# apple/ml-4m

Hardware: AMD Instinct MI355X
Metric: multimodal tokens/sec (4M-B train step, whole job) (higher is better)
Workload: dtype bf16; 1 GPU; 4M-B mod7 (fm_base_12e_12d_swiglu_nobias, 360.8M params, 8 input / 7 target modalities) masked-modeling train step, 224^2 token grids, 128 input + 128 target tokens/sample, AdamW; model=fm_base_12e_12d_swiglu_nobias, per_gpu_batch=256, global_batch=256, seq_len=256, parallelism=dp1

## Files before the change

include/fourm_hip.h:

```cpp
#ifndef FOURM_HIP_H
#define FOURM_HIP_H
#include <stdint.h>

#ifdef __cplusplus
extern "C" {
#endif

#define FM_ABI_VERSION 11
int fm_abi_version(void);
const char* fm_last_error(void);

enum fm_epilogue {
    FM_EPI_BF16 = 0,
    FM_EPI_GELU = 1,
    FM_EPI_RESIDUAL = 2,
    FM_EPI_SWIGLU = 3,
    FM_EPI_F32 = 4,
    FM_EPI_TANH = 5,
    FM_EPI_SWIGLU_BWD = 6,
    FM_EPI_GELU_BWD = 7
};

typedef struct fm_gemm_group {
    const void* W;
    void* out;
    int32_t N, K, ldw, pad_;
} fm_gemm_group;

typedef struct fm_gemm_nt_args {
    const void* W; const void* W2; const void* X;
    void* out; void* out2; const void* res; const void* bias; const void* bias2;
    int32_t M, N, K, ldw, ldx, ldo, ldo2, ldr, Hp, epilogue;
    const fm_gemm_group* groups; const int32_t* tile_group; int32_t max_N;
    int32_t fixed_tiling;
    const int32_t* m_dev; const int32_t* row0_dev;
    void* splitk_ws; int64_t splitk_ws_bytes;
    int32_t conv_C, conv_H, conv_W, conv_Ho, conv_Wo, conv_stride, conv_up, conv_pad_;
} fm_gemm_nt_args;
int fm_gemm_nt(const fm_gemm_nt_args* args, void* stream);
void fm_set_gemm_nt_config(int cfg);
int fm_get_gemm_nt_config(void);
void fm_set_reserved_cus(int n);
int fm_get_reserved_cus(void);

typedef struct fm_gemm_tn_args {
    const void* A; const void* B; void* out;
    int32_t R, N, K, lda, ldb, ldo, a_cols, b_cols, splits, force_tr;
    const fm_gemm_group* groups; const int32_t* seg_start; const int32_t* seg_count;
    int32_t n_groups, max_N, max_R, pad_;
} fm_gemm_tn_args;
int fm_gemm_tn(const fm_gemm_tn_args* args, void* stream);
#define FM_TN_MAX_JOBS 16
typedef struct fm_gemm_tn_job {
    const void* A; const void* B; void* out;
    int32_t R, N, K, lda, ldb, ldo, a_cols, b_cols;
} fm_gemm_tn_job;
int fm_gemm_tn_multi(const fm_gemm_tn_job* jobs, int n_jobs, void* stream);
void fm_set_gemm_tn_config(int cfg);
int fm_get_gemm_tn_config(void);
void fm_set_tn_transpose_read(int on);
int fm_get_tn_transpose_read(void);

int fm_layernorm_fwd(const void* x, int ldx, const void* w, const void* b, void* y, int ldy, int y_is_f32,
                     void* mean, void* rstd, const int32_t* row_map, int R, int D, float eps, void* stream);
int fm_layernorm_fwd_res(const void* x, int ldx, const void* delta, int ldd, void* x_out, int ldxo, const void* w, const void* b,
                         void* y, int ldy, int y_is_f32, void* mean, void* rstd, const int32_t* row_map, int R, int D, float eps,
                         void* stream);
int fm_layernorm_bwd(const void* dy, int lddy, const int32_t* dy_row_map, const void* x, int ldx, const void* w,
                     const void* mean, const void* rstd, const void* dres, void* dx, int lddx, void* dx_bf16,
                     int lddxbf, void* dw, void* db, int R, int D, void* stream);
int fm_layernorm_bwd_h(const void* dy, int lddy, const void* h, int ldh, const void* x, int ldx, const void* w,
                       const void* mean, const void* rstd, const void* dres, void* dx, int lddx, void* dx_bf16,
                       int lddxbf, void* dw, int R, int D, void* stream);

int fm_headnorm_fwd(const void* x, int ldx, const void* w, const void* b, void* y, int ldy, void* stats, int R, int H, float eps,
                    void* stream);
int fm_headnorm_bwd(const void* dy, int lddy, const void* x, int ldx, const void* w, const void* stats, void* dx, int lddx, void* dw,
                    void* db, int R, int H, void* stream);

enum fm_mask_kind {
    FM_MASK_NONE = 0,
    FM_MASK_KEYPAD = 1,
    FM_MASK_DECODER = 2,
    FM_MASK_DENSE = 3
};
typedef struct fm_attn_args {
    const void* Q; const void* K; const void* V; void* O;
    void* stat_m; void* stat_l;
    int32_t ldq, ldk, ldv, ldo;
    int32_t B, H, Nq, Nk, head_dim, mask_kind;
    float scale; int32_t causal;
    const void* kpad; const int32_t* cs; const int16_t* modq; const int16_t* modk; const void* dense;
    const void* dO; void* dQ; void* dK; void* dV;
    int32_t lddo, lddq, lddk, lddv;
    int32_t force_tr;
    int32_t kv_batch_rows;
    int32_t zero_attn;
} fm_attn_args;
int fm_attn_fwd(const fm_attn_args* args, void* stream);
int fm_attn_bwd(const fm_attn_args* args, void* stream);
void fm_set_attn_transpose_read(int on);
int fm_get_attn_transpose_read(void);

#define FM_ATTN_DECODE_MAX_NK 8192
typedef struct fm_attn_decode_args {
    const void* q; void* k; const void* v; void* o;
    const void* q_w; const void* q_b; const void* k_w; const void* k_b;
    const void* kpad;
    int32_t ldq, ldk, ldv, ldo;
    int32_t B, H, Nk, kv_batch_rows, k_new_row, is_f32, zero_attn, pad_;
    float scale, eps;
} fm_attn_decode_args;
int fm_attn_decode(const fm_attn_decode_args* args, void* stream);

#define FM_MAX_MODS 24
enum fm_mod_kind {
    FM_KIND_TOK = 0,
    FM_KIND_PATCH = 1,
    FM_KIND_SEQ = 2,
    FM_KIND_SEQ_EMB = 3
};
typedef struct fm_mod_desc {
    const void* ids;
    const void* mask;
    const void* dam;
    const void* table;
    const void* pos;
    const void* mod_emb;
    const void* proj_bias;
    int32_t L;
    int32_t kind, ids_are_i64, mod_id;
    int32_t max_len;
    int32_t shifted;
    int32_t mask_stride, id_stride;
    int32_t patch, channels, grid_w, orig_dim;
    int32_t head_index;
    int32_t pad_;
} fm_mod_desc;

typedef struct fm_select_desc {
    fm_mod_desc mods[FM_MAX_MODS];
    int32_t n_mods, batch, dim, n_keep, n_reg, total_len, is_decoder;
    int32_t raw;
    const void* reg_tokens;
    const void* mask_token;
    void* tokens;
    void* emb;
    void* x0;
    void* out_mask;
    void* out_mod;
    void* slot_mod;
    void* slot_src;
    void* slot_pos;
    void* target_ids;
    void* out_cs;
    void* out_mod_pre;
    void* out_mod_index;
    void* patch_rows;
    void* seqemb_rows;
    int32_t patch_ld, seqemb_ld;
    int32_t rows_f32;
    int32_t pad2_;
} fm_select_desc;
int fm_select_embed(const fm_select_desc* desc, void* stream);

typedef struct fm_embed_bwd_mod {
    void* d_table;
    void* d_pos;
    void* d_mod_emb;
    void* d_proj_bias;
    int32_t kind, has_padding_idx, padding_idx, pad_;
} fm_embed_bwd_mod;
typedef struct fm_embed_bwd_desc {
    fm_embed_bwd_mod mods[FM_MAX_MODS];
    const void* dx;
    const void* slot_mod; const void* slot_src; const void* slot_pos;
    void* d_mask_token;
    void* d_reg_tokens;
    int32_t n_mods, batch, dim, Nt, lddx, is_decoder;
} fm_embed_bwd_desc;
int fm_embed_bwd(const fm_embed_bwd_desc* desc, void* stream);

int fm_dense_decoder_mask(const int32_t* cs, const int16_t* mod, void* out, int B, int M, int causal, int use_cs,
                          int use_sep, void* stream);

enum fm_loss_type { FM_LOSS_MOD = 0, FM_LOSS_TOKEN = 1 };
#define FM_SEG_ROWS 256
int fm_segment_rows(const int32_t* head_of_row, int R, int n_heads, int32_t* seg_start, int32_t* seg_count,
                    int32_t* perm, int32_t* row_to_padded, int32_t* tile_group, int Rp, void* stream);
int fm_gather_rows(const void* src, int ld_src, const int32_t* perm, void* dst, int ld_dst, int Rp, int D, void* stream);
int fm_cross_entropy(void* logits, int ldl, const int32_t* perm, const int32_t* tile_group, const int64_t* target_ids,
                     const int32_t* vocab, const int32_t* seg_start, const int32_t* seg_count, const void* grad_scale,
                     int loss_type, int n_heads, int Rp, int max_vocab, void* row_loss, void* row_lse, void* head_loss,
                     void* total_loss, int write_grad, void* stream);

int fm_swiglu_bwd(const void* da, int ldda, const void* gu, int ldgu, void* dgu, int lddgu, int R, int H, int Hp, void* stream);
int fm_gelu_bwd(const void* dh, int lddh, const void* pre, int ldp, void* dpre, int lddp, int R, int H, int Hp, void* stream);
typedef struct fm_shadow_desc {
    const void* src; void* dst;
    int32_t ld_src, ld_dst, rows, cols, transpose, tile_start;
    const void* col_scale;
    int32_t dst_f32, reserved;
} fm_shadow_desc;
int fm_shadow_refresh(const fm_shadow_desc* descs, int n_descs, int total_tiles, void* stream);
#define FM_FOLD_MAX_JOBS 48
typedef struct fm_fold_grad_job {
    const void* dWp; const void* W; const void* gamma; void* gW; void* ggamma;
    int32_t rows, cols, ld_dwp, reserved;
} fm_fold_grad_job;
int fm_fold_colscale_grad(const fm_fold_grad_job* jobs, int n_jobs, void* stream);

int fm_cast_pad(const void* src, int ld_src, void* dst, int ld_dst, int rows, int cols, void* stream);
int fm_transpose_cast_pad(const void* src, int ld_src, void* dst, int ld_dst, int dst_cols, int rows, int cols, void* stream);
int fm_colsum(const void* dy, int ldy, void* db, int R, int N, void* stream);
int fm_f32_to_bf16(const void* src, void* dst, int64_t n, void* stream);
int fm_bf16_to_f32_scaled(const void* src, void* dst, int64_t n, float scale, void* stream);
int fm_add_bf16_f32(const void* x, const void* delta, void* out, int64_t n, void* stream);
int fm_scale_rows_bf16(void* x, int ld, const void* scale, int rows_per_sample, int R, int N, void* stream);

int fm_vit_patch_rows(const void* pixels, void* rows, int ld, int B, int C, int H, int W, int P, int rows_f32, void* stream);
int fm_vit_emb_rows(const void* pos, const void* mod_emb, void* x, int ldx, int B, int Np, int D, void* stream);
int fm_vit_colsum(const void* dy, int ldy, void* db, int R, int N, void* ws, int64_t ws_bytes, void* stream);

int fm_lora_apply(const void* x, int ldx, const void* down, int64_t down_sr, int64_t down_sk, const void* up, int64_t up_sn, int64_t up_sr,
                  void* y, int ldy, float scale, void* p_out, int R, int K, int N, int r, int x_f32, int y_f32, void* stream);
int fm_lora_grad(const void* a, int lda, const void* b, void* out, int64_t out_sn, int64_t out_sr, float scale, int accumulate,
                 int R, int n, int r, int a_f32, void* stream);

int fm_adamw(void* p, const void* g, void* m, void* v, int64_t n, float lr, float beta1, float beta2, float eps,
             float weight_decay, int64_t step, const void* grad_mult, const void* hyper, void* sumsq, void* stream);
#define FM_ADAMW_CHUNK 8192
typedef struct fm_adamw_job {
    void* p; const void* g; void* m; void* v; void* dst_plain; void* dst_t;
    int32_t rows, cols, ld_plain, ld_t, tile_start, pad_;
} fm_adamw_job;
int fm_adamw_shadow(const fm_adamw_job* jobs, int n_jobs, int total_tiles, float lr, float beta1, float beta2, float eps,
                    float weight_decay, int64_t step, const void* grad_mult, const void* hyper, void* sumsq, void* stream);
int fm_sumsq(const void* x, int64_t n, void* out, void* stream);
int fm_clip_coef(const void* sumsq, float max_norm, void* norm_out, void* coef_out, void* stream);

int fm_sample_tokens(const void* logits, int ld, int logits_are_f32, int R, int V, float temperature, int top_k, float top_p,
                     const void* uniforms, void* out_ids, void* out_prob, void* stream);
int fm_guidance_combine(const void* uncond, int ldu, int uncond_is_f32, const void* cond, int ldc, int cond_is_f32, float weight,
                        void* out, int ldo, int R, int V, int accumulate, void* stream);
int fm_maskgit_commit(const void* prob, const void* samples, const int32_t* mod_pos, int B, int N, int num_select, void* tensor,
                      int tensor_is_i64, int L, void* input_mask, void* target_mask, int32_t* top_idx, void* stream);

typedef struct fm_gemm_f32_args {
    const void* X; const void* W; const void* W2; void* out; void* out2; const void* res; const void* bias; const void* bias2;
    int64_t sxm, sxk, swn, swk;
    int32_t M, N, K, ldo, ldo2, ldr, Hp, epilogue, accumulate, max_N, seg_rows, n_groups;
    const fm_gemm_group* groups; const int32_t* tile_group; const int32_t* seg_start; const int32_t* seg_count;
} fm_gemm_f32_args;
int fm_gemm_f32(const fm_gemm_f32_args* args, void* stream);
int fm_attn_f32_fwd(const fm_attn_args* args, void* stream);
int fm_attn_f32_bwd(const fm_attn_args* args, void* stream);
int fm_layernorm_bwd_f32(const void* dy, int lddy, const int32_t* dy_row_map, const void* x, int ldx, const void* w, const void* mean,
                         const void* rstd, const void* dres, void* dx, int lddx, void* dx2, int lddx2, void* dw, void* db, int R, int D,
                         void* stream);
int fm_headnorm_f32_fwd(const void* x, int ldx, const void* w, const void* b, void* y, int ldy, void* stats, int R, int H, float eps, void* stream);
int fm_headnorm_f32_bwd(const void* dy, int lddy, const void* x, int ldx, const void* w, const void* stats, void* dx, int lddx, void* dw, void* db,
                        int R, int H, void* stream);
int fm_swiglu_bwd_f32(const void* da, int ldda, const void* gu, int ldgu, void* dgu, int lddgu, int R, int H, int Hp, void* stream);
int fm_gelu_bwd_f32(const void* dh, int lddh, const void* pre, int ldp, void* dpre, int lddp, int R, int H, void* stream);
int fm_colsum_f32(const void* dy, int ldy, void* db, int R, int N, void* stream);
int fm_cross_entropy_f32(void* logits, int ldl, const int32_t* perm, const int32_t* tile_group, const int64_t* target_ids,
                         const int32_t* vocab, const int32_t* seg_start, const int32_t* seg_count, const void* grad_scale, int loss_type,
                         int n_heads, int padded_rows, int max_vocab, void* row_loss, void* row_lse, void* head_loss, void* total_loss,
                         int write_grad, void* stream);

int fm_unet_im2col_f32(const void* src1, int ld1, int C1, const void* src2, int ld2, int C2, int H2, int W2, void* out, int ldo, int kpad,
                       int B, int H, int W, int ksize, int stride, int up1, void* stream);
int fm_groupnorm_nhwc_f32(const void* x, int ldx, const void* add, int ld_add, const void* w, const void* b, void* y, int ldy, int B, int HW, int C,
                          int groups, float eps, int silu, void* stream);
int fm_unet_attention_f32(const void* qkv, int ld, void* out, int ldo, int B, int T, int heads, int ch, void* stream);
int fm_add_f32(const void* a, int lda, const void* b, int ldb, void* out, int ldo, int64_t rows, int C, void* stream);
int fm_silu_f32(const void* x, void* y, int64_t n, void* stream);
int fm_timestep_embedding_f32(const void* t, void* out, int ldo, int B, int dim, float max_period, void* stream);
int fm_unet_col2im_f32(const void* col, int ldc, void* dsrc, int ld, int C, int B, int H, int W, int ksize, int stride, int up1, int accumulate, void* stream);
int fm_groupnorm_nhwc_bwd_f32(const void* dy, int lddy, const void* x, int ldx, const void* add, int ld_add, const void* w, const void* b, void* dx, int lddx,
                              void* dw, void* db, void* dadd, int ld_dadd, void* scratch, int B, int HW, int C, int groups, float eps, int silu, void* stream);
int fm_unet_attention_bwd_f32(const void* qkv, int ld, const void* dout, int lddo, void* dqkv, int lddqkv, void* scratch, int B, int T, int heads, int ch,
                              void* stream);
int fm_silu_bwd_f32(const void* dy, const void* x, void* dx, int64_t n, void* stream);

int fm_vq_patchify(const void* img, void* out, int ld_out, int B, int C, int H, int W, int P, void* stream);
int fm_l2norm_rows(const void* x, int ldx, void* y, int ldy, int R, int D, void* stream);
int fm_vq_assign(const void* z, int ldz, const void* codes_normalized, const void* embed, int K, int D, int R,
                 int tokens_per_image, int normalize_latents, void* ws_val, void* ws_idx, int splits, int64_t* tokens,
                 void* quant, void* stream);
#define FM_VQ_WIDE_TILE 128
int fm_vq_assign_wide(const void* z, int ldz, const void* codes_normalized, const void* embed, int K, int D, int R,
                      int tokens_per_image, void* ws_val, void* ws_idx, int code_tiles, int64_t* tokens, void* quant, void* stream);
int fm_memcodes_assign(const void* z, int ldz, const void* keys, const void* values, int K, int d, int H, int R,
                       int tokens_per_image, void* ws_val, void* ws_idx, int code_tiles, int64_t* tokens, void* quant, void* stream);
int fm_vq_code_stats(const void* z, int ldz, const int64_t* tokens, int R, int D, int K, void* bins, void* sums, void* stream);
int fm_vq_ema_update(const void* bins, const void* sums, void* embed, void* cluster_size, int K, int D, float decay, void* stream);
int fm_vq_code_bias(const void* embed, int K, int D, void* bias, void* stream);
int fm_vq_assign_bias(const void* z, int ldz, const void* codes, const void* code_bias, const void* embed, int K, int D, int R,
                      int tokens_per_image, int normalize_latents, void* ws_val, void* ws_idx, int splits, int64_t* tokens,
                      void* quant, void* stream);
int fm_vq_code_stats_raw(const void* z, int ldz, const int64_t* tokens, int R, int D, int K, void* bins, void* sums, void* stream);
int fm_vq_ema_update_euclid(const void* bins, const void* sums, void* embed, void* embed_avg, void* cluster_size, void* total_scratch,
                            int K, int D, float decay, float eps, void* stream);

int fm_vq_unpatchify(const void* rows, int ld_rows, void* img, int B, int C, int H, int W, int P, void* stream);
#define FM_CONVNEXT_MAX_C 4
int fm_convnext_block(const void* x, void* y, const void* dw_weight, const void* dw_bias, const void* ln_weight, const void* ln_bias,
                      const void* pw1_weight, const void* pw1_bias, const void* pw2_weight, const void* pw2_bias, const void* gamma,
                      int B, int C, int H, int W, float eps, void* stream);
int fm_vq_latent_grad(const void* z, int ldz, const void* embed, const int64_t* tokens, const void* dquant, int ld_dquant, const void* grad_loss,
                      float commitment_weight, void* dz, int ld_dz, void* commit_value, int R, int D, void* stream);
int fm_tanh_bwd_f32(const void* dy, const void* t, void* dx, int R, int N, int ld, void* stream);
int fm_embed_rows_f32(const void* table, const int64_t* idx, void* out, int ld_out, int R, int D, void* stream);
int fm_split3_bf16(const void* x, int ldx, void* out, int ldo, int R, int K, int weight_order, int apply_tanh, void* stream);
int fm_vq_patchify_ex(const void* img, const int64_t* labels, const void* cls_emb, const void* scale, const void* shift, void* out, int ld_out,
                      int B, int C, int H, int W, int P, void* stream);
int fm_vq_cls_emb_bwd(const void* d_patches, int ld, const int64_t* labels, void* d_cls_emb, int B, int C, int H, int W, int P, void* stream);
int fm_vq_latent_grad_normalized(const void* z, int ldz, const void* embed, const int64_t* tokens, const void* dquant, int ld_dquant, const void* grad_loss,
                                 float commitment_weight, void* dz, int ld_dz, void* commit_value, int R, int D, void* stream);

int fm_image_mask(const void* noise, const int32_t* input_budget, const int32_t* target_budget, int B, int L, void* input_mask,
                  void* target_mask, int32_t* decoder_attention_mask, void* stream);

int fm_unpack_image_u8(const void* src, void* dst, int B, int H, int W, int C, const float* mean, const float* stdv, void* stream);
int fm_unpack_ids_u16(const void* src, int64_t* dst, int64_t n, void* stream);
int fm_unpack_mask_bits(const void* bits, void* dst, int B, int L, void* stream);
int fm_decoder_attention_from_target(const void* target_mask, int32_t* decoder_attention_mask, int B, int L, void* stream);

int fm_token_budgets(const void* main_draws, const void* extra_draws, const int32_t* num_tokens, const int32_t* min_tokens,
                     const int32_t* max_tokens, const void* is_img, const int32_t* input_budget, int B, int T, int E, int M,
                     int32_t* budget, int32_t* tries, void* stream);

typedef struct fm_span_mask_args {
    const int32_t* ids; const int32_t* len; const int32_t* unit; const void* noise; const double* keep_prob; const int32_t* r_choice;
    const int32_t* input_budget; const int32_t* target_budget; const int32_t* sentinel_ids;
    const void* emb; void* emb_out; int32_t* src;
    int32_t* tensor; void* input_mask; void* target_mask; int32_t* decoder_attention_mask; int32_t* tries;
    int32_t B, ld_ids, T, ld_noise, n_sentinels, max_tokens, vocab_offset, pad_id, emb_rows, emb_dim;
} fm_span_mask_args;
int fm_span_mask(const fm_span_mask_args* p, void* stream);

int fm_unet_im2col(const void* src1, int ld1, int C1, const void* src2, int ld2, int C2, int H2, int W2, void* out, int ldo, int kpad,
// ... 19 lines not shown
```

ml-4m_amd/csrc/layernorm.hip:

```cpp
#include <algorithm>
#include "common.h"
#include "fourm_hip.h"

namespace {

constexpr int MAXC_LIMIT = 8;

__device__ __forceinline__ float4 ld4(const float* p, bool nt) {
    if (nt) { const f32x4_t t = __builtin_nontemporal_load((const f32x4_t*)p); return make_float4(t[0], t[1], t[2], t[3]); }
    return *(const float4*)p;
}
__device__ __forceinline__ uint2 ld2u(const bf16_t* p, bool nt) {
    typedef __attribute__((ext_vector_type(2))) unsigned int u2_t;
    if (nt) { const u2_t t = __builtin_nontemporal_load((const u2_t*)p); return make_uint2(t[0], t[1]); }
    return *(const uint2*)p;
}
template <typename T> __device__ __forceinline__ void store4(T* p, float a, float b, float c, float d);
template <> __device__ __forceinline__ void store4<float>(float* p, float a, float b, float c, float d) {
    *(float4*)p = make_float4(a, b, c, d);
}
template <> __device__ __forceinline__ void store4<bf16_t>(bf16_t* p, float a, float b, float c, float d) {
    *(uint2*)p = make_uint2(pack2bf(a, b), pack2bf(c, d));
}

template <typename OutT, int MAXC, bool RES = false>
__global__ __launch_bounds__(256) void ln_fwd_kernel(const float* __restrict__ x, int ldx, const float* __restrict__ w,
                                                     const float* __restrict__ b, OutT* __restrict__ y, int ldy,
                                                     float* __restrict__ mean, float* __restrict__ rstd,
                                                     const int* __restrict__ row_map, int R, int D, float eps,
                                                     const bf16_t* __restrict__ delta = nullptr, int ldd = 0, float* __restrict__ xo = nullptr, int ldxo = 0,
                                                     int nt_res = 0) {
    const int lane = threadIdx.x & 63, wave = threadIdx.x >> 6;
    const int nch = D >> 2;
    float4 ww[MAXC], bb[MAXC];
#pragma unroll
    for (int c = 0; c < MAXC; ++c) {
        const int ch = lane + 64 * c;
        ww[c] = ch < nch ? *(const float4*)(w + ch * 4) : make_float4(0.f, 0.f, 0.f, 0.f);
        bb[c] = (b && ch < nch) ? *(const float4*)(b + ch * 4) : make_float4(0.f, 0.f, 0.f, 0.f);
    }
    constexpr int NR = 2;
    for (int r0 = blockIdx.x * 4 + wave; r0 < R; r0 += gridDim.x * 4 * NR) {
        float4 v[NR][MAXC];
#pragma unroll
        for (int q = 0; q < NR; ++q) {
            const int r = r0 + q * gridDim.x * 4;
#pragma unroll
            for (int c = 0; c < MAXC; ++c) {
                const int ch = lane + 64 * c;
                v[q][c] = (ch < nch && r < R) ? ld4(x + (size_t)r * ldx + ch * 4, nt_res & 2) : make_float4(0.f, 0.f, 0.f, 0.f);
            }
        }
        if constexpr (RES) {
            uint2 dl[NR][MAXC];
#pragma unroll
            for (int q = 0; q < NR; ++q) {
                const int r = r0 + q * gridDim.x * 4;
#pragma unroll
                for (int c = 0; c < MAXC; ++c) {
                    const int ch = lane + 64 * c;
                    dl[q][c] = (ch < nch && r < R) ? ld2u(delta + (size_t)r * ldd + ch * 4, nt_res & 2) : make_uint2(0u, 0u);
                }
            }
#pragma unroll
            for (int q = 0; q < NR; ++q) {
                const int r = r0 + q * gridDim.x * 4;
#pragma unroll
                for (int c = 0; c < MAXC; ++c) {
                    const int ch = lane + 64 * c;
                    float d4[4];
                    unpack_bf4(dl[q][c], d4);
                    v[q][c].x += d4[0]; v[q][c].y += d4[1]; v[q][c].z += d4[2]; v[q][c].w += d4[3];
                    if (ch < nch && r < R) {
                        if (nt_res & 1) __builtin_nontemporal_store(f32x4_t{v[q][c].x, v[q][c].y, v[q][c].z, v[q][c].w}, (f32x4_t*)(xo + (size_t)r * ldxo + ch * 4));
                        else *(float4*)(xo + (size_t)r * ldxo + ch * 4) = v[q][c];
                    }
                }
            }
        }
#pragma unroll
        for (int q = 0; q < NR; ++q) {
            const int r = r0 + q * gridDim.x * 4;
            if (r >= R) continue;
            float s = 0.f;
#pragma unroll
            for (int c = 0; c < MAXC; ++c) s += (v[q][c].x + v[q][c].y) + (v[q][c].z + v[q][c].w);
            const float mu = wave_sum(s) / (float)D;
            float sq = 0.f;
#pragma unroll
            for (int c = 0; c < MAXC; ++c) {
                const int ch = lane + 64 * c;
                if (ch < nch) {
                    const float a0 = v[q][c].x - mu, a1 = v[q][c].y - mu, a2 = v[q][c].z - mu, a3 = v[q][c].w - mu;
                    sq += (a0 * a0 + a1 * a1) + (a2 * a2 + a3 * a3);
                }
            }
            const float rs = rsqrtf(wave_sum(sq) / (float)D + eps);
            if (lane == 0) {
                if (mean) mean[r] = mu;
                if (rstd) rstd[r] = rs;
            }
            const int dst = row_map ? row_map[r] : r;
            if (dst < 0) continue;
            OutT* yr = y + (size_t)dst * ldy;
#pragma unroll
            for (int c = 0; c < MAXC; ++c) {
                const int ch = lane + 64 * c;
                if (ch < nch)
                    store4<OutT>(yr + ch * 4, (v[q][c].x - mu) * rs * ww[c].x + bb[c].x, (v[q][c].y - mu) * rs * ww[c].y + bb[c].y,
                                 (v[q][c].z - mu) * rs * ww[c].z + bb[c].z, (v[q][c].w - mu) * rs * ww[c].w + bb[c].w);
            }
        }
    }
}

static int ln_nt_flags() {
    static const int f = [] { const char* e = getenv("FOURM_LN_NT"); return e ? atoi(e) : 24; }();
    return f;
}
static int bwd_rows(int R) {
    static const int env = [] { const char* e = getenv("FOURM_LN_BWD_ROWS"); return e ? atoi(e) : 0; }();
    if (env >= 4) return env;
    return R >= 512 * 64 ? 64 : 32;
}

template <int MAXC, bool FROM_H = false, bool HAS_DB = true>
__global__ __launch_bounds__(256) void ln_bwd_kernel(const bf16_t* __restrict__ dy, int lddy, const int* __restrict__ dy_row_map,
                                                     const bf16_t* __restrict__ h, int ldh,
                                                     const float* __restrict__ x, int ldx, const float* __restrict__ w,
                                                     const float* __restrict__ mean, const float* __restrict__ rstd,
                                                     const float* dres, float* dx, int lddx, bf16_t* __restrict__ dx_bf, int lddxbf,
                                                     float* __restrict__ dw, float* __restrict__ db, int R, int D, int BWD_ROWS, int nt_dx) {
    extern __shared__ __attribute__((aligned(16))) char smem[];
    float* red = (float*)smem;
    const int lane = threadIdx.x & 63, wave = threadIdx.x >> 6;
    const int nch = D >> 2;
    float4 aw[MAXC], ab[MAXC], wv[MAXC], iw[FROM_H ? MAXC : 1];
    bool from_x[FROM_H ? MAXC : 1];
#pragma unroll
    for (int c = 0; c < MAXC; ++c) {
        aw[c] = ab[c] = make_float4(0.f, 0.f, 0.f, 0.f);
        const int ch = lane + 64 * c;
        wv[c] = ch < nch ? *(const float4*)(w + ch * 4) : make_float4(0.f, 0.f, 0.f, 0.f);
        if constexpr (FROM_H) {
            from_x[c] = fminf(fminf(fabsf(wv[c].x), fabsf(wv[c].y)), fminf(fabsf(wv[c].z), fabsf(wv[c].w))) < 1e-20f;
            iw[c] = from_x[c] ? make_float4(0.f, 0.f, 0.f, 0.f) : make_float4(1.f / wv[c].x, 1.f / wv[c].y, 1.f / wv[c].z, 1.f / wv[c].w);
        }
    }
    const int r_end = min(R, (int)(blockIdx.x + 1) * BWD_ROWS);
    constexpr int NR = 2;
    for (int r0 = blockIdx.x * BWD_ROWS + wave; r0 < r_end; r0 += 4 * NR) {
        uint2 dyp[NR][MAXC], hp[NR][FROM_H ? MAXC : 1];
        float4 xv[NR][MAXC], rv[NR][MAXC];
        float mu[NR], rs[NR];
        bool live[NR];
#pragma unroll
        for (int q = 0; q < NR; ++q) {
            const int r = r0 + 4 * q;
            live[q] = r < r_end;
            const int rr = live[q] ? r : r0;
            const int src = dy_row_map ? dy_row_map[rr] : rr;
            mu[q] = mean[rr]; rs[q] = rstd[rr];
#pragma unroll
            for (int c = 0; c < MAXC; ++c) {
                const int ch = lane + 64 * c;
                dyp[q][c] = make_uint2(0u, 0u);
                xv[q][c] = rv[q][c] = make_float4(0.f, 0.f, 0.f, 0.f);
                if (ch < nch && live[q]) {
                    if (src >= 0) dyp[q][c] = ld2u(dy + (size_t)src * lddy + ch * 4, nt_dx & 2);
                    if constexpr (FROM_H) {
                        hp[q][c] = ld2u(h + (size_t)rr * ldh + ch * 4, nt_dx & 4);
                        if (from_x[c]) xv[q][c] = *(const float4*)(x + (size_t)rr * ldx + ch * 4);
                    } else xv[q][c] = *(const float4*)(x + (size_t)rr * ldx + ch * 4);
                    if (dres) rv[q][c] = ld4(dres + (size_t)rr * lddx + ch * 4, nt_dx & 2);
                }
            }
        }
#pragma unroll
        for (int q = 0; q < NR; ++q) {
            if (!live[q]) continue;
            const int r = r0 + 4 * q;
            float4 g[MAXC], xh[MAXC];
            float s1 = 0.f, s2 = 0.f;
#pragma unroll
            for (int c = 0; c < MAXC; ++c) {
                const int ch = lane + 64 * c;
                g[c] = xh[c] = make_float4(0.f, 0.f, 0.f, 0.f);
                if (ch < nch) {
                    const uint2 p = dyp[q][c];
                    const float4 d = make_float4(bf2f((bf16_t)(p.x & 0xffff)), bf2f((bf16_t)(p.x >> 16)), bf2f((bf16_t)(p.y & 0xffff)), bf2f((bf16_t)(p.y >> 16)));
                    const float4 v = xv[q][c];
                    xh[c] = make_float4((v.x - mu[q]) * rs[q], (v.y - mu[q]) * rs[q], (v.z - mu[q]) * rs[q], (v.w - mu[q]) * rs[q]);
                    if constexpr (FROM_H) {
                        const uint2 hh = hp[q][c];
                        if (!from_x[c]) xh[c] = make_float4(bf2f((bf16_t)(hh.x & 0xffff)) * iw[c].x, bf2f((bf16_t)(hh.x >> 16)) * iw[c].y,
                                                            bf2f((bf16_t)(hh.y & 0xffff)) * iw[c].z, bf2f((bf16_t)(hh.y >> 16)) * iw[c].w);
                    }
                    aw[c].x += d.x * xh[c].x; aw[c].y += d.y * xh[c].y; aw[c].z += d.z * xh[c].z; aw[c].w += d.w * xh[c].w;
                    if constexpr (HAS_DB) { ab[c].x += d.x; ab[c].y += d.y; ab[c].z += d.z; ab[c].w += d.w; }
                    g[c] = make_float4(d.x * wv[c].x, d.y * wv[c].y, d.z * wv[c].z, d.w * wv[c].w);
                    s1 += (g[c].x + g[c].y) + (g[c].z + g[c].w);
                    s2 += (g[c].x * xh[c].x + g[c].y * xh[c].y) + (g[c].z * xh[c].z + g[c].w * xh[c].w);
                }
            }
            const float m1 = wave_sum(s1) / (float)D, m2 = wave_sum(s2) / (float)D;
#pragma unroll
            for (int c = 0; c < MAXC; ++c) {
                const int ch = lane + 64 * c;
                if (ch < nch) {
                    const float4 t = rv[q][c];
                    const float4 o = make_float4(rs[q] * (g[c].x - m1 - xh[c].x * m2) + t.x, rs[q] * (g[c].y - m1 - xh[c].y * m2) + t.y,
                                                 rs[q] * (g[c].z - m1 - xh[c].z * m2) + t.z, rs[q] * (g[c].w - m1 - xh[c].w * m2) + t.w);
                    if (nt_dx & 1) __builtin_nontemporal_store(f32x4_t{o.x, o.y, o.z, o.w}, (f32x4_t*)(dx + (size_t)r * lddx + ch * 4));
                    else *(float4*)(dx + (size_t)r * lddx + ch * 4) = o;
                    if (dx_bf) *(uint2*)(dx_bf + (size_t)r * lddxbf + ch * 4) = make_uint2(pack2bf(o.x, o.y), pack2bf(o.z, o.w));
                }
            }
        }
    }
    if (!dw && !db) return;
#pragma unroll
    for (int c = 0; c < MAXC; ++c) {
        const int ch = lane + 64 * c;
        if (ch < nch) {
            *(float4*)(red + (size_t)wave * D + ch * 4) = aw[c];
            if constexpr (HAS_DB) *(float4*)(red + (size_t)(4 + wave) * D + ch * 4) = ab[c];
        }
    }
    __syncthreads();
    for (int i = threadIdx.x; i < D; i += 256) {
        if (dw) unsafeAtomicAdd(dw + i, (red[i] + red[D + i]) + (red[2 * D + i] + red[3 * D + i]));
        if constexpr (HAS_DB) if (db) unsafeAtomicAdd(db + i, (red[4 * D + i] + red[5 * D + i]) + (red[6 * D + i] + red[7 * D + i]));
    }
}


__device__ __forceinline__ float group16_sum(float v) {
    v += __shfl_xor(v, 1, 64); v += __shfl_xor(v, 2, 64); v += __shfl_xor(v, 4, 64); v += __shfl_xor(v, 8, 64);
    return v;
}

__global__ __launch_bounds__(256) void headnorm_fwd_kernel(const bf16_t* __restrict__ x, int ldx, const float* __restrict__ w,
                                                           const float* __restrict__ b, bf16_t* __restrict__ y, int ldy,
                                                           float2* __restrict__ stats, int R, int H, float eps) {
    const int sub = threadIdx.x & 15;
    const float4 wv = *(const float4*)(w + sub * 4);
    const float4 bv = b ? *(const float4*)(b + sub * 4) : make_float4(0.f, 0.f, 0.f, 0.f);
    const size_t total = (size_t)R * H;
    for (size_t v = (size_t)blockIdx.x * 16 + (threadIdx.x >> 4); v < total; v += (size_t)gridDim.x * 16) {
        const int r = v / H, h = v % H;
        const uint2 p = *(const uint2*)(x + (size_t)r * ldx + h * 64 + sub * 4);
        const float e[4] = {bf2f((bf16_t)(p.x & 0xffff)), bf2f((bf16_t)(p.x >> 16)), bf2f((bf16_t)(p.y & 0xffff)), bf2f((bf16_t)(p.y >> 16))};
        const float mean = group16_sum(e[0] + e[1] + e[2] + e[3]) * (1.0f / 64.0f);
        float q = 0.f;
#pragma unroll
        for (int i = 0; i < 4; ++i) q += (e[i] - mean) * (e[i] - mean);
        const float rs = rsqrtf(group16_sum(q) * (1.0f / 64.0f) + eps);
        const float o0 = (e[0] - mean) * rs * wv.x + bv.x, o1 = (e[1] - mean) * rs * wv.y + bv.y;
        const float o2 = (e[2] - mean) * rs * wv.z + bv.z, o3 = (e[3] - mean) * rs * wv.w + bv.w;
        *(uint2*)(y + (size_t)r * ldy + h * 64 + sub * 4) = make_uint2(pack2bf(o0, o1), pack2bf(o2, o3));
        if (sub == 0 && stats) stats[v] = make_float2(mean, rs);
    }
}

__global__ __launch_bounds__(256) void headnorm_bwd_kernel(const bf16_t* __restrict__ dy, int lddy, const bf16_t* __restrict__ x, int ldx,
                                                           const float* __restrict__ w, const float2* __restrict__ stats,
                                                           bf16_t* __restrict__ dx, int lddx, float* __restrict__ dw, float* __restrict__ db,
                                                           int R, int H) {
    __shared__ float red[2][16][64];
    const int sub = threadIdx.x & 15, grp = threadIdx.x >> 4;
    const float4 wv = *(const float4*)(w + sub * 4);
    const float wj[4] = {wv.x, wv.y, wv.z, wv.w};
    float aw[4] = {0.f, 0.f, 0.f, 0.f}, ab[4] = {0.f, 0.f, 0.f, 0.f};
    const size_t total = (size_t)R * H;
    for (size_t v = (size_t)blockIdx.x * 16 + grp; v < total; v += (size_t)gridDim.x * 16) {
        const int r = v / H, h = v % H;
        const uint2 px = *(const uint2*)(x + (size_t)r * ldx + h * 64 + sub * 4);
        const uint2 pd = *(const uint2*)(dy + (size_t)r * lddy + h * 64 + sub * 4);
        const float2 st = stats[v];
        const float e[4] = {bf2f((bf16_t)(px.x & 0xffff)), bf2f((bf16_t)(px.x >> 16)), bf2f((bf16_t)(px.y & 0xffff)), bf2f((bf16_t)(px.y >> 16))};
        const float d[4] = {bf2f((bf16_t)(pd.x & 0xffff)), bf2f((bf16_t)(pd.x >> 16)), bf2f((bf16_t)(pd.y & 0xffff)), bf2f((bf16_t)(pd.y >> 16))};
        float xh[4], g[4], s1 = 0.f, s2 = 0.f;
#pragma unroll
        for (int i = 0; i < 4; ++i) {
            xh[i] = (e[i] - st.x) * st.y;
            g[i] = d[i] * wj[i];
            s1 += g[i]; s2 += g[i] * xh[i];
            aw[i] += d[i] * xh[i]; ab[i] += d[i];
        }
        s1 = group16_sum(s1) * (1.0f / 64.0f); s2 = group16_sum(s2) * (1.0f / 64.0f);
        float o[4];
#pragma unroll
        for (int i = 0; i < 4; ++i) o[i] = st.y * (g[i] - s1 - xh[i] * s2);
        *(uint2*)(dx + (size_t)r * lddx + h * 64 + sub * 4) = make_uint2(pack2bf(o[0], o[1]), pack2bf(o[2], o[3]));
    }
#pragma unroll
    for (int i = 0; i < 4; ++i) { red[0][grp][sub * 4 + i] = aw[i]; red[1][grp][sub * 4 + i] = ab[i]; }
    __syncthreads();
    if (threadIdx.x < 128) {
        const int which = threadIdx.x >> 6, c = threadIdx.x & 63;
        float s = 0.f;
#pragma unroll
        for (int gq = 0; gq < 16; ++gq) s += red[which][gq][c];
        float* dst = which ? db : dw;
        if (dst) unsafeAtomicAdd(dst + c, s);
    }
}

}

static int chunks_for(int D) { const int c = (D / 4 + 63) / 64; return c <= 2 ? 2 : c <= 3 ? 3 : c <= 4 ? 4 : 8; }

extern "C" int fm_layernorm_fwd(const void* x, int ldx, const void* w, const void* b, void* y, int ldy, int y_is_f32,
                                void* mean, void* rstd, const int32_t* row_map, int R, int D, float eps, void* stream) {
    FM_CHECK_ARG(x && w && y, "fm_layernorm_fwd: null pointer");
    FM_CHECK_ARG(R > 0 && D > 0 && D % 4 == 0 && D <= 64 * 4 * MAXC_LIMIT, "fm_layernorm_fwd: D=%d must be a multiple of 4 and <= %d", D, 64 * 4 * MAXC_LIMIT);
    FM_CHECK_ARG(ldx % 4 == 0 && ldy % 4 == 0, "fm_layernorm_fwd: leading dims must be multiples of 4");
    int grid = (R + 3) / 4;
    if (grid > 256 * 16) grid = 256 * 16;
#define LN_FWD(T, C)                                                                                                        \
    hipLaunchKernelGGL((ln_fwd_kernel<T, C>), dim3(grid), dim3(256), 0, (hipStream_t)stream, (const float*)x, ldx, (const float*)w, \
                       (const float*)b, (T*)y, ldy, (float*)mean, (float*)rstd, row_map, R, D, eps)
#define LN_FWD_C(T)                                    \
    switch (chunks_for(D)) {                           \
        case 2: LN_FWD(T, 2); break;                   \
        case 3: LN_FWD(T, 3); break;                   \
        case 4: LN_FWD(T, 4); break;                   \
        default: LN_FWD(T, 8); break;                  \
    }
    if (y_is_f32) { LN_FWD_C(float) } else { LN_FWD_C(bf16_t) }
#undef LN_FWD_C
#undef LN_FWD
    FM_CHECK_LAUNCH("fm_layernorm_fwd");
    return 0;
}

extern "C" int fm_layernorm_fwd_res(const void* x, int ldx, const void* delta, int ldd, void* x_out, int ldxo, const void* w, const void* b,
                                    void* y, int ldy, int y_is_f32, void* mean, void* rstd, const int32_t* row_map, int R, int D, float eps,
                                    void* stream) {
    FM_CHECK_ARG(x && delta && x_out && w && y, "fm_layernorm_fwd_res: null pointer");
    FM_CHECK_ARG(R > 0 && D > 0 && D % 4 == 0 && D <= 64 * 4 * MAXC_LIMIT, "fm_layernorm_fwd_res: D=%d must be a multiple of 4 and <= %d", D, 64 * 4 * MAXC_LIMIT);
    FM_CHECK_ARG(ldx % 4 == 0 && ldy % 4 == 0 && ldd % 4 == 0 && ldxo % 4 == 0, "fm_layernorm_fwd_res: leading dims must be multiples of 4");
    FM_CHECK_ARG((((uintptr_t)delta) & 7) == 0 && (((uintptr_t)x_out | (uintptr_t)x) & 15) == 0, "fm_layernorm_fwd_res: alignment (delta 8 B, x / x_out 16 B)");
    int grid = (R + 3) / 4;
    if (grid > 256 * 16) grid = 256 * 16;
#define LN_FWD(T, C)                                                                                                        \
    hipLaunchKernelGGL((ln_fwd_kernel<T, C, true>), dim3(grid), dim3(256), 0, (hipStream_t)stream, (const float*)x, ldx, (const float*)w, \
                       (const float*)b, (T*)y, ldy, (float*)mean, (float*)rstd, row_map, R, D, eps, (const bf16_t*)delta, ldd, (float*)x_out, ldxo, (ln_nt_flags() & 1) | ((ln_nt_flags() >> 1) & 2))
#define LN_FWD_C(T)                                    \
    switch (chunks_for(D)) {                           \
        case 2: LN_FWD(T, 2); break;                   \
        case 3: LN_FWD(T, 3); break;                   \
        case 4: LN_FWD(T, 4); break;                   \
        default: LN_FWD(T, 8); break;                  \
    }
    if (y_is_f32) { LN_FWD_C(float) } else { LN_FWD_C(bf16_t) }
#undef LN_FWD_C
#undef LN_FWD
    FM_CHECK_LAUNCH("fm_layernorm_fwd_res");
    return 0;
}

static int layernorm_bwd_launch(const void* dy, int lddy, const int32_t* dy_row_map, const void* h, int ldh, const void* x, int ldx, const void* w,
                                const void* mean, const void* rstd, const void* dres, void* dx, int lddx, void* dx_bf16,
                                int lddxbf, void* dw, void* db, int R, int D, void* stream) {
    FM_CHECK_ARG(dy && x && w && mean && rstd && dx, "fm_layernorm_bwd: null pointer");
    FM_CHECK_ARG(!h || ldh % 4 == 0, "fm_layernorm_bwd_h: ldh must be a multiple of 4");
    FM_CHECK_ARG(R > 0 && D > 0 && D % 4 == 0 && D <= 64 * 4 * MAXC_LIMIT, "fm_layernorm_bwd: D=%d unsupported", D);
    FM_CHECK_ARG(ldx % 4 == 0 && lddy % 4 == 0 && lddx % 4 == 0 && lddxbf % 4 == 0, "fm_layernorm_bwd: leading dims must be multiples of 4");
    const int BWD_ROWS = bwd_rows(R);
    const int grid = (R + BWD_ROWS - 1) / BWD_ROWS;
    const size_t lds = (size_t)8 * D * sizeof(float);
#define LN_BWD_(C, FH)                                                                                                      \
    {                                                                                                                       \
        auto k = ln_bwd_kernel<C, FH, !FH>;                                                                                     \
        static bool once = (hipFuncSetAttribute((const void*)k, hipFuncAttributeMaxDynamicSharedMemorySize, 8 * 2048 * 4) == hipSuccess); \
        (void)once;                                                                                                         \
        hipLaunchKernelGGL(k, dim3(grid), dim3(256), lds, (hipStream_t)stream, (const bf16_t*)dy, lddy, dy_row_map, (const bf16_t*)h, ldh, \
                           (const float*)x, ldx, (const float*)w, (const float*)mean, (const float*)rstd, (const float*)dres, (float*)dx, lddx, \
                           (bf16_t*)dx_bf16, lddxbf, (float*)dw, (float*)db, R, D, BWD_ROWS, ((ln_nt_flags() >> 1) & 1) | ((ln_nt_flags() >> 2) & 2) | ((ln_nt_flags() >> 2) & 4));                               \
    }
#define LN_BWD(C) { if (h) LN_BWD_(C, true) else LN_BWD_(C, false) }
    switch (chunks_for(D)) {
        case 2: LN_BWD(2) break;
        case 3: LN_BWD(3) break;
        case 4: LN_BWD(4) break;
        default: LN_BWD(8) break;
    }
#undef LN_BWD
#undef LN_BWD_
    FM_CHECK_LAUNCH("fm_layernorm_bwd");
    return 0;
}

extern "C" int fm_layernorm_bwd(const void* dy, int lddy, const int32_t* dy_row_map, const void* x, int ldx, const void* w,
                                const void* mean, const void* rstd, const void* dres, void* dx, int lddx, void* dx_bf16,
                                int lddxbf, void* dw, void* db, int R, int D, void* stream) {
    return layernorm_bwd_launch(dy, lddy, dy_row_map, nullptr, 0, x, ldx, w, mean, rstd, dres, dx, lddx, dx_bf16, lddxbf, dw, db, R, D, stream);
}

extern "C" int fm_layernorm_bwd_h(const void* dy, int lddy, const void* h, int ldh, const void* x, int ldx, const void* w,
                                  const void* mean, const void* rstd, const void* dres, void* dx, int lddx, void* dx_bf16,
                                  int lddxbf, void* dw, int R, int D, void* stream) {
    FM_CHECK_ARG(h, "fm_layernorm_bwd_h: null pointer");
    return layernorm_bwd_launch(dy, lddy, nullptr, h, ldh, x, ldx, w, mean, rstd, dres, dx, lddx, dx_bf16, lddxbf, dw, nullptr, R, D, stream);
}

extern "C" int fm_headnorm_fwd(const void* x, int ldx, const void* w, const void* b, void* y, int ldy, void* stats, int R, int H, float eps,
                               void* stream) {
    FM_CHECK_ARG(x && w && y && R > 0 && H > 0, "fm_headnorm_fwd: bad argument");
    FM_CHECK_ARG(ldx % 4 == 0 && ldy % 4 == 0 && ((((uintptr_t)x | (uintptr_t)y) & 7) == 0) && ((((uintptr_t)w | (uintptr_t)b) & 15) == 0),
                 "fm_headnorm_fwd: alignment (x/y 8 B, w/b 16 B, leading dims %% 4)");
    const size_t total = (size_t)R * H;
    const int grid = (int)std::min<size_t>((total + 15) / 16, 256 * 32);
    hipLaunchKernelGGL(headnorm_fwd_kernel, dim3(grid), dim3(256), 0, (hipStream_t)stream, (const bf16_t*)x, ldx, (const float*)w, (const float*)b,
                       (bf16_t*)y, ldy, (float2*)stats, R, H, eps);
    FM_CHECK_LAUNCH("fm_headnorm_fwd");
    return 0;
}

extern "C" int fm_headnorm_bwd(const void* dy, int lddy, const void* x, int ldx, const void* w, const void* stats, void* dx, int lddx, void* dw,
                               void* db, int R, int H, void* stream) {
    FM_CHECK_ARG(dy && x && w && stats && dx && R > 0 && H > 0, "fm_headnorm_bwd: bad argument");
    FM_CHECK_ARG(ldx % 4 == 0 && lddy % 4 == 0 && lddx % 4 == 0 && ((((uintptr_t)x | (uintptr_t)dy | (uintptr_t)dx) & 7) == 0) &&
                     ((((uintptr_t)w) & 15) == 0), "fm_headnorm_bwd: alignment (x/dy/dx 8 B, w 16 B, leading dims %% 4)");
    const size_t total = (size_t)R * H;
    const int grid = (int)std::min<size_t>((total + 15) / 16, 256 * 8);
    hipLaunchKernelGGL(headnorm_bwd_kernel, dim3(grid), dim3(256), 0, (hipStream_t)stream, (const bf16_t*)dy, lddy, (const bf16_t*)x, ldx,
                       (const float*)w, (const float2*)stats, (bf16_t*)dx, lddx, (float*)dw, (float*)db, R, H);
    FM_CHECK_LAUNCH("fm_headnorm_bwd");
    return 0;
}
```

ml-4m_amd/csrc/loss.hip:

```cpp
#include "common.h"
#include "fourm_hip.h"

namespace {

constexpr int SEG_ALIGN = FM_SEG_ROWS;

__global__ __launch_bounds__(1024) void segment_rows_kernel(const int32_t* __restrict__ head_of_row, int R, int n_heads,
                                                            int32_t* __restrict__ seg_start, int32_t* __restrict__ seg_count,
                                                            int32_t* __restrict__ perm, int32_t* __restrict__ row_to_padded,
                                                            int32_t* __restrict__ tile_group, int Rp) {
    __shared__ int cnt[FM_MAX_MODS];
    __shared__ int wtot[16];
    const int g = blockIdx.x, tid = threadIdx.x, lane = tid & 63, wave = tid >> 6;
    if (tid < FM_MAX_MODS) cnt[tid] = 0;
    __syncthreads();
    for (int r = tid; r < R; r += 1024) {
        const int hh = head_of_row[r];
        if (hh >= 0 && hh <= g) atomicAdd(&cnt[hh], 1);
    }
    __syncthreads();
    int start = 0;
    for (int m = 0; m < g; ++m) start += (cnt[m] + SEG_ALIGN - 1) / SEG_ALIGN * SEG_ALIGN;
    const int mine = cnt[g];
    const int padded = (mine + SEG_ALIGN - 1) / SEG_ALIGN * SEG_ALIGN;
    if (tid == 0) { seg_start[g] = start; seg_count[g] = mine; }
    for (int t = tid; t < padded / SEG_ALIGN; t += 1024) tile_group[start / SEG_ALIGN + t] = g;
    if (g == n_heads - 1) {
        for (int t = (start + padded) / SEG_ALIGN + tid; t < Rp / SEG_ALIGN; t += 1024) tile_group[t] = -1;
        for (int r = start + padded + tid; r < Rp; r += 1024) perm[r] = -1;
    }
    for (int r = start + mine + tid; r < start + padded; r += 1024) perm[r] = -1;
    int run = 0;
    for (int base = 0; base < R; base += 1024) {
        const int r = base + tid;
        const int f = (r < R && head_of_row[r] == g) ? 1 : 0;
        const int inc = wave_scan_incl(f);
        if (lane == 63) wtot[wave] = inc;
        __syncthreads();
        int off = 0, tot = 0;
        for (int w = 0; w < 16; ++w) { if (w < wave) off += wtot[w]; tot += wtot[w]; }
        __syncthreads();
        if (f) {
            const int dst = start + run + off + inc - 1;
            perm[dst] = r;
            row_to_padded[r] = dst;
        }
        run += tot;
    }
}

__global__ void fill_i32_kernel(int32_t* p, int v, int n) {
    const int i = blockIdx.x * 256 + threadIdx.x;
    if (i < n) p[i] = v;
}

__device__ __forceinline__ void online_merge(float& m, float& s, float m2, float s2) {
    const float mn = fmaxf(m, m2);
    s = s * __expf(m - mn) + s2 * __expf(m2 - mn);
    m = mn;
}

__global__ __launch_bounds__(256) void ce_fwd_kernel(const bf16_t* __restrict__ logits, int ldl, const int32_t* __restrict__ perm,
                                                     const int32_t* __restrict__ tile_group, const long long* __restrict__ target_ids,
                                                     const int32_t* __restrict__ vocab, float* __restrict__ row_loss, float* __restrict__ row_lse) {
    __shared__ float red_m[4], red_s[4];
    const int pr = blockIdx.x;
    const int g = tile_group[pr / SEG_ALIGN];
    if (g < 0) return;
    const int src = perm[pr];
    if (src < 0) {
        if (threadIdx.x == 0) { row_loss[pr] = 0.f; row_lse[pr] = 0.f; }
        return;
    }
    const int V = vocab[g];
    const bf16_t* row = logits + (size_t)pr * ldl;
    float m = -INFINITY, ssum = 0.f;
    for (int c = threadIdx.x * 8; c < V; c += 256 * 8) {
        float v[8];
        if (c + 8 <= V) {
            const uint4 p = *(const uint4*)(row + c);
            const uint32_t w[4] = {p.x, p.y, p.z, p.w};
#pragma unroll
            for (int e = 0; e < 4; ++e) { v[2 * e] = bf2f((bf16_t)(w[e] & 0xffff)); v[2 * e + 1] = bf2f((bf16_t)(w[e] >> 16)); }
        } else {
#pragma unroll
            for (int e = 0; e < 8; ++e) v[e] = c + e < V ? bf2f(row[c + e]) : -INFINITY;
        }
        float cm = v[0];
#pragma unroll
        for (int e = 1; e < 8; ++e) cm = fmaxf(cm, v[e]);
        const float mn = fmaxf(m, cm);
        float add = 0.f;
#pragma unroll
        for (int e = 0; e < 8; ++e) add += __expf(v[e] - mn);
        ssum = ssum * __expf(m - mn) + add;
        m = mn;
    }
#pragma unroll
    for (int o = 32; o > 0; o >>= 1) {
        const float m2 = __shfl_xor(m, o, 64), s2 = __shfl_xor(ssum, o, 64);
        if (m2 > -INFINITY || m > -INFINITY) online_merge(m, ssum, m2, s2);
    }
    const int lane = threadIdx.x & 63, wave = threadIdx.x >> 6;
    if (lane == 0) { red_m[wave] = m; red_s[wave] = ssum; }
    __syncthreads();
    if (threadIdx.x == 0) {
        float M = red_m[0], S = red_s[0];
        for (int w = 1; w < 4; ++w)
            if (red_m[w] > -INFINITY) online_merge(M, S, red_m[w], red_s[w]);
        const float lse = M + __logf(S);
        row_lse[pr] = lse;
        row_loss[pr] = lse - bf2f(row[target_ids[src]]);
    }
}

__global__ __launch_bounds__(256) void ce_bwd_kernel(bf16_t* __restrict__ logits, int ldl, const int32_t* __restrict__ perm,
                                                     const int32_t* __restrict__ tile_group, const long long* __restrict__ target_ids,
                                                     const int32_t* __restrict__ vocab, const int32_t* __restrict__ seg_count,
                                                     const float* __restrict__ gscale, int loss_type, int n_heads,
                                                     const float* __restrict__ row_lse) {
    const int pr = blockIdx.x;
    const int g = tile_group[pr / SEG_ALIGN];
    if (g < 0) return;
    const int V = vocab[g];
    const int Vp = (V + 63) / 64 * 64;
    bf16_t* row = logits + (size_t)pr * ldl;
    const int src = perm[pr];
    if (src < 0) {
        for (int c = threadIdx.x; c < Vp / 8; c += 256) *(uint4*)(row + c * 8) = make_uint4(0u, 0u, 0u, 0u);
        return;
    }
    float w;
    if (loss_type == FM_LOSS_MOD) {
        w = 1.0f / ((float)seg_count[g] * (float)n_heads);
    } else {
        float tot = 0.f;
        for (int mm = 0; mm < n_heads; ++mm) tot += (float)seg_count[mm] * (float)vocab[mm];
        w = (float)V / tot;
    }
    w *= gscale ? gscale[0] : 1.0f;
    const float lse = row_lse[pr];
    const int tgt = (int)target_ids[src];
    for (int c = threadIdx.x * 8; c < Vp; c += 256 * 8) {
        const uint4 p = *(const uint4*)(row + c);
        const uint32_t wd[4] = {p.x, p.y, p.z, p.w};
        float o[8];
#pragma unroll
        for (int e = 0; e < 8; ++e) {
            const float x = bf2f((bf16_t)((e & 1) ? (wd[e >> 1] >> 16) : (wd[e >> 1] & 0xffff)));
            o[e] = (c + e < V) ? (__expf(x - lse) - ((c + e) == tgt ? 1.f : 0.f)) * w : 0.f;
        }
        *(uint4*)(row + c) = make_uint4(pack2bf(o[0], o[1]), pack2bf(o[2], o[3]), pack2bf(o[4], o[5]), pack2bf(o[6], o[7]));
    }
}

__global__ __launch_bounds__(256) void loss_finalize_kernel(const float* __restrict__ row_loss, const int32_t* __restrict__ seg_start,
                                                            const int32_t* __restrict__ seg_count, const int32_t* __restrict__ vocab,
                                                            int n_heads, int loss_type, float* __restrict__ head_loss, float* __restrict__ total) {
    __shared__ float red[4];
    __shared__ float hl[FM_MAX_MODS];
    const int lane = threadIdx.x & 63, wave = threadIdx.x >> 6;
    for (int g = 0; g < n_heads; ++g) {
        const int s0 = seg_start[g], n = seg_count[g];
        float s = 0.f;
        for (int i = threadIdx.x; i < n; i += 256) s += row_loss[s0 + i];
        s = wave_sum(s);
        if (lane == 0) red[wave] = s;
        __syncthreads();
        if (threadIdx.x == 0) hl[g] = n > 0 ? ((red[0] + red[1]) + (red[2] + red[3])) / (float)n : 0.f;
        __syncthreads();
    }
    if (threadIdx.x == 0) {
        float tot = 0.f, wsum = 0.f;
        for (int g = 0; g < n_heads; ++g) {
            head_loss[g] = hl[g];
            if (loss_type == FM_LOSS_MOD) { tot += hl[g]; wsum += 1.f; }
            else { const float w = (float)seg_count[g] * (float)vocab[g]; tot += hl[g] * w; wsum += w; }
        }
        total[0] = tot / wsum;
    }
}

__global__ __launch_bounds__(256) void ce_f32_kernel(float* logits, int ld, const int* perm, const int* tile_group, const long long* target_ids,
                                                     const int* vocab, const int* seg_count, const float* grad_scale, int loss_type, int n_heads,
                                                     float* row_loss, float* row_lse, int write_grad, int seg_rows) {
    __shared__ float red[4];
    const int pr = blockIdx.x;
    const int g = tile_group[pr / seg_rows];
    if (g < 0) return;
    const int src = perm[pr];
    const int V = vocab[g];
    float* row = logits + (size_t)pr * ld;
    if (src < 0) {
        if (!write_grad) { if (threadIdx.x == 0) { row_loss[pr] = 0.f; row_lse[pr] = 0.f; } }
        else for (int c = threadIdx.x; c < V; c += 256) row[c] = 0.f;
        return;
    }
    const int tgt = (int)target_ids[src];
    if (!write_grad) {
        float mx = -INFINITY;
        for (int c = threadIdx.x; c < V; c += 256) mx = fmaxf(mx, row[c]);
        mx = wave_max(mx);
        __syncthreads();
        if ((threadIdx.x & 63) == 0) red[threadIdx.x >> 6] = mx;
        __syncthreads();
        mx = fmaxf(fmaxf(red[0], red[1]), fmaxf(red[2], red[3]));
        float s = 0.f;
        for (int c = threadIdx.x; c < V; c += 256) s += expf(row[c] - mx);
        s = wave_sum(s);
        __syncthreads();
        if ((threadIdx.x & 63) == 0) red[threadIdx.x >> 6] = s;
        __syncthreads();
        s = (red[0] + red[1]) + (red[2] + red[3]);
        const float lse = mx + logf(s);
        if (threadIdx.x == 0) { row_lse[pr] = lse; row_loss[pr] = lse - row[tgt]; }
        return;
    }
    float coef;
    if (loss_type == FM_LOSS_MOD) coef = 1.0f / ((float)n_heads * (float)seg_count[g]);
    else {
        double tot = 0.0;
        for (int h = 0; h < n_heads; ++h) tot += (double)seg_count[h] * (double)vocab[h];
        coef = (float)((double)V / tot);
    }
    coef *= grad_scale ? grad_scale[0] : 1.0f;
    const float lse = row_lse[pr];
    for (int c = threadIdx.x; c < V; c += 256) row[c] = coef * (expf(row[c] - lse) - (c == tgt ? 1.0f : 0.f));
}


__global__ __launch_bounds__(256) void gather_rows_kernel(const bf16_t* __restrict__ src, int lds_, const int32_t* __restrict__ perm,
                                                          bf16_t* __restrict__ dst, int ldd, int Rp, int D) {
    const int lane = threadIdx.x & 63, wave = threadIdx.x >> 6;
    for (int pr = blockIdx.x * 4 + wave; pr < Rp; pr += gridDim.x * 4) {
        const int s = perm[pr];
        for (int c = lane; c < D / 8; c += 64) {
            uint4 v = make_uint4(0u, 0u, 0u, 0u);
            if (s >= 0) v = *(const uint4*)(src + (size_t)s * lds_ + c * 8);
            *(uint4*)(dst + (size_t)pr * ldd + c * 8) = v;
        }
    }
}

}

extern "C" int fm_segment_rows(const int32_t* head_of_row, int R, int n_heads, int32_t* seg_start, int32_t* seg_count,
                               int32_t* perm, int32_t* row_to_padded, int32_t* tile_group, int Rp, void* stream) {
    FM_CHECK_ARG(head_of_row && seg_start && seg_count && perm && row_to_padded && tile_group, "fm_segment_rows: null pointer");
    FM_CHECK_ARG(n_heads > 0 && n_heads <= FM_MAX_MODS && R > 0, "fm_segment_rows: bad shape");
    FM_CHECK_ARG(Rp % SEG_ALIGN == 0 && Rp >= (R + SEG_ALIGN - 1) / SEG_ALIGN * SEG_ALIGN + (n_heads - 1) * SEG_ALIGN,
                 "fm_segment_rows: padded capacity Rp=%d too small for R=%d rows in %d segments", Rp, R, n_heads);
    hipLaunchKernelGGL(fill_i32_kernel, dim3((R + 255) / 256), dim3(256), 0, (hipStream_t)stream, row_to_padded, -1, R);
    hipLaunchKernelGGL(segment_rows_kernel, dim3(n_heads), dim3(1024), 0, (hipStream_t)stream, head_of_row, R, n_heads, seg_start,
                       seg_count, perm, row_to_padded, tile_group, Rp);
    FM_CHECK_LAUNCH("fm_segment_rows");
    return 0;
}

extern "C" int fm_gather_rows(const void* src, int ld_src, const int32_t* perm, void* dst, int ld_dst, int Rp, int D, void* stream) {
    FM_CHECK_ARG(src && perm && dst && D % 8 == 0 && ld_src % 8 == 0 && ld_dst % 8 == 0, "fm_gather_rows: bad argument");
    int grid = (Rp + 3) / 4;
    if (grid > 4096) grid = 4096;
    hipLaunchKernelGGL(gather_rows_kernel, dim3(grid), dim3(256), 0, (hipStream_t)stream, (const bf16_t*)src, ld_src, perm, (bf16_t*)dst, ld_dst, Rp, D);
    FM_CHECK_LAUNCH("fm_gather_rows");
    return 0;
}

extern "C" int fm_cross_entropy(void* logits, int ldl, const int32_t* perm, const int32_t* tile_group, const int64_t* target_ids,
                                const int32_t* vocab, const int32_t* seg_start, const int32_t* seg_count, const void* grad_scale,
                                int loss_type, int n_heads, int Rp, int max_vocab, void* row_loss, void* row_lse, void* head_loss,
                                void* total_loss, int write_grad, void* stream) {
    FM_CHECK_ARG(logits && perm && tile_group && target_ids && vocab && seg_start && seg_count && row_loss && row_lse && head_loss && total_loss,
                 "fm_cross_entropy: null pointer");
    FM_CHECK_ARG(loss_type == FM_LOSS_MOD || loss_type == FM_LOSS_TOKEN, "fm_cross_entropy: invalid loss type %d", loss_type);
    FM_CHECK_ARG(ldl % 8 == 0 && ldl >= (max_vocab + 63) / 64 * 64, "fm_cross_entropy: ldl=%d too small for vocab %d", ldl, max_vocab);
    FM_CHECK_ARG((((uintptr_t)logits) & 15) == 0, "fm_cross_entropy: logits must be 16-byte aligned");
    if (!write_grad) {
        hipLaunchKernelGGL(ce_fwd_kernel, dim3(Rp), dim3(256), 0, (hipStream_t)stream, (const bf16_t*)logits, ldl, perm, tile_group,
                           (const long long*)target_ids, vocab, (float*)row_loss, (float*)row_lse);
        hipLaunchKernelGGL(loss_finalize_kernel, dim3(1), dim3(256), 0, (hipStream_t)stream, (const float*)row_loss, seg_start, seg_count,
                           vocab, n_heads, loss_type, (float*)head_loss, (float*)total_loss);
    } else {
        hipLaunchKernelGGL(ce_bwd_kernel, dim3(Rp), dim3(256), 0, (hipStream_t)stream, (bf16_t*)logits, ldl, perm, tile_group,
                           (const long long*)target_ids, vocab, seg_count, (const float*)grad_scale, loss_type, n_heads, (const float*)row_lse);
    }
    FM_CHECK_LAUNCH("fm_cross_entropy");
    return 0;
}

extern "C" int fm_cross_entropy_f32(void* logits, int ldl, const int32_t* perm, const int32_t* tile_group, const int64_t* target_ids,
                                    const int32_t* vocab, const int32_t* seg_start, const int32_t* seg_count, const void* grad_scale,
                                    int loss_type, int n_heads, int Rp, int max_vocab, void* row_loss, void* row_lse, void* head_loss,
                                    void* total_loss, int write_grad, void* stream) {
    FM_CHECK_ARG(logits && perm && tile_group && target_ids && vocab && seg_start && seg_count && row_loss && row_lse && head_loss && total_loss,
                 "fm_cross_entropy_f32: null pointer");
    FM_CHECK_ARG(loss_type == FM_LOSS_MOD || loss_type == FM_LOSS_TOKEN, "fm_cross_entropy_f32: invalid loss type %d", loss_type);
    FM_CHECK_ARG(ldl >= max_vocab, "fm_cross_entropy_f32: ldl=%d too small for vocab %d", ldl, max_vocab);
    hipLaunchKernelGGL(ce_f32_kernel, dim3(Rp), dim3(256), 0, (hipStream_t)stream, (float*)logits, ldl, perm, tile_group,
                       (const long long*)target_ids, vocab, seg_count, (const float*)grad_scale, loss_type, n_heads, (float*)row_loss,
                       (float*)row_lse, write_grad, SEG_ALIGN);
    if (!write_grad)
        hipLaunchKernelGGL(loss_finalize_kernel, dim3(1), dim3(256), 0, (hipStream_t)stream, (const float*)row_loss, seg_start, seg_count,
                           vocab, n_heads, loss_type, (float*)head_loss, (float*)total_loss);
    FM_CHECK_LAUNCH("fm_cross_entropy_f32");
    return 0;
}
```

ml-4m_amd/fourm/hip/_lib.py:

```python
import ctypes as C
import os

FM_MAX_MODS = 24
_LIB_PATH = os.environ.get("FOURM_HIP_LIB") or os.path.join(os.path.dirname(os.path.dirname(os.path.abspath(__file__))), "_lib", "libfourm_hip.so")


class FourmHipUnavailable(ImportError):
    pass


def _load():
    if not os.path.exists(_LIB_PATH):
        raise FourmHipUnavailable(
            f"{_LIB_PATH} is missing - build the gfx950 kernels first: python ml-4m_amd/build_ext.py "
            "(the 4M hot path has no fallback implementation)")
    return C.CDLL(_LIB_PATH)


lib = _load()
lib.fm_last_error.restype = C.c_char_p
lib.fm_abi_version.restype = C.c_int
ABI_VERSION = 11
if lib.fm_abi_version() != ABI_VERSION:
    raise FourmHipUnavailable(f"libfourm_hip.so ABI {lib.fm_abi_version()} != expected {ABI_VERSION}; rebuild")

vp, i32, i64, f32 = C.c_void_p, C.c_int32, C.c_int64, C.c_float

EPI_BF16, EPI_GELU, EPI_RESIDUAL, EPI_SWIGLU, EPI_F32, EPI_TANH, EPI_SWIGLU_BWD, EPI_GELU_BWD = 0, 1, 2, 3, 4, 5, 6, 7
MASK_NONE, MASK_KEYPAD, MASK_DECODER, MASK_DENSE = 0, 1, 2, 3
KIND_TOK, KIND_PATCH, KIND_SEQ, KIND_SEQ_EMB = 0, 1, 2, 3
LOSS_MOD, LOSS_TOKEN = 0, 1


class GemmGroup(C.Structure):
    _fields_ = [("W", vp), ("out", vp), ("N", i32), ("K", i32), ("ldw", i32), ("pad_", i32)]


class GemmNTArgs(C.Structure):
    _fields_ = [("W", vp), ("W2", vp), ("X", vp), ("out", vp), ("out2", vp), ("res", vp), ("bias", vp), ("bias2", vp),
                ("M", i32), ("N", i32), ("K", i32), ("ldw", i32), ("ldx", i32), ("ldo", i32), ("ldo2", i32), ("ldr", i32),
                ("Hp", i32), ("epilogue", i32), ("groups", vp), ("tile_group", vp), ("max_N", i32), ("fixed_tiling", i32),
                ("m_dev", vp), ("row0_dev", vp), ("splitk_ws", vp), ("splitk_ws_bytes", i64),
                ("conv_C", i32), ("conv_H", i32), ("conv_W", i32), ("conv_Ho", i32), ("conv_Wo", i32), ("conv_stride", i32), ("conv_up", i32), ("conv_pad_", i32)]


class GemmTNArgs(C.Structure):
    _fields_ = [("A", vp), ("B", vp), ("out", vp), ("R", i32), ("N", i32), ("K", i32), ("lda", i32), ("ldb", i32),
                ("ldo", i32), ("a_cols", i32), ("b_cols", i32), ("splits", i32), ("force_tr", i32), ("groups", vp),
                ("seg_start", vp), ("seg_count", vp), ("n_groups", i32), ("max_N", i32), ("max_R", i32), ("pad_", i32)]


class GemmTNJob(C.Structure):
    _fields_ = [("A", vp), ("B", vp), ("out", vp), ("R", i32), ("N", i32), ("K", i32), ("lda", i32), ("ldb", i32),
                ("ldo", i32), ("a_cols", i32), ("b_cols", i32)]


TN_MAX_JOBS = 16


class AttnArgs(C.Structure):
    _fields_ = [("Q", vp), ("K", vp), ("V", vp), ("O", vp), ("stat_m", vp), ("stat_l", vp),
                ("ldq", i32), ("ldk", i32), ("ldv", i32), ("ldo", i32),
                ("B", i32), ("H", i32), ("Nq", i32), ("Nk", i32), ("head_dim", i32), ("mask_kind", i32),
                ("scale", f32), ("causal", i32),
                ("kpad", vp), ("cs", vp), ("modq", vp), ("modk", vp), ("dense", vp),
                ("dO", vp), ("dQ", vp), ("dK", vp), ("dV", vp),
                ("lddo", i32), ("lddq", i32), ("lddk", i32), ("lddv", i32), ("force_tr", i32), ("kv_batch_rows", i32), ("zero_attn", i32)]


class AttnDecodeArgs(C.Structure):
    _fields_ = [("q", vp), ("k", vp), ("v", vp), ("o", vp), ("q_w", vp), ("q_b", vp), ("k_w", vp), ("k_b", vp), ("kpad", vp),
                ("ldq", i32), ("ldk", i32), ("ldv", i32), ("ldo", i32),
                ("B", i32), ("H", i32), ("Nk", i32), ("kv_batch_rows", i32), ("k_new_row", i32), ("is_f32", i32), ("zero_attn", i32), ("pad_", i32),
                ("scale", f32), ("eps", f32)]


class ModDesc(C.Structure):
    _fields_ = [("ids", vp), ("mask", vp), ("dam", vp), ("table", vp), ("pos", vp), ("mod_emb", vp), ("proj_bias", vp),
                ("L", i32), ("kind", i32), ("ids_are_i64", i32), ("mod_id", i32), ("max_len", i32), ("shifted", i32),
                ("mask_stride", i32), ("id_stride", i32), ("patch", i32), ("channels", i32), ("grid_w", i32),
                ("orig_dim", i32), ("head_index", i32), ("pad_", i32)]


class ShadowDesc(C.Structure):
    _fields_ = [("src", vp), ("dst", vp), ("ld_src", i32), ("ld_dst", i32), ("rows", i32), ("cols", i32),
                ("transpose", i32), ("tile_start", i32), ("col_scale", vp), ("dst_f32", i32), ("reserved", i32)]


FOLD_MAX_JOBS = 48


class FoldGradJob(C.Structure):
    _fields_ = [("dWp", vp), ("W", vp), ("gamma", vp), ("gW", vp), ("ggamma", vp), ("rows", i32), ("cols", i32), ("ld_dwp", i32), ("reserved", i32)]


class GemmF32Args(C.Structure):
    _fields_ = [("X", vp), ("W", vp), ("W2", vp), ("out", vp), ("out2", vp), ("res", vp), ("bias", vp), ("bias2", vp),
                ("sxm", i64), ("sxk", i64), ("swn", i64), ("swk", i64),
                ("M", i32), ("N", i32), ("K", i32), ("ldo", i32), ("ldo2", i32), ("ldr", i32), ("Hp", i32), ("epilogue", i32),
                ("accumulate", i32), ("max_N", i32), ("seg_rows", i32), ("n_groups", i32),
                ("groups", vp), ("tile_group", vp), ("seg_start", vp), ("seg_count", vp)]


class SpanMaskArgs(C.Structure):
    _fields_ = [("ids", vp), ("len", vp), ("unit", vp), ("noise", vp), ("keep_prob", vp), ("r_choice", vp), ("input_budget", vp), ("target_budget", vp),
                ("sentinel_ids", vp), ("emb", vp), ("emb_out", vp), ("src", vp), ("tensor", vp), ("input_mask", vp), ("target_mask", vp),
                ("decoder_attention_mask", vp), ("tries", vp),
                ("B", i32), ("ld_ids", i32), ("T", i32), ("ld_noise", i32), ("n_sentinels", i32), ("max_tokens", i32), ("vocab_offset", i32), ("pad_id", i32),
                ("emb_rows", i32), ("emb_dim", i32)]


class AdamWJob(C.Structure):
    _fields_ = [("p", vp), ("g", vp), ("m", vp), ("v", vp), ("dst_plain", vp), ("dst_t", vp),
                ("rows", i32), ("cols", i32), ("ld_plain", i32), ("ld_t", i32), ("tile_start", i32), ("pad_", i32)]


class SelectDesc(C.Structure):
    _fields_ = [("mods", ModDesc * FM_MAX_MODS),
                ("n_mods", i32), ("batch", i32), ("dim", i32), ("n_keep", i32), ("n_reg", i32), ("total_len", i32),
                ("is_decoder", i32), ("raw", i32),
                ("reg_tokens", vp), ("mask_token", vp),
                ("tokens", vp), ("emb", vp), ("x0", vp), ("out_mask", vp), ("out_mod", vp), ("slot_mod", vp),
                ("slot_src", vp), ("slot_pos", vp), ("target_ids", vp), ("out_cs", vp), ("out_mod_pre", vp),
                ("out_mod_index", vp), ("patch_rows", vp), ("seqemb_rows", vp), ("patch_ld", i32), ("seqemb_ld", i32),
                ("rows_f32", i32), ("pad2_", i32)]


class EmbedBwdMod(C.Structure):
    _fields_ = [("d_table", vp), ("d_pos", vp), ("d_mod_emb", vp), ("d_proj_bias", vp),
                ("kind", i32), ("has_padding_idx", i32), ("padding_idx", i32), ("pad_", i32)]


class EmbedBwdDesc(C.Structure):
    _fields_ = [("mods", EmbedBwdMod * FM_MAX_MODS), ("dx", vp), ("slot_mod", vp), ("slot_src", vp), ("slot_pos", vp),
                ("d_mask_token", vp), ("d_reg_tokens", vp),
                ("n_mods", i32), ("batch", i32), ("dim", i32), ("Nt", i32), ("lddx", i32), ("is_decoder", i32)]


def _sig(name, *argtypes):
    fn = getattr(lib, name)
    fn.argtypes = list(argtypes)
    fn.restype = C.c_int
    return fn


P = C.POINTER
gemm_nt = _sig("fm_gemm_nt", P(GemmNTArgs), vp)
gemm_tn = _sig("fm_gemm_tn", P(GemmTNArgs), vp)
gemm_tn_multi = _sig("fm_gemm_tn_multi", P(GemmTNJob), C.c_int, vp)
layernorm_fwd = _sig("fm_layernorm_fwd", vp, i32, vp, vp, vp, i32, i32, vp, vp, vp, i32, i32, f32, vp)
layernorm_fwd_res = _sig("fm_layernorm_fwd_res", vp, i32, vp, i32, vp, i32, vp, vp, vp, i32, i32, vp, vp, vp, i32, i32, f32, vp)
layernorm_bwd = _sig("fm_layernorm_bwd", vp, i32, vp, vp, i32, vp, vp, vp, vp, vp, i32, vp, i32, vp, vp, i32, i32, vp)
layernorm_bwd_h = _sig("fm_layernorm_bwd_h", vp, i32, vp, i32, vp, i32, vp, vp, vp, vp, vp, i32, vp, i32, vp, i32, i32, vp)
attn_fwd = _sig("fm_attn_fwd", P(AttnArgs), vp)
attn_bwd = _sig("fm_attn_bwd", P(AttnArgs), vp)
attn_decode = _sig("fm_attn_decode", P(AttnDecodeArgs), vp)
ATTN_DECODE_MAX_NK = 8192
select_embed = _sig("fm_select_embed", P(SelectDesc), vp)
embed_bwd = _sig("fm_embed_bwd", P(EmbedBwdDesc), vp)
dense_decoder_mask = _sig("fm_dense_decoder_mask", vp, vp, vp, i32, i32, i32, i32, i32, vp)
segment_rows = _sig("fm_segment_rows", vp, i32, i32, vp, vp, vp, vp, vp, i32, vp)
gather_rows = _sig("fm_gather_rows", vp, i32, vp, vp, i32, i32, i32, vp)
cross_entropy = _sig("fm_cross_entropy", vp, i32, vp, vp, vp, vp, vp, vp, vp, i32, i32, i32, i32, vp, vp, vp, vp, i32, vp)
swiglu_bwd = _sig("fm_swiglu_bwd", vp, i32, vp, i32, vp, i32, i32, i32, i32, vp)
gelu_bwd = _sig("fm_gelu_bwd", vp, i32, vp, i32, vp, i32, i32, i32, i32, vp)
cast_pad = _sig("fm_cast_pad", vp, i32, vp, i32, i32, i32, vp)
transpose_cast_pad = _sig("fm_transpose_cast_pad", vp, i32, vp, i32, i32, i32, i32, vp)
colsum = _sig("fm_colsum", vp, i32, vp, i32, i32, vp)
shadow_refresh = _sig("fm_shadow_refresh", vp, i32, i32, vp)
fold_colscale_grad = _sig("fm_fold_colscale_grad", vp, i32, vp)
headnorm_fwd = _sig("fm_headnorm_fwd", vp, i32, vp, vp, vp, i32, vp, i32, i32, C.c_float, vp)
headnorm_bwd = _sig("fm_headnorm_bwd", vp, i32, vp, i32, vp, vp, vp, i32, vp, vp, i32, i32, vp)
f32_to_bf16 = _sig("fm_f32_to_bf16", vp, vp, i64, vp)
bf16_to_f32_scaled = _sig("fm_bf16_to_f32_scaled", vp, vp, i64, f32, vp)
add_bf16_f32 = _sig("fm_add_bf16_f32", vp, vp, vp, i64, vp)
lib.fm_set_reserved_cus.argtypes = [C.c_int]
lib.fm_get_reserved_cus.restype = C.c_int
lib.fm_get_reserved_cus.argtypes = []
adamw = _sig("fm_adamw", vp, vp, vp, vp, i64, f32, f32, f32, f32, f32, i64, vp, vp, vp, vp)
adamw_shadow = _sig("fm_adamw_shadow", vp, i32, i32, f32, f32, f32, f32, f32, i64, vp, vp, vp, vp)
sumsq = _sig("fm_sumsq", vp, i64, vp, vp)
clip_coef = _sig("fm_clip_coef", vp, f32, vp, vp, vp)
sample_tokens = _sig("fm_sample_tokens", vp, i32, i32, i32, i32, f32, i32, f32, vp, vp, vp, vp)
maskgit_commit = _sig("fm_maskgit_commit", vp, vp, vp, i32, i32, i32, vp, i32, i32, vp, vp, vp, vp)
gemm_f32 = _sig("fm_gemm_f32", P(GemmF32Args), vp)
attn_f32_fwd = _sig("fm_attn_f32_fwd", P(AttnArgs), vp)
attn_f32_bwd = _sig("fm_attn_f32_bwd", P(AttnArgs), vp)
layernorm_bwd_f32 = _sig("fm_layernorm_bwd_f32", vp, i32, vp, vp, i32, vp, vp, vp, vp, vp, i32, vp, i32, vp, vp, i32, i32, vp)
headnorm_f32_fwd = _sig("fm_headnorm_f32_fwd", vp, i32, vp, vp, vp, i32, vp, i32, i32, C.c_float, vp)
headnorm_f32_bwd = _sig("fm_headnorm_f32_bwd", vp, i32, vp, i32, vp, vp, vp, i32, vp, vp, i32, i32, vp)
swiglu_bwd_f32 = _sig("fm_swiglu_bwd_f32", vp, i32, vp, i32, vp, i32, i32, i32, i32, vp)
gelu_bwd_f32 = _sig("fm_gelu_bwd_f32", vp, i32, vp, i32, vp, i32, i32, i32, vp)
colsum_f32 = _sig("fm_colsum_f32", vp, i32, vp, i32, i32, vp)
cross_entropy_f32 = _sig("fm_cross_entropy_f32", vp, i32, vp, vp, vp, vp, vp, vp, vp, i32, i32, i32, i32, vp, vp, vp, vp, i32, vp)
vq_patchify = _sig("fm_vq_patchify", vp, vp, i32, i32, i32, i32, i32, i32, vp)
l2norm_rows = _sig("fm_l2norm_rows", vp, i32, vp, i32, i32, i32, vp)
vq_assign = _sig("fm_vq_assign", vp, i32, vp, vp, i32, i32, i32, i32, i32, vp, vp, i32, vp, vp, vp)
lib.fm_set_tn_transpose_read.argtypes = [C.c_int]
lib.fm_set_gemm_tn_config.argtypes = [C.c_int]
lib.fm_set_attn_transpose_read.argtypes = [C.c_int]

lib.fm_set_gemm_nt_config.argtypes = [C.c_int]
lib.fm_lab_set.argtypes = [C.c_int, C.c_int]
lib.fm_lab_set.restype = None
vq_code_stats = _sig("fm_vq_code_stats", vp, i32, vp, i32, i32, i32, vp, vp, vp)
vq_ema_update = _sig("fm_vq_ema_update", vp, vp, vp, vp, i32, i32, f32, vp)
vq_code_bias = _sig("fm_vq_code_bias", vp, i32, i32, vp, vp)
vq_assign_bias = _sig("fm_vq_assign_bias", vp, i32, vp, vp, vp, i32, i32, i32, i32, i32, vp, vp, i32, vp, vp, vp)
vq_code_stats_raw = _sig("fm_vq_code_stats_raw", vp, i32, vp, i32, i32, i32, vp, vp, vp)
vq_ema_update_euclid = _sig("fm_vq_ema_update_euclid", vp, vp, vp, vp, vp, vp, i32, i32, f32, f32, vp)
vq_unpatchify = _sig("fm_vq_unpatchify", vp, i32, vp, i32, i32, i32, i32, i32, vp)
VQ_WIDE_TILE, CONVNEXT_MAX_C = 128, 4
vq_assign_wide = _sig("fm_vq_assign_wide", vp, i32, vp, vp, i32, i32, i32, i32, vp, vp, i32, vp, vp, vp)
memcodes_assign = _sig("fm_memcodes_assign", vp, i32, vp, vp, i32, i32, i32, i32, i32, vp, vp, i32, vp, vp, vp)
convnext_block = _sig("fm_convnext_block", vp, vp, vp, vp, vp, vp, vp, vp, vp, vp, vp, i32, i32, i32, i32, f32, vp)
vq_latent_grad = _sig("fm_vq_latent_grad", vp, i32, vp, vp, vp, i32, vp, f32, vp, i32, vp, i32, i32, vp)
tanh_bwd_f32 = _sig("fm_tanh_bwd_f32", vp, vp, vp, i32, i32, i32, vp)
embed_rows_f32 = _sig("fm_embed_rows_f32", vp, vp, vp, i32, i32, i32, vp)
vq_patchify_ex = _sig("fm_vq_patchify_ex", vp, vp, vp, vp, vp, vp, i32, i32, i32, i32, i32, i32, vp)
vq_cls_emb_bwd = _sig("fm_vq_cls_emb_bwd", vp, i32, vp, vp, i32, i32, i32, i32, i32, vp)
vq_latent_grad_normalized = _sig("fm_vq_latent_grad_normalized", vp, i32, vp, vp, vp, i32, vp, f32, vp, i32, vp, i32, i32, vp)
scale_rows_bf16 = _sig("fm_scale_rows_bf16", vp, i32, vp, i32, i32, i32, vp)
image_mask = _sig("fm_image_mask", vp, vp, vp, i32, i32, vp, vp, vp, vp)
token_budgets = _sig("fm_token_budgets", vp, vp, vp, vp, vp, vp, vp, i32, i32, i32, i32, vp, vp, vp)
span_mask = _sig("fm_span_mask", P(SpanMaskArgs), vp)
guidance_combine = _sig("fm_guidance_combine", vp, i32, i32, vp, i32, i32, f32, vp, i32, i32, i32, i32, vp)
unpack_image_u8 = _sig("fm_unpack_image_u8", vp, vp, i32, i32, i32, i32, P(C.c_float), P(C.c_float), vp)
unpack_ids_u16 = _sig("fm_unpack_ids_u16", vp, vp, i64, vp)
unpack_mask_bits = _sig("fm_unpack_mask_bits", vp, vp, i32, i32, vp)
decoder_attention_from_target = _sig("fm_decoder_attention_from_target", vp, vp, i32, i32, vp)
split3_bf16 = _sig("fm_split3_bf16", vp, i32, vp, i32, i32, i32, i32, i32, vp)
unet_im2col = _sig("fm_unet_im2col", vp, i32, i32, vp, i32, i32, i32, i32, vp, i32, i32, i32, i32, i32, i32, i32, i32, vp)
groupnorm_nhwc = _sig("fm_groupnorm_nhwc", vp, i32, vp, i32, vp, vp, vp, i32, vp, i32, i32, i32, i32, f32, i32, vp)
add_bf16 = _sig("fm_add_bf16", vp, i32, vp, i32, vp, i32, i64, i32, vp)
silu_f32_to_bf16 = _sig("fm_silu_f32_to_bf16", vp, vp, i64, vp)
timestep_embedding = _sig("fm_timestep_embedding", vp, vp, i32, i32, i32, f32, vp)
unet_attention = _sig("fm_unet_attention", vp, i32, vp, i32, i32, i32, i32, i32, vp)
unet_im2col_f32 = _sig("fm_unet_im2col_f32", vp, i32, i32, vp, i32, i32, i32, i32, vp, i32, i32, i32, i32, i32, i32, i32, i32, vp)
groupnorm_nhwc_f32 = _sig("fm_groupnorm_nhwc_f32", vp, i32, vp, i32, vp, vp, vp, i32, i32, i32, i32, i32, f32, i32, vp)
unet_attention_f32 = _sig("fm_unet_attention_f32", vp, i32, vp, i32, i32, i32, i32, i32, vp)
add_f32 = _sig("fm_add_f32", vp, i32, vp, i32, vp, i32, i64, i32, vp)
silu_f32 = _sig("fm_silu_f32", vp, vp, i64, vp)
timestep_embedding_f32 = _sig("fm_timestep_embedding_f32", vp, vp, i32, i32, i32, f32, vp)
unet_col2im_f32 = _sig("fm_unet_col2im_f32", vp, i32, vp, i32, i32, i32, i32, i32, i32, i32, i32, i32, vp)
groupnorm_nhwc_bwd_f32 = _sig("fm_groupnorm_nhwc_bwd_f32", vp, i32, vp, i32, vp, i32, vp, vp, vp, i32, vp, vp, vp, i32, vp, i32, i32, i32, i32, f32, i32, vp)
unet_attention_bwd_f32 = _sig("fm_unet_attention_bwd_f32", vp, i32, vp, i32, vp, i32, vp, i32, i32, i32, i32, vp)
silu_bwd_f32 = _sig("fm_silu_bwd_f32", vp, vp, vp, i64, vp)
diffusion_x0 = _sig("fm_diffusion_x0", vp, vp, f32, f32, vp, i64, vp)
quantile_abs = _sig("fm_quantile_abs", vp, i32, i64, f32, vp, vp)
diffusion_step = _sig("fm_diffusion_step", vp, vp, f32, f32, vp, vp, vp, f32, f32, f32, f32, vp, vp, i32, i64, vp)
lora_apply = _sig("fm_lora_apply", vp, i32, vp, i64, i64, vp, i64, i64, vp, i32, f32, vp, i32, i32, i32, i32, i32, i32, vp)
lora_grad = _sig("fm_lora_grad", vp, i32, vp, vp, i64, i64, f32, i32, i32, i32, i32, i32, vp)
vit_patch_rows = _sig("fm_vit_patch_rows", vp, vp, i32, i32, i32, i32, i32, i32, i32, vp)
vit_emb_rows = _sig("fm_vit_emb_rows", vp, vp, vp, i32, i32, i32, i32, vp)
vit_colsum = _sig("fm_vit_colsum", vp, i32, vp, i32, i32, vp, i64, vp)
EXPORTS = ["fm_attn_decode", "fm_vit_patch_rows", "fm_vit_emb_rows", "fm_vit_colsum", "fm_lora_apply", "fm_lora_grad", "fm_vq_assign_wide", "fm_memcodes_assign", "fm_convnext_block", "fm_split3_bf16", "fm_unet_im2col", "fm_groupnorm_nhwc", "fm_add_bf16", "fm_silu_f32_to_bf16", "fm_timestep_embedding", "fm_unet_attention", "fm_diffusion_x0", "fm_quantile_abs",
           "fm_diffusion_step", "fm_unpack_image_u8", "fm_unpack_ids_u16", "fm_unpack_mask_bits", "fm_decoder_attention_from_target", "fm_guidance_combine", "fm_image_mask", "fm_token_budgets", "fm_span_mask", "fm_vq_code_stats", "fm_vq_ema_update", "fm_vq_code_bias", "fm_vq_assign_bias", "fm_vq_code_stats_raw", "fm_vq_ema_update_euclid", "fm_vq_unpatchify", "fm_vq_latent_grad", "fm_tanh_bwd_f32", "fm_embed_rows_f32", "fm_vq_patchify_ex", "fm_vq_cls_emb_bwd", "fm_vq_latent_grad_normalized", "fm_abi_version", "fm_last_error", "fm_gemm_nt", "fm_set_gemm_nt_config", "fm_get_gemm_nt_config", "fm_set_reserved_cus", "fm_get_reserved_cus", "fm_bf16_to_f32_scaled", "fm_add_bf16_f32", "fm_scale_rows_bf16", "fm_gemm_tn", "fm_gemm_tn_multi", "fm_set_gemm_tn_config", "fm_get_gemm_tn_config", "fm_set_tn_transpose_read",
           "fm_get_tn_transpose_read", "fm_layernorm_fwd", "fm_layernorm_fwd_res", "fm_layernorm_bwd", "fm_layernorm_bwd_h", "fm_headnorm_fwd", "fm_headnorm_bwd", "fm_attn_fwd", "fm_attn_bwd",
           "fm_set_attn_transpose_read", "fm_get_attn_transpose_read", "fm_select_embed", "fm_embed_bwd",
           "fm_dense_decoder_mask", "fm_segment_rows", "fm_gather_rows", "fm_cross_entropy", "fm_swiglu_bwd",
           "fm_gelu_bwd", "fm_cast_pad", "fm_transpose_cast_pad", "fm_shadow_refresh", "fm_fold_colscale_grad", "fm_colsum", "fm_f32_to_bf16", "fm_adamw", "fm_adamw_shadow",
           "fm_sumsq", "fm_clip_coef", "fm_vq_patchify", "fm_l2norm_rows", "fm_vq_assign",
           "fm_sample_tokens", "fm_maskgit_commit", "fm_gemm_f32", "fm_attn_f32_fwd", "fm_attn_f32_bwd", "fm_layernorm_bwd_f32", "fm_headnorm_f32_fwd", "fm_headnorm_f32_bwd",
           "fm_swiglu_bwd_f32", "fm_gelu_bwd_f32", "fm_colsum_f32", "fm_cross_entropy_f32", "fm_lab_set",
           "fm_unet_im2col_f32", "fm_groupnorm_nhwc_f32", "fm_unet_attention_f32", "fm_add_f32", "fm_silu_f32", "fm_timestep_embedding_f32",
           "fm_unet_col2im_f32", "fm_groupnorm_nhwc_bwd_f32", "fm_unet_attention_bwd_f32", "fm_silu_bwd_f32"]


def check(rc: int):
    if rc != 0:
        raise RuntimeError(f"libfourm_hip: {lib.fm_last_error().decode()} (rc={rc})")
```

ml-4m_amd/fourm/hip/engine.py:

```python
import math
import os
import random
import weakref
from typing import Dict, List, Optional

import torch
import torch.nn as nn

from . import _lib as L
from . import ops

_WEIGHT_EPOCH = 0
FUSE_ACT_BWD = os.environ.get("FOURM_FUSE_ACT_BWD", "0") == "1"
HEADS_DENSE = os.environ.get("FOURM_HEADS_DENSE", "1") == "1"
HEADS_DENSE_MAX = int(os.environ.get("FOURM_HEADS_DENSE_MAX", "8"))
DEFER_RESIDUAL = os.environ.get("FOURM_DEFER_RESIDUAL", "1") == "1"
HOIST_CTX = os.environ.get("FOURM_HOIST_CTX", "1") == "1"
LN_BWD_FROM_H = os.environ.get("FOURM_LN_BWD_FROM_H", "1") == "1"
DP_RESERVE_ALWAYS = os.environ.get("FOURM_DP_RESERVE_ALWAYS", "0") == "1"


def bump_weight_epoch():
    global _WEIGHT_EPOCH
    _WEIGHT_EPOCH += 1


def ru(x, m):
    return (x + m - 1) // m * m


def is_lora(lin) -> bool:
    return hasattr(lin, "lora_down")


def check_lora_targets(model):
    from fourm.models.lora_utils import MAX_LORA_WIDTH, LoRAWrapper
    ok = set()
    for blk in model.encoder:
        ok |= {id(blk.attn.qkv), id(blk.attn.proj)}
    for blk in getattr(model, "decoder", ()):
        ok |= {id(blk.self_attn.qkv), id(blk.self_attn.proj), id(blk.cross_attn.q), id(blk.cross_attn.kv), id(blk.cross_attn.proj)}
    for name, mod in model.named_modules():
        if not isinstance(mod, LoRAWrapper):
            continue
        if id(mod) not in ok:
            raise NotImplementedError(f"LoRA wrapper at '{name}': the HIP engine adapts the attention Linears of the encoder / decoder blocks only "
                                      "(the MLP's fc1 / fc3 run as one launch whose SwiGLU epilogue consumes the pre-activation; embeddings and "
                                      "heads have no low-rank path)")
        width = mod.lora_down.weight.shape[0]
        if width > MAX_LORA_WIDTH:
            raise NotImplementedError(f"LoRA wrapper at '{name}': rank x packed Linears = {width} exceeds {MAX_LORA_WIDTH}")


class Shadow:
    __slots__ = ("buf", "params", "jobs", "stamp")

    def __init__(self, buf, params, jobs):
        self.buf, self.params, self.jobs, self.stamp = buf, params, jobs, None


class Workspace:

    def __init__(self, device, per_stream: bool = False):
        self.device = device
        self.per_stream = per_stream
        self.bufs: Dict[tuple, torch.Tensor] = {}

    def get(self, name, shape, dtype):
        key = (name, tuple(shape), dtype, torch.cuda.current_stream(self.device).cuda_stream) if self.per_stream else (name, tuple(shape), dtype)
        t = self.bufs.get(key)
        if t is None:
            t = self.bufs[key] = torch.zeros(shape, dtype=dtype, device=self.device)
        return t

    def nbytes(self):
        return sum(t.numel() * t.element_size() for t in self.bufs.values())


def fill_mod_desc(md, d, emb, is_dec: bool, mod_id: int, head_index: int = 0, raw: int = 0, name: str = "modality"):
    kind = emb.kind
    t = d["tensor"]
    B = t.shape[0]
    mask = d["target_mask" if is_dec else "input_mask"]
    mask = mask.reshape(B, -1)
    if mask.dtype != torch.bool:
        mask = mask.bool()
    mask = mask.contiguous()
    keep = [mask]
    md.mask, md.mask_stride = mask.data_ptr(), mask.shape[1]
    md.kind, md.mod_id, md.head_index = kind, mod_id, head_index
    md.pos = emb.pos_emb.data_ptr()
    md.mod_emb = emb.mod_emb.data_ptr()
    md.shifted = 1 if (is_dec and kind == L.KIND_SEQ and raw != 2) else 0
    md.max_len = getattr(emb, "max_length", 0) or 0
    if kind in (L.KIND_TOK, L.KIND_SEQ):
        ids = t.reshape(B, -1)
        if ids.dtype not in (torch.int32, torch.int64):
            ids = ids.long()
        ids = ids.contiguous()
        keep.append(ids)
        md.ids, md.ids_are_i64, md.id_stride = ids.data_ptr(), 1 if ids.dtype == torch.int64 else 0, ids.shape[1]
        md.table = emb.token_emb.weight.data_ptr()
        md.L = ids.shape[1] - (1 if md.shifted else 0)
        if ids.shape[1] != mask.shape[1]:
            raise ValueError(f"{name}: tensor has {ids.shape[1]} positions but the mask has {mask.shape[1]}")
    elif kind == L.KIND_PATCH:
        px = t.float().contiguous()
        keep.append(px)
        _, C, Hh, Ww = px.shape
        ps = emb.patch_size[0]
        md.ids, md.id_stride = px.data_ptr(), C * Hh * Ww
        md.patch, md.channels, md.grid_w = ps, C, Ww // ps
        md.L = (Hh // ps) * (Ww // ps)
    else:
        e = t.float().contiguous()
        keep.append(e)
        md.ids, md.id_stride, md.orig_dim = e.data_ptr(), e.shape[1] * e.shape[2], e.shape[2]
        md.proj_bias = emb.emb_proj.bias.data_ptr()
        md.L = e.shape[1]
    if is_dec and (raw != 2 or "decoder_attention_mask" in d):
        dam = d["decoder_attention_mask"].reshape(B, -1)
        if dam.dtype != torch.int32:
            dam = dam.int()
        dam = dam.contiguous()
        keep.append(dam)
        md.dam = dam.data_ptr()
    return keep


class FourMEngine:
    _pending = None
    _drop_now = None
    drop_uniforms = None

    def __init__(self, model):
        from fourm.models.fm_utils import GatedMlp, NormAttention, act_name
        self.model = model
        check_lora_targets(model)
        self.D = model.dim
        blk = model.encoder[0] if len(model.encoder) else model.decoder[0]
        attn0 = blk.attn if hasattr(blk, "attn") else blk.self_attn
        self.H = attn0.num_heads
        if self.D // self.H != 64:
            raise NotImplementedError(f"head_dim {self.D // self.H}: the HIP attention kernels are built for head_dim 64")
        self.qk_norm = isinstance(attn0, NormAttention)
        self.gated = isinstance(blk.mlp, GatedMlp)
        self.act = act_name(blk.mlp.act)
        if self.gated and self.act != "silu":
            raise NotImplementedError("gated MLP is implemented for SiLU (SwiGLU) only")
        if not self.gated and self.act != "gelu":
            raise NotImplementedError("plain MLP is implemented for exact GELU only")
        self.Hd = blk.mlp.hidden_features
        self.Hp = ru(self.Hd, 64)
        self.scale = 64 ** -0.5
        self.eps = blk.norm1.eps
        prec = getattr(model, "compute_precision", None) or os.environ.get("FOURM_PRECISION", "bf16")
        if prec not in ("bf16", "fp32"):
            raise ValueError(f"compute_precision {prec!r}: 'bf16' or 'fp32'")
        self.fp32 = prec == "fp32"
        self.adt = torch.float32 if self.fp32 else torch.bfloat16
        self.ws: Optional[Workspace] = None
        self.shadows: Dict[tuple, Shadow] = {}
        self._shadow_table = None
        self.flat_params = self.flat_grads = None
        self._slices = {}
        self._ctx = None
        self._dw_jobs = None
        self._pending = None
        self.reducer = None

    @property
    def checkpointing(self):
        return bool(getattr(self.model, "use_act_checkpoint", False))

    @property
    def device(self):
        t = getattr(self.model, "mask_token", None)
        return (t if t is not None else next(self.model.parameters())).device

    def _unique_params(self):
        seen, out = set(), []
        for n, p in getattr(self.model, "engine_parameters", self.model.named_parameters)():
            if id(p) not in seen:
                seen.add(id(p))
                out.append((n, p))
        return out

    def flatten(self):
        named = self._unique_params()
        dev = self.device

        def nodecay(n):
            return "norm." in n or ".norm" in n or n.endswith(".bias")
        late = {id(b.cross_attn.kv.weight) for b in self.model.decoder} if self.hoist_ctx else set()
        named.sort(key=lambda np_: (nodecay(np_[0]), id(np_[1]) in late))
        off, slices = 0, {}
        for n, p in named:
            slices[id(p)] = (off, p.numel())
            off += ru(p.numel(), 16)
        flat = torch.zeros(off, dtype=torch.float32, device=dev)
        for n, p in named:
            o, k = slices[id(p)]
            flat[o:o + k].copy_(p.data.reshape(-1))
            p.data = flat[o:o + k].view(p.shape)
        self.flat_params, self._slices = flat, slices
        self.flat_grads = torch.zeros_like(flat)
        self._named = named
        bump_weight_epoch()

    def _ensure_flat(self):
        if self.flat_params is None or self.flat_params.device != self.device:
            self.flatten()
            return
        for n, p in self._named[:4] + self._named[-4:]:
            o, k = self._slices[id(p)]
            if p.data_ptr() != self.flat_params.data_ptr() + 4 * o:
                self.flatten()
                return

    def grad_stages(self):
        m = self.model
        owner = {}

        def claim(stage, module_or_params):
            ps = module_or_params.parameters() if isinstance(module_or_params, nn.Module) else module_or_params
            for p in ps:
                owner[id(p)] = stage
        for i, blk in enumerate(m.decoder):
            claim(f"dec{i}", blk)
        if self.hoist_ctx:
            claim("dec_emb", [b.cross_attn.kv.weight for b in m.decoder] + [b.context_norm.weight for b in m.decoder])
        claim("heads", [m.decoder_norm.weight] + ([m.decoder_norm.bias] if isinstance(m.decoder_norm.bias, nn.Parameter) else []))
        claim("dec_emb", m.decoder_embeddings)
        claim("dec_emb", [m.mask_token])
        claim("ctx", m.decoder_proj_context)
        claim("ctx", m.encoder_norm)
        for i, blk in enumerate(m.encoder):
            claim(f"enc{i}", blk)
        claim("enc_emb", m.encoder_embeddings)
        if m.register_tokens is not None:
            claim("enc_emb", [m.register_tokens])
        stages = {}
        for n, p in self._named:
            o, k = self._slices[id(p)]
            stage = owner.get(id(p), "enc_emb") if k >= 65536 else "tail"
            stages.setdefault(stage, []).append((o, ru(k, 16)))
        return stages

    def _stage(self, name):
        if self.reducer is not None:
            self.reducer.stage_done(name)

    def grad_view(self, p):
        o, k = self._slices[id(p)]
        return self.flat_grads[o:o + k].view(p.shape)

    def grads_were_cleared(self) -> bool:
        live = getattr(self, "_attached", None)
        if not live:
            return True
        for p in live[:4] + live[-4:]:
            if p.grad is None or p.grad.data_ptr() != self.grad_view(p).data_ptr():
                return True
        return False

    def untouched_params(self):
        c = self._ctx
        if c is None or self.reducer is not None:
            return []
        m, touched, cand = self.model, set(), []
        for names, embs in ((c["enc"]["names"], m.encoder_embeddings), (c["dec"]["names"], m.decoder_embeddings)):
            for n, e in embs.items():
                if n in names:
                    touched.update(id(p) for p in e.parameters())
                else:
                    cand.extend(e.parameters())
        return [p for p in cand if id(p) not in touched]

    def attach_grads(self, zero: bool, untouched=()):
        if zero:
            with ops._prof("fills"):
                self.flat_grads.zero_()
            self._window_touched = set()
        skip = {id(p) for p in untouched} - getattr(self, "_window_touched", set())
        self._attached = []
        for n, p in self._named:
            if not p.requires_grad:
                continue
            if id(p) in skip:
                p.grad = None
                continue
            self._window_touched.add(id(p))
            p.grad = self.grad_view(p)
            self._attached.append(p)

    def _stamp(self, params):
        return tuple((p._version, _WEIGHT_EPOCH, p.data_ptr()) for p in params)

    def _get_shadow(self, key, make) -> torch.Tensor:
        s = self.shadows.get(key)
        if s is None:
            s = self.shadows[key] = make()
            for p in s.params:
                regs = getattr(p, "_fourm_shadows", None)
                if regs is None:
                    regs = p._fourm_shadows = []
                regs.append((weakref.ref(self), key))
        if s.stamp != self._stamp(s.params):
            self._refresh_shadows()
        return s.buf

    def _refresh_shadows(self):
        stale = [s for s in self.shadows.values() if s.stamp != self._stamp(s.params)]
        jobs = []
        for s in stale:
            jobs += [(j[0].detach().reshape(j[0].shape[0], -1), j[1], j[2], j[3].detach() if len(j) > 3 and j[3] is not None else None) for j in s.jobs]
        sig = tuple((a.data_ptr(), b.data_ptr(), tr, sc.data_ptr() if sc is not None else 0) for (a, b, tr, sc) in jobs)
        if self._shadow_table is None or self._shadow_table[0] != sig:
            table, tiles = ops.shadow_jobs_table(jobs, self.device)
            self._shadow_table = (sig, table, len(jobs), tiles)
        _, table, n, tiles = self._shadow_table
        ops.shadow_refresh(table, n, tiles)
        for s in stale:
            s.stamp = self._stamp(s.params)

    def mark_shadows_fresh(self, keys, written):
        for key in keys:
            s = self.shadows.get(key)
            if s is not None and all(len(j) == 3 and (id(j[0]), j[1].data_ptr()) in written for j in s.jobs):
                s.stamp = self._stamp(s.params)

    def w(self, p, pad_rows=False):
        if self.fp32:
            return p.detach().reshape(p.shape[0], -1)
        def make():
            out_f, in_f = p.shape[0], p[0].numel()
            buf = torch.zeros(ru(out_f, 64) if pad_rows else out_f, ru(in_f, 64), dtype=torch.bfloat16, device=p.device)
            return Shadow(buf, (p,), [(p, buf, False)])
        s = self._get_shadow(("w", id(p)), make)
        assert not pad_rows or s.shape[0] >= ru(p.shape[0], 64), "w(): the cached image was created without pad_rows"
        return s

    def wt(self, p, pad_rows=False):
        if self.fp32:
            return p.detach().reshape(p.shape[0], -1).t()
        def make():
            out_f, in_f = p.shape[0], p[0].numel()
            buf = torch.zeros(ru(in_f, 64) if pad_rows else in_f, ru(out_f, 64), dtype=torch.bfloat16, device=p.device)
            return Shadow(buf, (p,), [(p, buf, True)])
        s = self._get_shadow(("wt", id(p)), make)
        assert not pad_rows or s.shape[0] >= ru(p[0].numel(), 64), "wt(): the cached image was created without pad_rows"
        return s

    def w_fold(self, lin, norm):
        p, g = lin.weight, norm.weight
        def make():
            out_f, in_f = p.shape
            buf = torch.zeros(out_f, in_f if self.fp32 else ru(in_f, 64), dtype=self.adt, device=p.device)
            return Shadow(buf, (p, g), [(p, buf, False, g)])
        return self._get_shadow(("wfold", id(p)), make)

    def wt_fold_stack(self):
        m, D = self.model, self.D
        def make():
            Ld = len(m.decoder)
            buf = torch.zeros(D, Ld * 2 * D, dtype=self.adt, device=self.device)
            ps, jobs = [], []
            for i, blk in enumerate(m.decoder):
                p, g = blk.cross_attn.kv.weight, blk.context_norm.weight
                ps += [p, g]
                jobs.append((p, buf[:, i * 2 * D:(i + 1) * 2 * D], True, g))
            return Shadow(buf, tuple(ps), jobs)
        return self._get_shadow(("wtfold", 0), make)

    @property
    def hoist_ctx(self):
        h = getattr(self, "_hoist_ctx", None)
        if h is None:
            dec = getattr(self.model, "decoder", ())
            h = HOIST_CTX and len(dec) > 0 and all(
                not isinstance(b.context_norm.bias, nn.Parameter) and b.cross_attn.kv.bias is None and not is_lora(b.cross_attn.kv)
                for b in dec)
            self._hoist_ctx = h
        return h

    def w13t(self, mlp):
        def make():
            buf = torch.zeros(self.D, 2 * self.Hp, dtype=torch.bfloat16, device=self.device)
            p1, p3 = mlp.fc1.weight, mlp.fc3.weight
            return Shadow(buf, (p1, p3), [(p1, buf[:, :self.Hp], True), (p3, buf[:, self.Hp:], True)])
        return self._get_shadow(("w13t", id(mlp)), make)

    def _mod_desc(self, md: L.ModDesc, name, d, emb, is_dec, head_index=0, raw=0):
        return fill_mod_desc(md, d, emb, is_dec, int(self.model.modality_info[name]["id"]), head_index, raw, name)

    def select(self, mod_dict, n_keep: int, is_dec: bool, order: List[str], prefix: str, want_x0=True, heads=None, raw=0):
        m = self.model
        embs = m.decoder_embeddings if is_dec else m.encoder_embeddings
        names = [n for n in order if n in embs]
        if not names:
            raise ValueError("no modality of mod_dict is known to the model")
        if len(names) > L.FM_MAX_MODS:
            raise ValueError(f"{len(names)} modalities exceed FM_MAX_MODS={L.FM_MAX_MODS}")
# ... 216 lines not shown
        R, Rp, D = B * N, x_in.shape[0], self.D
        bf, f32 = self.adt, torch.float32
        dp = self._drop_scales(blk, B, 2, sv, dp)
        h1 = self._ln(blk.norm1, x_in, self._buf(sv, tag, "h1", (Rp, D), bf), R, sv, "n1", tag)
        x_mid = self._buf(sv, tag, "x_mid", (Rp, D), f32)
        self._drop_now = (dp[0], N) if dp else None
        self._self_attn_fwd(blk.attn, h1, x_in, x_mid, B, N, R, Rp, mask, sv, tag)
        h2 = self._ln(blk.norm2, x_mid, self._buf(sv, tag, "h2", (Rp, D), bf), R, sv, "n2", tag)
        x_out = self.ws.get(out_name or (tag + ".x_out" if sv is not None else "scratch.x_out" + tag[-1:]), (Rp, D), f32)
        self._drop_now = (dp[1], N) if dp else None
        self._mlp_fwd(blk.mlp, h2, x_mid, x_out, R, Rp, sv, tag, defer=defer_out)
        self._drop_now = None
        if sv is not None:
            sv["x_in"] = x_in
        return x_out

    def decoder_block_fwd(self, blk, y_in, ctx, B, M, N, sa_mask, xa_mask, sv, tag, defer_out=False, out_name=None, dp=None, ctx_hat=None):
        Rq, Rqp, Rc, Rcp, D = B * M, y_in.shape[0], B * N, ctx.shape[0], self.D
        bf, f32 = self.adt, torch.float32
        dp = self._drop_scales(blk, B, 3, sv, dp)
        h1 = self._ln(blk.norm1, y_in, self._buf(sv, tag, "h1", (Rqp, D), bf), Rq, sv, "n1", tag)
        y1 = self._buf(sv, tag, "y1", (Rqp, D), f32)
        self._drop_now = (dp[0], M) if dp else None
        self._self_attn_fwd(blk.self_attn, h1, y_in, y1, B, M, Rq, Rqp, sa_mask, sv, tag)
        self._drop_now = (dp[1], M) if dp else None
        hq = self._ln(blk.query_norm, y1, self._buf(sv, tag, "hq", (Rqp, D), bf), Rq, sv, "nq", tag)
        if ctx_hat is None:
            hc, w_kv = self._ln(blk.context_norm, ctx, self._buf(sv, tag, "hc", (Rcp, D), bf), Rc, sv, "nc", tag), None
        else:
            hc, w_kv = ctx_hat, self.w_fold(blk.cross_attn.kv, blk.context_norm)
        y2 = self._buf(sv, tag, "y2", (Rqp, D), f32)
        self._cross_attn_fwd(blk.cross_attn, hq, hc, y1, y2, B, M, N, Rq, Rqp, Rc, Rcp, xa_mask, sv, tag, w_kv=w_kv)
        h2 = self._ln(blk.norm2, y2, self._buf(sv, tag, "h2", (Rqp, D), bf), Rq, sv, "n2", tag)
        y_out = self.ws.get(out_name or (tag + ".y_out" if sv is not None else "scratch.y_out" + tag[-1:]), (Rqp, D), f32)
        self._drop_now = (dp[2], M) if dp else None
        self._mlp_fwd(blk.mlp, h2, y2, y_out, Rq, Rqp, sv, tag, defer=defer_out)
        self._drop_now = None
        if sv is not None:
            sv["y_in"] = y_in
        return y_out

    def prepare(self):
        if self.ws is None or self.ws.device != self.device:
            self.ws = Workspace(self.device)

    @staticmethod
    def keypad(mask_u8):
        return dict(mask_kind=L.MASK_KEYPAD, kpad=mask_u8)

    def decoder_mask(self, cs, mod_pre):
        m = self.model
        return dict(mask_kind=L.MASK_DECODER, cs=None if m.decoder_causal_mask else cs, causal=m.decoder_causal_mask,
                    modq=mod_pre if m.decoder_sep_mask else None, modk=mod_pre if m.decoder_sep_mask else None)

    def encode_context(self, enc, st=None):
        m = self.model
        save = st is not None
        B, N = enc["B"], enc["Nt"]
        emask = self.keypad(enc["mask"])
        x = enc["x0"]
        ckpt = save and self.checkpointing
        for i, blk in enumerate(m.encoder):
            if ckpt:
                st["enc_layers"].append(dict(ckpt_in=x))
                x = self.encoder_block_fwd(blk, x, B, N, emask, None, f"enc{i % 2}", defer_out=True, out_name=f"enc{i}.x_out")
                st["enc_layers"][-1]["dp"] = self._last_dp
                continue
            sv = {} if save else None
            x = self.encoder_block_fwd(blk, x, B, N, emask, sv, f"enc{i}" if save else f"enc{i % 2}", defer_out=True)
            if save:
                st["enc_layers"].append(sv)
        R, Rp, D = B * N, x.shape[0], self.D
        sv_top = {} if save else None
        xn = self._ln(m.encoder_norm, x, self._buf(sv_top, "top", "xn", (Rp, D), self.adt), R, sv_top, "en", "top")
        ctx = self._buf(sv_top, "top", "ctx", (Rp, D), torch.float32)
        pc = m.decoder_proj_context
        ops.gemm_nt(xn, self.w(pc.weight), ctx, epilogue=L.EPI_RESIDUAL, res=enc["emb"], bias=pc.bias, M=R, N=D, K=D)
        return x, ctx, emask, sv_top

    def trunk_forward(self, enc, dec, save: bool):
        m = self.model
        B, N, Mt = enc["B"], enc["Nt"], dec["Nt"]
        st = dict(enc_layers=[], dec_layers=[]) if save else None
        x, ctx, emask, sv_top = self.encode_context(enc, st)
        y = dec["x0"]
        smask = self.decoder_mask(dec["cs"], dec["mod_pre"]) if "cs" in dec else dec["sa_mask"]
        ctx_hat, sv_hat = None, None
        if self.hoist_ctx:
            sv_hat = {} if save else None
            ctx_hat = self._ln(self._unit_norm(), ctx, self._buf(sv_hat, "top", "ctx_hat", (ctx.shape[0], self.D), self.adt), B * N, sv_hat, "ch", "top")
        for i, blk in enumerate(m.decoder):
            if save and self.checkpointing:
                st["dec_layers"].append(dict(ckpt_in=y))
                y = self.decoder_block_fwd(blk, y, ctx, B, Mt, N, smask, emask, None, f"dec{i % 2}", defer_out=i + 1 < len(m.decoder),
                                           out_name=f"dec{i}.y_out", ctx_hat=ctx_hat)
                st["dec_layers"][-1]["dp"] = self._last_dp
                continue
            sv = {} if save else None
            y = self.decoder_block_fwd(blk, y, ctx, B, Mt, N, smask, emask, sv, f"dec{i}" if save else f"dec{i % 2}",
                                       defer_out=i + 1 < len(m.decoder), ctx_hat=ctx_hat)
            if save:
                st["dec_layers"].append(sv)
        if save:
            st.update(top=sv_top, x_final=x, y_final=y, ctx=ctx, emask=emask, smask=smask, ctx_hat=ctx_hat, sv_hat=sv_hat)
        return y, st

    def heads_setup(self, dec, y_final, save):
        m = self.model
        heads = dec["heads"]
        nH = len(heads)
        B, Mt, D = dec["B"], dec["Nt"], self.D
        R = B * Mt
        Rp = ops.padded_rows(R, nH)
        ws, dev, i32 = self.ws, self.device, torch.int32
        hs = dict(n=nH, Rp=Rp, heads=heads)
        hs["seg_start"], hs["seg_count"] = ws.get("heads.seg_start", (nH,), i32), ws.get("heads.seg_count", (nH,), i32)
        hs["perm"], hs["r2p"] = ws.get("heads.perm", (Rp,), i32), ws.get("heads.r2p", (R,), i32)
        hs["tile_group"] = ws.get("heads.tile_group", (Rp // ops.SEG,), i32)
        ops.segment_rows(dec["head_of_row"].view(-1), nH, hs["seg_start"], hs["seg_count"], hs["perm"], hs["r2p"], hs["tile_group"])
        sv = {} if save else None
        yp = ws.get("heads.yp", (Rp, D), self.adt)
        with ops._prof("fills"):
            yp.zero_()
        self._ln(m.decoder_norm, y_final, yp, R, sv, "dn", "heads", row_map=hs["r2p"])
        vocabs = [m.decoder_embeddings[h].vocab_size for h in heads]
        hs["vocabs"], hs["maxV"] = vocabs, max(vocabs)
        ldl = ru(hs["maxV"], 64)
        w_fwd = [self.w(m.decoder_embeddings[h].to_logits.weight) for h in heads]
        w_bwd = [self.wt(m.decoder_embeddings[h].to_logits.weight) for h in heads] if save else None
        key = tuple(t.data_ptr() for t in w_fwd) + (tuple(t.data_ptr() for t in w_bwd) if save else ())
        cache = getattr(self, "_head_groups", None)
        if cache is None or cache[0] != key:
            fwd = ops.make_groups([dict(W=t, N=v, K=D, ldw=D) for t, v in zip(w_fwd, vocabs)], dev)
            if self.fp32:
                bwd = ops.make_groups([dict(W=m.decoder_embeddings[h].to_logits.weight, N=D, K=v, ldw=D, transposed=1)
                                       for h, v in zip(heads, vocabs)], dev) if save else None
            else:
                bwd = ops.make_groups([dict(W=t, N=D, K=ru(v, 64), ldw=ru(v, 64)) for t, v in zip(w_bwd, vocabs)], dev) if save else None
            vt = torch.tensor(vocabs, dtype=i32, device=dev)
            self._head_groups = cache = (key, fwd, bwd, vt)
        hs["g_fwd"], hs["g_bwd"], hs["vocab_t"] = cache[1], cache[2], cache[3]
        logits = ws.get("heads.logits", (Rp, ldl), self.adt)
        if HEADS_DENSE and not self.fp32 and nH <= HEADS_DENSE_MAX and ops.heads_dense_ok(w_fwd, vocabs, logits):
            ops.gemm_nt_heads(yp, w_fwd, vocabs, hs["seg_start"], hs["seg_count"], logits, D)
        else:
            ops.gemm_nt_grouped(yp, hs["g_fwd"], hs["tile_group"], logits, hs["maxV"], max_K=D)
        hs.update(yp=yp, logits=logits, sv=sv)
        hs["row_loss"] = ws.get("heads.row_loss", (Rp,), torch.float32)
        hs["row_lse"] = ws.get("heads.row_lse", (Rp,), torch.float32)
        hs["head_loss"] = ws.get("heads.head_loss", (nH,), torch.float32)
        hs["total"] = ws.get("heads.total", (1,), torch.float32)
        return hs

    def loss_forward(self, dec, hs, loss_type):
        lt = L.LOSS_MOD if loss_type in ("mod", "modality") else L.LOSS_TOKEN
        hs["loss_type"] = lt
        ops.cross_entropy(hs["logits"], hs["perm"], hs["tile_group"], dec["target_ids"].view(-1), hs["vocab_t"], hs["seg_start"],
                          hs["seg_count"], hs["n"], hs["maxV"], hs["row_loss"], hs["row_lse"], hs["head_loss"], hs["total"], loss_type=lt)
        return hs["total"], hs["head_loss"]

    def dec_order(self, mod_dict):
        names = [n for n in mod_dict if n in self.model.decoder_embeddings]
        return random.sample(names, len(names))

    def train_forward(self, mod_dict, n_enc, n_dec, loss_type, save=True):
        if loss_type not in ("mod", "modality", "token"):
            raise ValueError("Invalid loss type")
        self.prepare()
        if save:
            self._ensure_flat()
        enc_names = [n for n in mod_dict if n in self.model.encoder_embeddings]
        enc = self.select(mod_dict, n_enc, False, enc_names, "enc.")
        dec = self.select(mod_dict, n_dec, True, self.dec_order(mod_dict), "dec.")
        y, st = self.trunk_forward(enc, dec, save)
        hs = self.heads_setup(dec, y, save)
        total, head_loss = self.loss_forward(dec, hs, loss_type)
        if save:
            self._ctx = dict(enc=enc, dec=dec, st=st, hs=hs)
        return total, head_loss, hs["heads"], hs["seg_count"]

    def _g(self, p):
        return self.grad_view(p) if p.requires_grad else None

    def _dW(self, dy, x, lin, R64, n_cols=None, dy_cols=None):
        g = self._g(lin.weight)
        N = lin.weight.shape[0] if n_cols is None else n_cols
        if g is not None:
            if self._dw_jobs is not None:
                self._dw_jobs.append((dy, x, g.view(g.shape[0], -1), N, lin.weight[0].numel(), R64))
            else:
                ops.gemm_tn(dy, x, g.view(g.shape[0], -1), N=N, K=lin.weight[0].numel(), R=R64)
        if lin.bias is not None and lin.bias.requires_grad:
            ops.colsum(dy, self.grad_view(lin.bias), N, R=R64)

    def _flush_dW(self):
        jobs, self._dw_jobs = self._dw_jobs, None
        ops.gemm_tn_multi(jobs)

    def _ln_bwd(self, norm, dy, x, sv, key, g, g_bf, R, dres, dy_row_map=None):
        dw = self._g(norm.weight)
        db = self._g(norm.bias) if isinstance(norm.bias, nn.Parameter) else None
        ops.layernorm_bwd(dy, x, norm.weight, sv[key + ".mu"], sv[key + ".rs"], g, dres=dres, dx_bf16=g_bf, dw=dw, db=db,
                          dy_row_map=dy_row_map, R=R, h=sv.get(key + ".h"))

    def _mlp_bwd(self, mlp, sv, g_bf, R, Rp):
        bf, D, Hp, Hd = self.adt, self.D, self.Hp, self.Hd
        R64 = R
        ws = self.ws
        self._dW(g_bf, sv["act"], mlp.fc2, R64)
        dh = ws.get("bwd.dh", (Rp, D), bf)
        fuse = FUSE_ACT_BWD
        if not fuse:
            da = ws.get("bwd.da", (Rp, Hp), bf)
            padN = not self.fp32 and Hp != Hd
            ops.gemm_nt(g_bf, self.wt(mlp.fc2.weight, padN), da, M=R, N=Hp if padN else Hd, K=D)
        if self.gated:
            dgu = ws.get("bwd.dgu", (Rp, 2 * Hp), bf)
            if fuse:
                ops.gemm_nt(g_bf, self.wt(mlp.fc2.weight), dgu, M=R, N=Hd, K=D, epilogue=L.EPI_SWIGLU_BWD, res=sv["gu"], Hp=Hp)
            else:
                ops.swiglu_bwd(da, sv["gu"], dgu, Hd, Hp, R=R)
            self._dW(dgu[:, :Hp], sv["h2"], mlp.fc1, R64, n_cols=Hd)
            self._dW(dgu[:, Hp:], sv["h2"], mlp.fc3, R64, n_cols=Hd)
            if self.fp32:
                ops.gemm_nt(dgu[:, :Hp], self.wt(mlp.fc1.weight), dh, M=R, N=D, K=Hd)
                ops.gemm_nt(dgu[:, Hp:], self.wt(mlp.fc3.weight), dh, M=R, N=D, K=Hd, epilogue=L.EPI_F32, res=dh)
            else:
                ops.gemm_nt(dgu, self.w13t(mlp), dh, M=R, N=D, K=2 * Hp)
        else:
            dpre = ws.get("bwd.dpre", (Rp, Hp), bf)
            if fuse:
                ops.gemm_nt(g_bf, self.wt(mlp.fc2.weight), dpre, M=R, N=Hd, K=D, epilogue=L.EPI_GELU_BWD, res=sv["pre"])
            else:
                ops.gelu_bwd(da, sv["pre"], dpre, Hd, Hp, R=R)
            self._dW(dpre, sv["h2"], mlp.fc1, R64, n_cols=Hd)
            ops.gemm_nt(dpre, self.wt(mlp.fc1.weight), dh, M=R, N=D, K=Hp)
        return dh

    def _self_attn_bwd(self, attn, sv, g_bf, B, N, R, Rp, mask):
        bf, D = self.adt, self.D
        R64, ws = R, self.ws
        self._dW(g_bf, sv["o"], attn.proj, R64)
        do = ws.get("bwd.do", (Rp, D), bf)
        ops.gemm_nt(g_bf, self.wt(attn.proj.weight), do, M=R, N=D, K=D)
        self._lora_bwd(attn.proj, g_bf, sv["o"], do, sv.get("lora.proj"), R)
        dqkv = ws.get("bwd.dqkv", (Rp, 3 * D), bf)
        qkv = sv["qkv"]
        if self.qk_norm:
            dqkn = ws.get("bwd.dqkn", (Rp, 2 * D), bf)
            ops.attn_bwd(sv["qkn.q"], sv["qkn.k"], qkv[:, 2 * D:], sv["o"], do, dqkn[:, :D], dqkn[:, D:], dqkv[:, 2 * D:],
                         B, self.H, N, N, self.scale, sv["sm"], sv["sl"], zero_attn=getattr(attn, "allow_zero_attn", False), **mask)
            self._qk_norm_bwd(attn, sv, "qkn", dqkn[:, :D], dqkn[:, D:], qkv[:, :D], qkv[:, D:2 * D], dqkv[:, :D], dqkv[:, D:2 * D], R, R)
        else:
            ops.attn_bwd(qkv[:, :D], qkv[:, D:2 * D], qkv[:, 2 * D:], sv["o"], do, dqkv[:, :D], dqkv[:, D:2 * D], dqkv[:, 2 * D:],
                         B, self.H, N, N, self.scale, sv["sm"], sv["sl"], zero_attn=getattr(attn, "allow_zero_attn", False), **mask)
        self._dW(dqkv, sv["h1"], attn.qkv, R64)
        dh = ws.get("bwd.dh", (Rp, D), bf)
        ops.gemm_nt(dqkv, self.wt(attn.qkv.weight), dh, M=R, N=D, K=3 * D)
        self._lora_bwd(attn.qkv, dqkv, sv["h1"], dh, sv.get("lora.qkv"), R)
        return dh

    def encoder_block_bwd(self, blk, sv, g, g_bf, B, N, mask):
        R, Rp = B * N, g.shape[0]
        self._dw_jobs = []
        dp = sv.get("dp")
        if dp:
            ops.scale_rows_bf16(g_bf, dp[1], N, R)
        dh = self._mlp_bwd(blk.mlp, sv, g_bf, R, Rp)
        g1 = self.ws.get("bwd.enc.gbf1", tuple(g_bf.shape), g_bf.dtype)
        self._ln_bwd(blk.norm2, dh, sv["x_mid"], sv, "n2", g, g1, R, dres=g)
        if dp:
            ops.scale_rows_bf16(g1, dp[0], N, R)
        dh = self._self_attn_bwd(blk.attn, sv, g1, B, N, R, Rp, mask)
        self._flush_dW()
        self._ln_bwd(blk.norm1, dh, sv["x_in"], sv, "n1", g, g_bf, R, dres=g)

    def decoder_block_bwd(self, blk, sv, g, g_bf, dctx, dctx_bf, ctx, B, M, N, sa_mask, xa_mask, hoist=None):
        bf, D = self.adt, self.D
        Rq, Rqp, Rc, Rcp = B * M, g.shape[0], B * N, ctx.shape[0]
        ws = self.ws
        self._dw_jobs = []
        g_in = g_bf
        dp = sv.get("dp")
        if dp:
            ops.scale_rows_bf16(g_in, dp[2], M, Rq)
        dh = self._mlp_bwd(blk.mlp, sv, g_in, Rq, Rqp)
        g_bf = ws.get("bwd.dec.gbf1", tuple(g_in.shape), g_in.dtype)
        self._ln_bwd(blk.norm2, dh, sv["y2"], sv, "n2", g, g_bf, Rq, dres=g)
        if dp:
            ops.scale_rows_bf16(g_bf, dp[1], M, Rq)
        xa = blk.cross_attn
        self._dW(g_bf, sv["o2"], xa.proj, Rq)
        do = ws.get("bwd.do", (Rqp, D), bf)
        ops.gemm_nt(g_bf, self.wt(xa.proj.weight), do, M=Rq, N=D, K=D)
        self._lora_bwd(xa.proj, g_bf, sv["o2"], do, sv.get("lora.proj2"), Rq)
        dq = ws.get("bwd.dq", (Rqp, D), bf)
        dkv = ws.get("bwd.dkv", (Rcp, 2 * D), bf) if hoist is None else hoist[0]
        kv = sv["kv"]
        if self.qk_norm:
            dqn = ws.get("bwd.dqn", (Rqp, D), bf)
            dkn = ws.get("bwd.dkn", (Rcp, D), bf)
            ops.attn_bwd(sv["xqkn.q"], sv["xqkn.k"], kv[:, D:], sv["o2"], do, dqn, dkn, dkv[:, D:], B, self.H, M, N, self.scale,
                         sv["sm2"], sv["sl2"], zero_attn=getattr(xa, "allow_zero_attn", False), **xa_mask)
            self._qk_norm_bwd(xa, sv, "xqkn", dqn, dkn, sv["q"], kv[:, :D], dq, dkv[:, :D], Rq, Rc)
        else:
            ops.attn_bwd(sv["q"], kv[:, :D], kv[:, D:], sv["o2"], do, dq, dkv[:, :D], dkv[:, D:], B, self.H, M, N, self.scale,
                         sv["sm2"], sv["sl2"], zero_attn=getattr(xa, "allow_zero_attn", False), **xa_mask)
        self._dW(dq, sv["hq"], xa.q, Rq)
        dhq = ws.get("bwd.dh", (Rqp, D), bf)
        ops.gemm_nt(dq, self.wt(xa.q.weight), dhq, M=Rq, N=D, K=D)
        self._lora_bwd(xa.q, dq, sv["hq"], dhq, sv.get("lora.q"), Rq)
        g_bf = ws.get("bwd.dec.gbf2", tuple(g_in.shape), g_in.dtype)
        self._ln_bwd(blk.query_norm, dhq, sv["y1"], sv, "nq", g, g_bf, Rq, dres=g)
        if dp:
            ops.scale_rows_bf16(g_bf, dp[0], M, Rq)
        if hoist is None:
            self._dW(dkv, sv["hc"], xa.kv, Rc)
            dhc = ws.get("bwd.dhc", (Rcp, D), bf)
            ops.gemm_nt(dkv, self.wt(xa.kv.weight), dhc, M=Rc, N=D, K=2 * D)
            self._lora_bwd(xa.kv, dkv, sv["hc"], dhc, sv.get("lora.kv"), Rc)
            self._ln_bwd(blk.context_norm, dhc, ctx, sv, "nc", dctx, dctx_bf, Rc, dres=dctx)
        elif xa.kv.weight.requires_grad or blk.context_norm.weight.requires_grad:
            self._dw_jobs.append((dkv, hoist[1], hoist[2], 2 * D, D, Rc))
        dh = self._self_attn_bwd(blk.self_attn, sv, g_bf, B, M, Rq, Rqp, sa_mask)
        self._flush_dW()
        self._ln_bwd(blk.norm1, dh, sv["y_in"], sv, "n1", g, g_in, Rq, dres=g)

    def _embed_bwd(self, sel, dx, dx_extra, is_dec):
        m = self.model
        embs = m.decoder_embeddings if is_dec else m.encoder_embeddings
        d = L.EmbedBwdDesc()
        for i, n in enumerate(sel["names"]):
            e, md = embs[n], d.mods[i]
            md.kind = e.kind
            if e.kind in (L.KIND_TOK, L.KIND_SEQ) and not (is_dec and e.kind == L.KIND_TOK):
                w = e.token_emb.weight
                md.d_table = self.grad_view(w).data_ptr() if w.requires_grad else None
                pad = e.token_emb.padding_idx
                md.has_padding_idx, md.padding_idx = (1, pad) if pad is not None else (0, 0)
            if isinstance(e.pos_emb, nn.Parameter) and e.pos_emb.requires_grad:
                md.d_pos = self.grad_view(e.pos_emb).data_ptr()
            if e.mod_emb.requires_grad:
                md.d_mod_emb = self.grad_view(e.mod_emb).data_ptr()
            if e.kind == L.KIND_SEQ_EMB and e.emb_proj.bias.requires_grad:
                md.d_proj_bias = self.grad_view(e.emb_proj.bias).data_ptr()
        d.dx, d.lddx = dx.data_ptr(), dx.stride(0)
        d.slot_mod, d.slot_src, d.slot_pos = sel["slot_mod"].data_ptr(), sel["slot_src"].data_ptr(), sel["slot_pos"].data_ptr()
        if is_dec and m.mask_token.requires_grad:
            d.d_mask_token = self.grad_view(m.mask_token).data_ptr()
        if not is_dec and m.num_register_tokens and m.register_tokens.requires_grad:
            d.d_reg_tokens = self.grad_view(m.register_tokens).data_ptr()
        d.n_mods, d.batch, d.dim, d.Nt, d.is_decoder = len(sel["names"]), sel["B"], self.D, sel["Nt"], 1 if is_dec else 0
        with ops._prof("embed_bwd"):
            L.check(L.embed_bwd(ops.C.byref(d), ops._stream()))
        if dx_extra is not None:
            d2 = L.EmbedBwdDesc()
            ops.C.memmove(ops.C.byref(d2), ops.C.byref(d), ops.C.sizeof(d))
            for i in range(d.n_mods):
                d2.mods[i].d_table = None
                d2.mods[i].d_proj_bias = None
            d2.d_reg_tokens = None
            d2.dx, d2.lddx = dx_extra.data_ptr(), dx_extra.stride(0)
            with ops._prof("embed_bwd"):
                L.check(L.embed_bwd(ops.C.byref(d2), ops._stream()))

    def train_backward(self, grad_scale: torch.Tensor):
        c = self._ctx
        if c is None:
            raise RuntimeError("train_backward without a preceding training forward")
        self._ctx, self._dw_jobs = None, None
        if self.reducer is not None:
            self.reducer.begin()
            if getattr(self.reducer, "reserved_cus", 0):
                L.lib.fm_set_reserved_cus(int(self.reducer.reserved_cus))
        m, ws = self.model, self.ws
        enc, dec, st, hs = c["enc"], c["dec"], c["st"], c["hs"]
        B, N, Mt, D = enc["B"], enc["Nt"], dec["Nt"], self.D
        bf, f32 = self.adt, torch.float32
        Rq, Rc = B * Mt, B * N
        Rqp, Rcp = st["y_final"].shape[0], st["x_final"].shape[0]
        ops.cross_entropy(hs["logits"], hs["perm"], hs["tile_group"], dec["target_ids"].view(-1), hs["vocab_t"], hs["seg_start"],
                          hs["seg_count"], hs["n"], hs["maxV"], hs["row_loss"], hs["row_lse"], hs["head_loss"], hs["total"],
                          loss_type=hs["loss_type"], grad_scale=grad_scale, write_grad=True)
        dyp = ws.get("bwd.dyp", (hs["Rp"], D), bf)
        ops.gemm_nt_grouped(hs["logits"], hs["g_bwd"], hs["tile_group"], dyp, D, max_K=ru(hs["maxV"], 64))
        heads = [m.decoder_embeddings[h] for h in hs["heads"]]
        if any(h.to_logits.weight.requires_grad for h in heads):
            outs = [self.grad_view(h.to_logits.weight) if h.to_logits.weight.requires_grad else None for h in heads]
            key = tuple(o.data_ptr() if o is not None else 0 for o in outs)
            cache = getattr(self, "_head_tn_groups", None)
            if cache is None or cache[0] != key:
                cache = self._head_tn_groups = (key, ops.make_groups(
                    [dict(out=o, N=(v if o is not None else 0)) for o, v in zip(outs, hs["vocabs"])], self.device))
            tn = cache[1]
            ops.gemm_tn_grouped(hs["logits"], hs["yp"], tn, hs["seg_start"], hs["seg_count"], hs["n"], hs["maxV"], hs["Rp"], D)
        g = ws.get("bwd.g_dec", (Rqp, D), f32)
        g_bf = ws.get("bwd.g_dec_bf", (Rqp, D), bf)
        self._ln_bwd(m.decoder_norm, dyp, st["y_final"], hs["sv"], "dn", g, g_bf, Rq, dres=None, dy_row_map=hs["r2p"])
        self._stage("heads")
        dctx = ws.get("bwd.dctx", (Rcp, D), f32)
        dctx_bf = ws.get("bwd.dctx_bf", (Rcp, D), bf)
        Ld = len(m.decoder)
        ctx_hat = st.get("ctx_hat")
        if ctx_hat is None:
            with ops._prof("fills"):
                dctx.zero_()
        else:
            dkv_all = ws.get("bwd.dkv_all", (Rcp, Ld * 2 * D), bf)
            dwp = ws.get("bwd.dwp", (Ld, 2 * D, D), f32)
            with ops._prof("fills"):
                dwp.zero_()
        for i in reversed(range(Ld)):
            sv = st["dec_layers"][i]
            if "ckpt_in" in sv:
                y_in, dp, sv = sv["ckpt_in"], sv["dp"], {}
                self.decoder_block_fwd(m.decoder[i], y_in, st["ctx"], B, Mt, N, st["smask"], st["emask"], sv, "ckpt", out_name="ckpt.out", dp=dp,
                                       ctx_hat=ctx_hat)
            hoist = None if ctx_hat is None else (dkv_all[:, i * 2 * D:(i + 1) * 2 * D], ctx_hat, dwp[i])
            self.decoder_block_bwd(m.decoder[i], sv, g, g_bf, dctx, dctx_bf, st["ctx"], B, Mt, N, st["smask"], st["emask"], hoist=hoist)
            self._stage(f"dec{i}")
        if ctx_hat is not None and Ld:
            dxh = ws.get("bwd.dhc", (Rcp, D), bf)
            ops.gemm_nt(dkv_all, self.wt_fold_stack(), dxh, M=Rc, N=D, K=Ld * 2 * D)
            self._ln_bwd(self._unit_norm(), dxh, st["ctx"], st["sv_hat"], "ch", dctx, dctx_bf, Rc, dres=None)
            jobs = [(dwp[i], b.cross_attn.kv.weight.detach(), b.context_norm.weight.detach(), self._g(b.cross_attn.kv.weight), self._g(b.context_norm.weight))
                    for i, b in enumerate(m.decoder) if b.cross_attn.kv.weight.requires_grad or b.context_norm.weight.requires_grad]
            if jobs:
                ops.fold_colscale_grad(jobs)
        self._embed_bwd(dec, g, None, True)
        self._stage("dec_emb")
        top = st["top"]
        if len(m.decoder) == 0:
            ops.f32_to_bf16(dctx, dctx_bf)
        self._dW(dctx_bf, top["xn"], m.decoder_proj_context, Rc)
        dxn = ws.get("bwd.dh", (Rcp, D), bf)
        ops.gemm_nt(dctx_bf, self.wt(m.decoder_proj_context.weight), dxn, M=Rc, N=D, K=D)
        ge = ws.get("bwd.g_enc", (Rcp, D), f32)
        ge_bf = ws.get("bwd.g_enc_bf", (Rcp, D), bf)
        self._ln_bwd(m.encoder_norm, dxn, st["x_final"], top, "en", ge, ge_bf, Rc, dres=None)
        self._stage("ctx")
        for i in reversed(range(len(m.encoder))):
            sv = st["enc_layers"][i]
            if "ckpt_in" in sv:
                x_in, dp, sv = sv["ckpt_in"], sv["dp"], {}
                self.encoder_block_fwd(m.encoder[i], x_in, B, N, st["emask"], sv, "ckpt", out_name="ckpt.out", dp=dp)
            self.encoder_block_bwd(m.encoder[i], sv, ge, ge_bf, B, N, st["emask"])
            self._stage(f"enc{i}")
        for n in enc["names"]:
            e = m.encoder_embeddings[n]
            if e.kind == L.KIND_PATCH and e.proj.weight.requires_grad:
                ops.gemm_tn(ge_bf, enc["patch_rows"], self.grad_view(e.proj.weight), N=D, K=e.proj.weight.shape[1], R=Rc)
            elif e.kind == L.KIND_SEQ_EMB and e.emb_proj.weight.requires_grad:
                ops.gemm_tn(ge_bf, enc["seqemb_rows"], self.grad_view(e.emb_proj.weight), N=D, K=e.emb_proj.weight.shape[1], R=Rc)
        self._embed_bwd(enc, ge, dctx, False)
        if self.reducer is not None:
            self.reducer.finish()
            if getattr(self.reducer, "reserved_cus", 0) and not DP_RESERVE_ALWAYS:
                L.lib.fm_set_reserved_cus(0)
```

ml-4m_amd/fourm/hip/ops.py:

```python
import contextlib
import ctypes as C
import threading
from typing import Optional

import torch

from . import _lib as L

_PROFILER = None


def set_profiler(p):
    global _PROFILER
    _PROFILER = p


class _Null:
    def __enter__(self):
        return self

    def __exit__(self, *a):
        return False


# ... 122 lines not shown
def gemm_nt_grouped(x, groups, tile_group, out, max_N, M=None, max_K=0):
    if x.dtype == torch.float32:
        a = L.GemmF32Args()
        a.X, a.out, a.groups, a.tile_group = _p(x), _p(out), _p(groups), _p(tile_group)
        a.M, a.N, a.max_N, a.seg_rows = (x.shape[0] if M is None else M), max_N, max_N, SEG
        a.sxm, a.sxk, a.ldo, a.epilogue = x.stride(0), 1, out.stride(0), L.EPI_BF16
        L.check(L.gemm_f32(C.byref(a), _stream()))
        return out
    a = L.GemmNTArgs()
    a.X, a.out = _p(x), _p(out)
    a.M = x.shape[0] if M is None else M
    a.K = max_K
    a.ldx, a.ldo = _ld(x), _ld(out)
    a.epilogue = L.EPI_BF16
    a.groups, a.tile_group, a.max_N = _p(groups), _p(tile_group), max_N
    L.check(L.gemm_nt(C.byref(a), _stream()))
    return out


def heads_dense_ok(ws, vocabs, out):
    return (out.dtype == torch.bfloat16 and all(v % 8 == 0 for v in vocabs) and all(w.dtype == torch.bfloat16 and w.shape[1] % 64 == 0 for w in ws)
            and _ld(out) % 64 == 0 and out.data_ptr() % 128 == 0)


@_timed("heads_gemm_nt (logits, dY)")
def gemm_nt_heads(x, ws, vocabs, seg_start, seg_count, out, K):
    for h, (w, v) in enumerate(zip(ws, vocabs)):
        a = L.GemmNTArgs()
        a.W, a.X, a.out = _p(w), _p(x), _p(out)
        a.M, a.N, a.K = x.shape[0], v, K
        a.ldw, a.ldx, a.ldo = _ld(w), _ld(x), _ld(out)
        a.epilogue = L.EPI_BF16
        a.m_dev, a.row0_dev = seg_count.data_ptr() + 4 * h, seg_start.data_ptr() + 4 * h
        L.check(L.gemm_nt(C.byref(a), _stream()))
    return out


def gemm_tn(a_mat, b_mat, out, *, N=None, K=None, R=None, splits=0, force_tr=-1, a_cols=0, b_cols=0):
    if a_mat.dtype == torch.float32:
        g = L.GemmF32Args()
        g.X, g.W, g.out = _p(a_mat), _p(b_mat), _p(out)
        g.M = a_mat.shape[1] if N is None else N
        g.N = b_mat.shape[1] if K is None else K
        g.K = a_mat.shape[0] if R is None else R
        g.sxm, g.sxk, g.swn, g.swk = 1, a_mat.stride(0), 1, b_mat.stride(0)
        g.ldo, g.epilogue, g.accumulate = _ld(out), L.EPI_BF16, 1
        L.check(L.gemm_f32(C.byref(g), _stream()))
        return out
    a = L.GemmTNArgs()
    a.A, a.B, a.out = _p(a_mat), _p(b_mat), _p(out)
    a.R = a_mat.shape[0] if R is None else R
    a.N = a_mat.shape[1] if N is None else N
    a.K = b_mat.shape[1] if K is None else K
    a.lda, a.ldb, a.ldo = _ld(a_mat), _ld(b_mat), _ld(out)
    a.a_cols = a_cols or a_mat.shape[1]
    a.b_cols = b_cols or b_mat.shape[1]
    a.splits, a.force_tr = splits, force_tr
    with _prof("gemm_tn", 2.0 * a.R * a.N * a.K, 2.0 * a.R * (a.N + a.K) + 4.0 * a.N * a.K, tag=f"R{a.R} N{a.N} K{a.K}"):
        L.check(L.gemm_tn(C.byref(a), _stream()))
    return out


def gemm_tn_multi(jobs):
    if not jobs:
        return
    if jobs[0][0].dtype == torch.float32:
        for a_mat, b_mat, out, N, K, R in jobs:
            gemm_tn(a_mat, b_mat, out, N=N, K=K, R=R)
        return
    for lo in range(0, len(jobs), L.TN_MAX_JOBS):
        part = jobs[lo:lo + L.TN_MAX_JOBS]
        arr = (L.GemmTNJob * len(part))()
        flops = 0.0
        for j, (a_mat, b_mat, out, N, K, R) in zip(arr, part):
            j.A, j.B, j.out = _p(a_mat), _p(b_mat), _p(out)
            j.R, j.N, j.K = R, N, K
            j.lda, j.ldb, j.ldo = _ld(a_mat), _ld(b_mat), _ld(out)
            j.a_cols, j.b_cols = a_mat.shape[1], b_mat.shape[1]
            flops += 2.0 * R * N * K
        with _prof("gemm_tn_multi", flops, 0.0, tag=f"jobs{len(part)} R{part[0][5]}"):
            L.check(L.gemm_tn_multi(arr, len(part), _stream()))


@_timed("heads_gemm_tn (dW)")
def gemm_tn_grouped(a_mat, b_mat, groups, seg_start, seg_count, n_groups, max_N, max_R, K, *, splits=0, force_tr=-1):
    if a_mat.dtype == torch.float32:
        g = L.GemmF32Args()
        g.X, g.W, g.groups, g.seg_start, g.seg_count = _p(a_mat), _p(b_mat), _p(groups), _p(seg_start), _p(seg_count)
        g.N, g.max_N, g.n_groups = K, max_N, n_groups
        g.sxm, g.sxk, g.swn, g.swk = 1, a_mat.stride(0), 1, b_mat.stride(0)
        g.ldo, g.epilogue, g.accumulate = K, L.EPI_BF16, 1
        L.check(L.gemm_f32(C.byref(g), _stream()))
        return
    a = L.GemmTNArgs()
    a.A, a.B = _p(a_mat), _p(b_mat)
    a.K = K
    a.lda, a.ldb, a.ldo = _ld(a_mat), _ld(b_mat), K
    a.a_cols, a.b_cols = a_mat.shape[1], b_mat.shape[1]
    a.splits, a.force_tr = splits, force_tr
    a.groups, a.seg_start, a.seg_count = _p(groups), _p(seg_start), _p(seg_count)
    a.n_groups, a.max_N, a.max_R = n_groups, max_N, max_R
    L.check(L.gemm_tn(C.byref(a), _stream()))


def make_groups(entries, device):
    arr = (L.GemmGroup * len(entries))()
    for i, e in enumerate(entries):
        arr[i].W = e["W"].data_ptr() if e.get("W") is not None else None
        arr[i].out = e["out"].data_ptr() if e.get("out") is not None else None
        arr[i].N, arr[i].K, arr[i].ldw = e["N"], e.get("K", 0), e.get("ldw", 0)
        arr[i].pad_ = e.get("transposed", 0)
    host = torch.frombuffer(bytearray(bytes(arr)), dtype=torch.uint8)
    return host.to(device)


def layernorm_fwd(x, w, b, y, mean=None, rstd=None, row_map=None, eps=1e-6, R=None, delta=None, x_out=None):
    R = x.shape[0] if R is None else R
    if delta is not None:
        with _prof("layernorm_fwd", 0.0, R * w.numel() * (10 + y.element_size())):
            L.check(L.layernorm_fwd_res(_p(x), _ld(x), _p(delta), _ld(delta), _p(x_out), _ld(x_out), _p(w), _p(b), _p(y), _ld(y),
                                        1 if y.dtype == torch.float32 else 0, _p(mean), _p(rstd), _p(row_map), R, w.numel(), eps, _stream()))
        return y
    with _prof("layernorm_fwd", 0.0, R * w.numel() * (4 + y.element_size())):
        return _ln_fwd(x, w, b, y, mean, rstd, row_map, eps, R)


def _ln_fwd(x, w, b, y, mean, rstd, row_map, eps, R):
    L.check(L.layernorm_fwd(_p(x), _ld(x), _p(w), _p(b), _p(y), _ld(y), 1 if y.dtype == torch.float32 else 0,
                            _p(mean), _p(rstd), _p(row_map), R, w.numel(), eps, _stream()))
    return y


def layernorm_bwd(dy, x, w, mean, rstd, dx, *, dres=None, dx_bf16=None, dw=None, db=None, dy_row_map=None, R=None, h=None):
    R = x.shape[0] if R is None else R
    if h is not None and dy.dtype != torch.float32 and db is None and dy_row_map is None:
        with _prof("layernorm_bwd", 0.0, R * w.numel() * (2 + 2 + 4 + 4 + (2 if dx_bf16 is not None else 0))):
            L.check(L.layernorm_bwd_h(_p(dy), _ld(dy), _p(h), _ld(h), _p(x), _ld(x), _p(w), _p(mean), _p(rstd), _p(dres), _p(dx), _ld(dx),
                                      _p(dx_bf16), _ld(dx_bf16) if dx_bf16 is not None else 0, _p(dw), R, w.numel(), _stream()))
        return dx
    with _prof("layernorm_bwd", 0.0, R * w.numel() * (2 + 4 + 4 + 4 + (2 if dx_bf16 is not None else 0))):
        return _ln_bwd(dy, x, w, mean, rstd, dx, dres, dx_bf16, dw, db, dy_row_map, R)


def _ln_bwd(dy, x, w, mean, rstd, dx, dres, dx_bf16, dw, db, dy_row_map, R):
    if dy.dtype == torch.float32:
        L.check(L.layernorm_bwd_f32(_p(dy), _ld(dy), _p(dy_row_map), _p(x), _ld(x), _p(w), _p(mean), _p(rstd), _p(dres), _p(dx), _ld(dx),
                                    _p(dx_bf16), _ld(dx_bf16) if dx_bf16 is not None else 0, _p(dw), _p(db), R, w.numel(), _stream()))
        return dx
    L.check(L.layernorm_bwd(_p(dy), _ld(dy), _p(dy_row_map), _p(x), _ld(x), _p(w), _p(mean), _p(rstd), _p(dres), _p(dx), _ld(dx),
                            _p(dx_bf16), _ld(dx_bf16) if dx_bf16 is not None else 0, _p(dw), _p(db), R, w.numel(), _stream()))
    return dx


@_timed("headnorm")
def headnorm_fwd(x, w, b, y, stats, R, H, eps):
    if x.dtype == torch.float32:
        return L.check(L.headnorm_f32_fwd(_p(x), _ld(x), _p(w), _p(b), _p(y), _ld(y), _p(stats), R, H, eps, _stream()))
    L.check(L.headnorm_fwd(_p(x), _ld(x), _p(w), _p(b), _p(y), _ld(y), _p(stats), R, H, eps, _stream()))


@_timed("headnorm")
def headnorm_bwd(dy, x, w, stats, dx, dw, db, R, H):
    if x.dtype == torch.float32:
        return L.check(L.headnorm_f32_bwd(_p(dy), _ld(dy), _p(x), _ld(x), _p(w), _p(stats), _p(dx), _ld(dx), _p(dw), _p(db), R, H, _stream()))
    L.check(L.headnorm_bwd(_p(dy), _ld(dy), _p(x), _ld(x), _p(w), _p(stats), _p(dx), _ld(dx), _p(dw), _p(db), R, H, _stream()))


def _attn_args(q, k, v, o, B, H, Nq, Nk, scale, mask_kind, kpad, cs, modq, modk, dense, causal, stat_m, stat_l, force_tr, zero_attn=False):
    a = L.AttnArgs()
    a.Q, a.K, a.V, a.O = _p(q), _p(k), _p(v), _p(o)
    a.ldq, a.ldk, a.ldv, a.ldo = q.stride(0), k.stride(0), v.stride(0), o.stride(0)
    a.B, a.H, a.Nq, a.Nk, a.head_dim, a.mask_kind = B, H, Nq, Nk, 64, mask_kind
    a.scale, a.causal = scale, 1 if causal else 0
    a.kpad, a.cs, a.modq, a.modk, a.dense = _p(kpad), _p(cs), _p(modq), _p(modk), _p(dense)
    a.stat_m, a.stat_l = _p(stat_m), _p(stat_l)
    a.force_tr, a.zero_attn = force_tr, 1 if zero_attn else 0
    return a


def attn_fwd(q, k, v, o, B, H, Nq, Nk, scale, *, mask_kind=L.MASK_NONE, kpad=None, cs=None, modq=None, modk=None, dense=None,
             causal=False, stat_m=None, stat_l=None, force_tr=-1, kv_batch_rows=0, zero_attn=False):
    a = _attn_args(q, k, v, o, B, H, Nq, Nk, scale, mask_kind, kpad, cs, modq, modk, dense, causal, stat_m, stat_l, force_tr, zero_attn)
    a.kv_batch_rows = kv_batch_rows
    if q.dtype == torch.float32:
        L.check(L.attn_f32_fwd(C.byref(a), _stream()))
        return o
    with _prof("attn_fwd", 4.0 * B * H * Nq * Nk * 64):
        L.check(L.attn_fwd(C.byref(a), _stream()))
    return o


@_timed("attn_decode")
def attn_decode(q, k, v, o, B, H, Nk, scale, *, kv_batch_rows=0, k_new_row=-1, q_norm=None, k_norm=None, eps=1e-6, kpad=None, zero_attn=False):
    a = L.AttnDecodeArgs()
    a.q, a.k, a.v, a.o = _p(q), _p(k), _p(v), _p(o)
    if not (q.dtype == k.dtype == v.dtype == o.dtype) or q.dtype not in (torch.bfloat16, torch.float32):
        raise TypeError("attn_decode: q, k, v, o must share one of bf16 / fp32")
    for w in (q_norm or ()) + (k_norm or ()):
        if w is not None and (w.dtype != torch.float32 or w.numel() != 64 or not w.is_contiguous()):
            raise TypeError("attn_decode: norm vectors are contiguous fp32 (64)")
    a.q_w, a.q_b = (_p(q_norm[0]), _p(q_norm[1])) if q_norm is not None else (None, None)
    a.k_w, a.k_b = (_p(k_norm[0]), _p(k_norm[1])) if k_norm is not None else (None, None)
    if kpad is not None and (kpad.dtype not in (torch.bool, torch.uint8) or kpad.shape != (B, Nk) or not kpad.is_contiguous()):
        raise TypeError("attn_decode: kpad is a contiguous (B, Nk) bool / uint8 tensor")
    a.kpad = _p(kpad)
    a.ldq, a.ldk, a.ldv, a.ldo = _ld(q), _ld(k), _ld(v), _ld(o)
    a.B, a.H, a.Nk, a.kv_batch_rows, a.k_new_row = B, H, Nk, kv_batch_rows, k_new_row
    a.is_f32, a.zero_attn, a.scale, a.eps = int(q.dtype == torch.float32), 1 if zero_attn else 0, scale, eps
    L.check(L.attn_decode(C.byref(a), _stream()))
    return o


def attn_bwd(q, k, v, o, do, dq, dk, dv, B, H, Nq, Nk, scale, stat_m, stat_l, *, mask_kind=L.MASK_NONE, kpad=None, cs=None,
             modq=None, modk=None, dense=None, causal=False, force_tr=-1, zero_attn=False):
    a = _attn_args(q, k, v, o, B, H, Nq, Nk, scale, mask_kind, kpad, cs, modq, modk, dense, causal, stat_m, stat_l, force_tr, zero_attn)
    a.dO, a.dQ, a.dK, a.dV = _p(do), _p(dq), _p(dk), _p(dv)
    a.lddo, a.lddq, a.lddk, a.lddv = do.stride(0), dq.stride(0), dk.stride(0), dv.stride(0)
    if q.dtype == torch.float32:
        dk.zero_(); dv.zero_()
        L.check(L.attn_f32_bwd(C.byref(a), _stream()))
        return
    with _prof("attn_bwd", 10.0 * B * H * Nq * Nk * 64):
        L.check(L.attn_bwd(C.byref(a), _stream()))


def padded_rows(R: int, n_heads: int) -> int:
    return ru(R, SEG) + SEG * (n_heads - 1)


@_timed("heads_misc")
def segment_rows(head_of_row, n_heads, seg_start, seg_count, perm, row_to_padded, tile_group):
    L.check(L.segment_rows(_p(head_of_row), head_of_row.numel(), n_heads, _p(seg_start), _p(seg_count), _p(perm),
                           _p(row_to_padded), _p(tile_group), perm.numel(), _stream()))


@_timed("heads_misc")
def gather_rows(src, perm, dst, D):
    L.check(L.gather_rows(_p(src), _ld(src), _p(perm), _p(dst), _ld(dst), perm.numel(), D, _stream()))


@_timed("cross_entropy")
def cross_entropy(logits, perm, tile_group, target_ids, vocab, seg_start, seg_count, n_heads, max_vocab, row_loss, row_lse, head_loss,
                  total_loss, *, loss_type=L.LOSS_MOD, grad_scale=None, write_grad=False):
    fn = L.cross_entropy_f32 if logits.dtype == torch.float32 else L.cross_entropy
    L.check(fn(_p(logits), _ld(logits), _p(perm), _p(tile_group), _p(target_ids), _p(vocab), _p(seg_start),
                            _p(seg_count), _p(grad_scale), loss_type, n_heads, perm.numel(), max_vocab, _p(row_loss), _p(row_lse),
                            _p(head_loss), _p(total_loss), 1 if write_grad else 0, _stream()))


@_timed("swiglu_bwd")
def swiglu_bwd(da, gu, dgu, H, Hp, R=None):
    if da.dtype == torch.float32:
        return L.check(L.swiglu_bwd_f32(_p(da), _ld(da), _p(gu), _ld(gu), _p(dgu), _ld(dgu), da.shape[0] if R is None else R, H, Hp, _stream()))
    L.check(L.swiglu_bwd(_p(da), _ld(da), _p(gu), _ld(gu), _p(dgu), _ld(dgu), da.shape[0] if R is None else R, H, Hp, _stream()))


@_timed("gelu_bwd")
def gelu_bwd(dh, pre, dpre, H, Hp, R=None):
    if dh.dtype == torch.float32:
        return L.check(L.gelu_bwd_f32(_p(dh), _ld(dh), _p(pre), _ld(pre), _p(dpre), _ld(dpre), dh.shape[0] if R is None else R, H, _stream()))
    L.check(L.gelu_bwd(_p(dh), _ld(dh), _p(pre), _ld(pre), _p(dpre), _ld(dpre), dh.shape[0] if R is None else R, H, Hp, _stream()))


def cast_pad(src, dst):
    s2 = src.reshape(src.shape[0], -1)
    L.check(L.cast_pad(_p(s2), s2.stride(0), _p(dst), _ld(dst), s2.shape[0], s2.shape[1], _stream()))
    return dst


def transpose_cast_pad(src, dst):
    s2 = src.reshape(src.shape[0], -1)
    L.check(L.transpose_cast_pad(_p(s2), s2.stride(0), _p(dst), _ld(dst), dst.shape[1], s2.shape[0], s2.shape[1], _stream()))
    return dst


def shadow_jobs_table(jobs, device):
    arr = (L.ShadowDesc * len(jobs))()
    tiles = 0
    for i, job in enumerate(jobs):
        src, dst, tr = job[:3]
        scale = job[3] if len(job) > 3 else None
        rows, cols = src.shape
        need = (cols, rows) if tr else (rows, cols)
        assert src.dtype == torch.float32 and dst.dtype in (torch.bfloat16, torch.float32) and src.stride(1) == 1 and dst.stride(1) == 1
        assert dst.shape[0] >= need[0] and dst.shape[1] >= need[1], (tuple(dst.shape), need)
        d = arr[i]
        d.src, d.dst, d.ld_src, d.ld_dst = src.data_ptr(), dst.data_ptr(), src.stride(0), dst.stride(0)
        d.rows, d.cols, d.transpose, d.tile_start = rows, cols, 1 if tr else 0, tiles
        d.dst_f32 = 1 if dst.dtype == torch.float32 else 0
        if scale is not None:
            assert scale.dtype == torch.float32 and scale.numel() == cols and scale.is_contiguous()
            d.col_scale = scale.data_ptr()
        tiles += ((rows + 63) // 64) * ((cols + 63) // 64)
    raw = torch.frombuffer(bytearray(bytes(arr)), dtype=torch.uint8).to(device)
    return raw, tiles


@_timed("fold_colscale_grad")
def fold_colscale_grad(jobs):
    for lo in range(0, len(jobs), L.FOLD_MAX_JOBS):
        part = jobs[lo:lo + L.FOLD_MAX_JOBS]
        arr = (L.FoldGradJob * len(part))()
        for j, (dwp, w, gamma, gw, gg) in zip(arr, part):
            rows, cols = w.shape[0], w[0].numel()
            assert w.is_contiguous() and (gw is None or gw.is_contiguous()) and dwp.stride(1) == 1
            j.dWp, j.W, j.gamma, j.gW, j.ggamma = _p(dwp), _p(w), _p(gamma), _p(gw), _p(gg)
            j.rows, j.cols, j.ld_dwp = rows, cols, dwp.stride(0)
        L.check(L.fold_colscale_grad(arr, len(part), _stream()))


@_timed("shadow_refresh")
def shadow_refresh(table, n_jobs, tiles):
    L.check(L.shadow_refresh(_p(table), n_jobs, tiles, _stream()))


@_timed("colsum")
def colsum(dy, db, N, R=None):
    if dy.dtype == torch.float32:
        return L.check(L.colsum_f32(_p(dy), _ld(dy), _p(db), dy.shape[0] if R is None else R, N, _stream()))
    L.check(L.colsum(_p(dy), _ld(dy), _p(db), dy.shape[0] if R is None else R, N, _stream()))


@_timed("casts")
def f32_to_bf16(src, dst):
    if dst.dtype == torch.float32:
        return dst.copy_(src)
    L.check(L.f32_to_bf16(_p(src), _p(dst), src.numel(), _stream()))
    return dst


@_timed("casts")
def bf16_to_f32_scaled(src, dst, scale=1.0):
    L.check(L.bf16_to_f32_scaled(_p(src), _p(dst), src.numel(), float(scale), _stream()))
    return dst


@_timed("drop_path")
def scale_rows_bf16(x, scale, rows_per_sample, R, N=None):
    L.check(L.scale_rows_bf16(_p(x), _ld(x), _p(scale), rows_per_sample, R, x.shape[1] if N is None else N, _stream()))
    return x


@_timed("casts")
def add_bf16_to_f32(x, delta, out, R=None):
    R = x.shape[0] if R is None else R
    assert x.is_contiguous() and delta.is_contiguous() and out.is_contiguous() and x.shape[1] == delta.shape[1] == out.shape[1]
    L.check(L.add_bf16_f32(_p(x), _p(delta), _p(out), R * x.shape[1], _stream()))
    return out


@_timed("adamw")
def adamw(p, g, m, v, n, lr, beta1, beta2, eps, wd, step, grad_mult=None, hyper=None, sumsq=None):
    L.check(L.adamw(_p(p), _p(g), _p(m), _p(v), n, lr, beta1, beta2, eps, wd, step, _p(grad_mult), _p(hyper), _p(sumsq), _stream()))


ADAMW_CHUNK = 8192


def adamw_jobs_table(jobs, device):
    arr = (L.AdamWJob * len(jobs))()
    tiles = 0
    for i, j in enumerate(jobs):
        p = j["p"]
        rows, cols = p.shape[0], p[0].numel()
        d = arr[i]
        for k in ("p", "g", "m", "v"):
            t = j[k]
            assert t.dtype == torch.float32 and t.is_contiguous() and t.numel() == rows * cols, (k, t.dtype, tuple(t.shape))
            setattr(d, k, t.data_ptr())
        pl, tr = j.get("plain"), j.get("t")
        if pl is not None:
            assert pl.dtype == torch.bfloat16 and pl.stride(1) == 1 and pl.shape[0] >= rows and pl.shape[1] >= cols
            d.dst_plain, d.ld_plain = pl.data_ptr(), pl.stride(0)
        assert tr is None, "transposed shadows are refreshed by fm_shadow_refresh"
        d.rows, d.cols, d.tile_start = rows, cols, tiles
        tiles += (rows * cols + ADAMW_CHUNK - 1) // ADAMW_CHUNK
    raw = torch.frombuffer(bytearray(bytes(arr)), dtype=torch.uint8).to(device)
    return raw, tiles


@_timed("adamw")
def adamw_shadow(table, n_jobs, tiles, lr, beta1, beta2, eps, wd, step, grad_mult=None, hyper=None, sumsq=None):
    L.check(L.adamw_shadow(_p(table), n_jobs, tiles, lr, beta1, beta2, eps, wd, step, _p(grad_mult), _p(hyper), _p(sumsq), _stream()))


@_timed("grad_norm")
def sumsq(x, out):
    L.check(L.sumsq(_p(x), x.numel(), _p(out), _stream()))


@_timed("grad_norm")
def clip_coef(ss, max_norm, norm_out, coef_out):
    L.check(L.clip_coef(_p(ss), float(max_norm or 0.0), _p(norm_out), _p(coef_out), _stream()))


def dense_decoder_mask(cs, mod, B, M, causal, use_sep):
    out = torch.empty(B, M, M, dtype=torch.bool, device=(cs if cs is not None else mod).device)
    L.check(L.dense_decoder_mask(_p(cs), _p(mod), _p(out), B, M, 1 if causal else 0, 1 if cs is not None else 0,
                                 1 if use_sep else 0, _stream()))
    return out
# ... 60 lines not shown
```

Before: 1.192 million tokens/s.

## Replace LayerNorm backward atomics with batched partial reduce and fuse CE grad into forward

LayerNorm backward now writes per-block weight and bias gradient partials into a ring buffer instead of issuing atomic adds. A single batched reduce kernel sums them into the gradient buffers, flushed at reducer stages and at the end of backward. Separately, the training forward cross-entropy computes the loss and writes the unscaled softmax gradient in one pass over register-held logits, so backward only applies a scale pass instead of rereading and recomputing the softmax. This removes atomic contention and one logits pass, at the cost of extra partial buffer traffic and more kernels.

Measured after the change: 1.200 million tokens/s, median of 6. About the same (+0.7%).

```diff
diff --git a/include/fourm_hip.h b/include/fourm_hip.h
--- a/include/fourm_hip.h
+++ b/include/fourm_hip.h
@@ -72,6 +72,16 @@
 int fm_layernorm_bwd_h(const void* dy, int lddy, const void* h, int ldh, const void* x, int ldx, const void* w,
                        const void* mean, const void* rstd, const void* dres, void* dx, int lddx, void* dx_bf16,
                        int lddxbf, void* dw, int R, int D, void* stream);
+int fm_ln_bwd_blocks(int R);
+int fm_layernorm_bwd_partials(const void* dy, int lddy, const int32_t* dy_row_map, const void* h, int ldh, const void* x, int ldx,
+                              const void* w, const void* mean, const void* rstd, const void* dres, void* dx, int lddx,
+                              void* dx_bf16, int lddxbf, void* part_w, void* part_b, int R, int D, void* stream);
+#define FM_LN_REDUCE_MAX_JOBS 64
+typedef struct fm_ln_reduce_job {
+    const void* partials; void* dst;
+    int32_t n_blocks, D, first, reserved;
+} fm_ln_reduce_job;
+int fm_ln_dw_reduce(const fm_ln_reduce_job* jobs, int n_jobs, void* stream);
 
 int fm_headnorm_fwd(const void* x, int ldx, const void* w, const void* b, void* y, int ldy, void* stats, int R, int H, float eps,
                     void* stream);
@@ -189,6 +199,9 @@
 int fm_segment_rows(const int32_t* head_of_row, int R, int n_heads, int32_t* seg_start, int32_t* seg_count,
                     int32_t* perm, int32_t* row_to_padded, int32_t* tile_group, int Rp, void* stream);
 int fm_gather_rows(const void* src, int ld_src, const int32_t* perm, void* dst, int ld_dst, int Rp, int D, void* stream);
+#define FM_CE_FUSED 2
+#define FM_CE_SCALE 3
+#define FM_CE_FUSED_MAX_VOCAB 32768
 int fm_cross_entropy(void* logits, int ldl, const int32_t* perm, const int32_t* tile_group, const int64_t* target_ids,
                      const int32_t* vocab, const int32_t* seg_start, const int32_t* seg_count, const void* grad_scale,
                      int loss_type, int n_heads, int Rp, int max_vocab, void* row_loss, void* row_lse, void* head_loss,
diff --git a/ml-4m_amd/csrc/layernorm.hip b/ml-4m_amd/csrc/layernorm.hip
--- a/ml-4m_amd/csrc/layernorm.hip
+++ b/ml-4m_amd/csrc/layernorm.hip
@@ -130,7 +130,8 @@
                                                      const float* __restrict__ x, int ldx, const float* __restrict__ w,
                                                      const float* __restrict__ mean, const float* __restrict__ rstd,
                                                      const float* dres, float* dx, int lddx, bf16_t* __restrict__ dx_bf, int lddxbf,
-                                                     float* __restrict__ dw, float* __restrict__ db, int R, int D, int BWD_ROWS, int nt_dx) {
+                                                     float* __restrict__ dw, float* __restrict__ db, int R, int D, int BWD_ROWS, int nt_dx,
+                                                     float* __restrict__ part_w, float* __restrict__ part_b) {
     extern __shared__ __attribute__((aligned(16))) char smem[];
     float* red = (float*)smem;
     const int lane = threadIdx.x & 63, wave = threadIdx.x >> 6;
@@ -218,7 +219,7 @@
             }
         }
     }
-    if (!dw && !db) return;
+    if (!dw && !db && !part_w && !part_b) return;
 #pragma unroll
     for (int c = 0; c < MAXC; ++c) {
         const int ch = lane + 64 * c;
@@ -228,9 +229,61 @@
         }
     }
     __syncthreads();
+    if (part_w || part_b) {
+        for (int i = threadIdx.x; i < D; i += 256) {
+            if (part_w) part_w[(size_t)blockIdx.x * D + i] = (red[i] + red[D + i]) + (red[2 * D + i] + red[3 * D + i]);
+            if constexpr (HAS_DB) if (part_b) part_b[(size_t)blockIdx.x * D + i] = (red[4 * D + i] + red[5 * D + i]) + (red[6 * D + i] + red[7 * D + i]);
+        }
+        return;
+    }
     for (int i = threadIdx.x; i < D; i += 256) {
         if (dw) unsafeAtomicAdd(dw + i, (red[i] + red[D + i]) + (red[2 * D + i] + red[3 * D + i]));
         if constexpr (HAS_DB) if (db) unsafeAtomicAdd(db + i, (red[4 * D + i] + red[5 * D + i]) + (red[6 * D + i] + red[7 * D + i]));
+    }
+}
+
+struct LnReduceTable { fm_ln_reduce_job j[FM_LN_REDUCE_MAX_JOBS]; };
+constexpr int LN_RED_GROUPS = 64;
+__global__ __launch_bounds__(1024) void ln_dw_reduce_kernel(const LnReduceTable t, int n_jobs) {
+    __shared__ float4 red[LN_RED_GROUPS][16];
+    const fm_ln_reduce_job& me = t.j[blockIdx.y];
+    if (me.first != (int)blockIdx.y) return;
+    const int D = me.D, sub = threadIdx.x & 15, grp = threadIdx.x >> 4;
+    const int ch = blockIdx.x * 16 + sub;
+    if ((int)blockIdx.x * 64 >= D) return;
+    const bool live = ch * 4 < D;
+    float4 tot = make_float4(0.f, 0.f, 0.f, 0.f);
+    for (int j = blockIdx.y; j < n_jobs; ++j) {
+        if (t.j[j].first != (int)blockIdx.y) continue;
+        const float* part = (const float*)t.j[j].partials;
+        const int nb = t.j[j].n_blocks;
+        float4 a = make_float4(0.f, 0.f, 0.f, 0.f);
+        if (live) {
+            const int per = (nb + LN_RED_GROUPS - 1) / LN_RED_GROUPS, b0 = grp * per, b1 = min(nb, b0 + per);
+            int b = b0;
+            for (; b + 8 <= b1; b += 8) {
+                float4 v[8];
+#pragma unroll
+                for (int k = 0; k < 8; ++k) v[k] = *(const float4*)(part + (size_t)(b + k) * D + ch * 4);
+#pragma unroll
+                for (int k = 0; k < 8; ++k) { a.x += v[k].x; a.y += v[k].y; a.z += v[k].z; a.w += v[k].w; }
+            }
+            for (; b < b1; ++b) {
+                const float4 v = *(const float4*)(part + (size_t)b * D + ch * 4);
+                a.x += v.x; a.y += v.y; a.z += v.z; a.w += v.w;
+            }
+        }
+        red[grp][sub] = a;
+        __syncthreads();
+        if (grp == 0) {
+#pragma unroll 8
+            for (int q = 0; q < LN_RED_GROUPS; ++q) { const float4 v = red[q][sub]; tot.x += v.x; tot.y += v.y; tot.z += v.z; tot.w += v.w; }
+        }
+        __syncthreads();
+    }
+    if (grp == 0 && live) {
+        float* d = (float*)me.dst + ch * 4;
+        d[0] += tot.x; d[1] += tot.y; d[2] += tot.z; d[3] += tot.w;
     }
 }
 
@@ -363,7 +416,7 @@
 
 static int layernorm_bwd_launch(const void* dy, int lddy, const int32_t* dy_row_map, const void* h, int ldh, const void* x, int ldx, const void* w,
                                 const void* mean, const void* rstd, const void* dres, void* dx, int lddx, void* dx_bf16,
-                                int lddxbf, void* dw, void* db, int R, int D, void* stream) {
+                                int lddxbf, void* dw, void* db, int R, int D, void* stream, void* part_w = nullptr, void* part_b = nullptr) {
     FM_CHECK_ARG(dy && x && w && mean && rstd && dx, "fm_layernorm_bwd: null pointer");
     FM_CHECK_ARG(!h || ldh % 4 == 0, "fm_layernorm_bwd_h: ldh must be a multiple of 4");
     FM_CHECK_ARG(R > 0 && D > 0 && D % 4 == 0 && D <= 64 * 4 * MAXC_LIMIT, "fm_layernorm_bwd: D=%d unsupported", D);
@@ -378,7 +431,8 @@
         (void)once;                                                                                                         \
         hipLaunchKernelGGL(k, dim3(grid), dim3(256), lds, (hipStream_t)stream, (const bf16_t*)dy, lddy, dy_row_map, (const bf16_t*)h, ldh, \
                            (const float*)x, ldx, (const float*)w, (const float*)mean, (const float*)rstd, (const float*)dres, (float*)dx, lddx, \
-                           (bf16_t*)dx_bf16, lddxbf, (float*)dw, (float*)db, R, D, BWD_ROWS, ((ln_nt_flags() >> 1) & 1) | ((ln_nt_flags() >> 2) & 2) | ((ln_nt_flags() >> 2) & 4));                               \
+                           (bf16_t*)dx_bf16, lddxbf, (float*)dw, (float*)db, R, D, BWD_ROWS, ((ln_nt_flags() >> 1) & 1) | ((ln_nt_flags() >> 2) & 2) | ((ln_nt_flags() >> 2) & 4), \
+                           (float*)part_w, (float*)part_b);                                                                 \
     }
 #define LN_BWD(C) { if (h) LN_BWD_(C, true) else LN_BWD_(C, false) }
     switch (chunks_for(D)) {
@@ -404,6 +458,41 @@
                                   int lddxbf, void* dw, int R, int D, void* stream) {
     FM_CHECK_ARG(h, "fm_layernorm_bwd_h: null pointer");
     return layernorm_bwd_launch(dy, lddy, nullptr, h, ldh, x, ldx, w, mean, rstd, dres, dx, lddx, dx_bf16, lddxbf, dw, nullptr, R, D, stream);
+}
+
+extern "C" int fm_ln_bwd_blocks(int R) { return R > 0 ? (R + bwd_rows(R) - 1) / bwd_rows(R) : 0; }
+
+extern "C" int fm_layernorm_bwd_partials(const void* dy, int lddy, const int32_t* dy_row_map, const void* h, int ldh, const void* x, int ldx,
+                                         const void* w, const void* mean, const void* rstd, const void* dres, void* dx, int lddx,
+                                         void* dx_bf16, int lddxbf, void* part_w, void* part_b, int R, int D, void* stream) {
+    FM_CHECK_ARG(part_w || part_b, "fm_layernorm_bwd_partials: no partials buffer");
+    FM_CHECK_ARG(!h || (!dy_row_map && !part_b), "fm_layernorm_bwd_partials: the from-h kernel takes no row map and no bias gradient");
+    FM_CHECK_ARG(((((uintptr_t)part_w) | ((uintptr_t)part_b)) & 15) == 0, "fm_layernorm_bwd_partials: partials must be 16-byte aligned");
+    return layernorm_bwd_launch(dy, lddy, dy_row_map, h, ldh, x, ldx, w, mean, rstd, dres, dx, lddx, dx_bf16, lddxbf, nullptr, nullptr, R, D, stream,
+                                part_w, part_b);
+}
+
+extern "C" int fm_ln_dw_reduce(const fm_ln_reduce_job* jobs, int n_jobs, void* stream) {
+    FM_CHECK_ARG(jobs && n_jobs > 0 && n_jobs <= FM_LN_REDUCE_MAX_JOBS, "fm_ln_dw_reduce: 1 .. %d jobs", FM_LN_REDUCE_MAX_JOBS);
+    LnReduceTable t;
+    int maxD = 0;
+    for (int i = 0; i < n_jobs; ++i) {
+        t.j[i] = jobs[i];
+        FM_CHECK_ARG(jobs[i].partials && jobs[i].dst && jobs[i].n_blocks > 0 && jobs[i].D > 0 && jobs[i].D % 4 == 0,
+                     "fm_ln_dw_reduce: job %d: null pointer or bad shape (n_blocks=%d, D=%d)", i, jobs[i].n_blocks, jobs[i].D);
+        FM_CHECK_ARG((((uintptr_t)jobs[i].partials) & 15) == 0, "fm_ln_dw_reduce: job %d: partials must be 16-byte aligned", i);
+        t.j[i].first = i;
+        for (int k = 0; k < i; ++k)
+            if (jobs[k].dst == jobs[i].dst) {
+                FM_CHECK_ARG(jobs[k].D == jobs[i].D, "fm_ln_dw_reduce: jobs %d and %d share a destination but not D", k, i);
+                t.j[i].first = k;
+                break;
+            }
+        maxD = std::max(maxD, jobs[i].D);
+    }
+    hipLaunchKernelGGL(ln_dw_reduce_kernel, dim3((maxD + 63) / 64, n_jobs), dim3(1024), 0, (hipStream_t)stream, t, n_jobs);
+    FM_CHECK_LAUNCH("fm_ln_dw_reduce");
+    return 0;
 }
 
 extern "C" int fm_headnorm_fwd(const void* x, int ldx, const void* w, const void* b, void* y, int ldy, void* stats, int R, int H, float eps,
diff --git a/ml-4m_amd/csrc/loss.hip b/ml-4m_amd/csrc/loss.hip
--- a/ml-4m_amd/csrc/loss.hip
+++ b/ml-4m_amd/csrc/loss.hip
@@ -1,3 +1,4 @@
+#include <algorithm>
 #include "common.h"
 #include "fourm_hip.h"
 
@@ -60,6 +61,41 @@
     m = mn;
 }
 
+__device__ __forceinline__ void unpack_chunk(const uint4 p, int c, int V, float (&v)[8]) {
+    const uint32_t w[4] = {p.x, p.y, p.z, p.w};
+#pragma unroll
+    for (int e = 0; e < 4; ++e) { v[2 * e] = bf2f((bf16_t)(w[e] & 0xffff)); v[2 * e + 1] = bf2f((bf16_t)(w[e] >> 16)); }
+    if (c + 8 > V) {
+#pragma unroll
+        for (int e = 0; e < 8; ++e) if (c + e >= V) v[e] = -INFINITY;
+    }
+}
+__device__ __forceinline__ void online_chunk(const float (&v)[8], float& m, float& ssum) {
+    float cm = v[0];
+#pragma unroll
+    for (int e = 1; e < 8; ++e) cm = fmaxf(cm, v[e]);
+    const float mn = fmaxf(m, cm);
+    float add = 0.f;
+#pragma unroll
+    for (int e = 0; e < 8; ++e) add += __expf(v[e] - mn);
+    ssum = ssum * __expf(m - mn) + add;
+    m = mn;
+}
+__device__ __forceinline__ float block_lse(float m, float ssum, float* red_m, float* red_s) {
+#pragma unroll
+    for (int o = 32; o > 0; o >>= 1) {
+        const float m2 = __shfl_xor(m, o, 64), s2 = __shfl_xor(ssum, o, 64);
+        if (m2 > -INFINITY || m > -INFINITY) online_merge(m, ssum, m2, s2);
+    }
+    const int lane = threadIdx.x & 63, wave = threadIdx.x >> 6;
+    if (lane == 0) { red_m[wave] = m; red_s[wave] = ssum; }
+    __syncthreads();
+    float M = red_m[0], S = red_s[0];
+    for (int w = 1; w < 4; ++w)
+        if (red_m[w] > -INFINITY) online_merge(M, S, red_m[w], red_s[w]);
+    return M + __logf(S);
+}
+
 __global__ __launch_bounds__(256) void ce_fwd_kernel(const bf16_t* __restrict__ logits, int ldl, const int32_t* __restrict__ perm,
                                                      const int32_t* __restrict__ tile_group, const long long* __restrict__ target_ids,
                                                      const int32_t* __restrict__ vocab, float* __restrict__ row_loss, float* __restrict__ row_lse) {
@@ -77,38 +113,15 @@
     float m = -INFINITY, ssum = 0.f;
     for (int c = threadIdx.x * 8; c < V; c += 256 * 8) {
         float v[8];
-        if (c + 8 <= V) {
-            const uint4 p = *(const uint4*)(row + c);
-            const uint32_t w[4] = {p.x, p.y, p.z, p.w};
-#pragma unroll
-            for (int e = 0; e < 4; ++e) { v[2 * e] = bf2f((bf16_t)(w[e] & 0xffff)); v[2 * e + 1] = bf2f((bf16_t)(w[e] >> 16)); }
-        } else {
+        if (c + 8 <= V) unpack_chunk(*(const uint4*)(row + c), c, V, v);
+        else {
 #pragma unroll
             for (int e = 0; e < 8; ++e) v[e] = c + e < V ? bf2f(row[c + e]) : -INFINITY;
         }
-        float cm = v[0];
-#pragma unroll
-        for (int e = 1; e < 8; ++e) cm = fmaxf(cm, v[e]);
-        const float mn = fmaxf(m, cm);
-        float add = 0.f;
-#pragma unroll
-        for (int e = 0; e < 8; ++e) add += __expf(v[e] - mn);
-        ssum = ssum * __expf(m - mn) + add;
-        m = mn;
-    }
-#pragma unroll
-    for (int o = 32; o > 0; o >>= 1) {
-        const float m2 = __shfl_xor(m, o, 64), s2 = __shfl_xor(ssum, o, 64);
-        if (m2 > -INFINITY || m > -INFINITY) online_merge(m, ssum, m2, s2);
-    }
-    const int lane = threadIdx.x & 63, wave = threadIdx.x >> 6;
-    if (lane == 0) { red_m[wave] = m; red_s[wave] = ssum; }
-    __syncthreads();
+        online_chunk(v, m, ssum);
+    }
+    const float lse = block_lse(m, ssum, red_m, red_s);
     if (threadIdx.x == 0) {
-        float M = red_m[0], S = red_s[0];
-        for (int w = 1; w < 4; ++w)
-            if (red_m[w] > -INFINITY) online_merge(M, S, red_m[w], red_s[w]);
-        const float lse = M + __logf(S);
         row_lse[pr] = lse;
         row_loss[pr] = lse - bf2f(row[target_ids[src]]);
     }
@@ -154,6 +167,82 @@
     }
 }
 
+__device__ __forceinline__ float head_coef(int g, int V, const int32_t* seg_count, const int32_t* vocab, int loss_type, int n_heads) {
+    if (loss_type == FM_LOSS_MOD) return 1.0f / ((float)seg_count[g] * (float)n_heads);
+    float tot = 0.f;
+    for (int mm = 0; mm < n_heads; ++mm) tot += (float)seg_count[mm] * (float)vocab[mm];
+    return (float)V / tot;
+}
+
+template <int NCH>
+__global__ __launch_bounds__(256) void ce_fused_kernel(bf16_t* __restrict__ logits, int ldl, const int32_t* __restrict__ perm,
+                                                       const int32_t* __restrict__ tile_group, const long long* __restrict__ target_ids,
+                                                       const int32_t* __restrict__ vocab, const int32_t* __restrict__ seg_count,
+                                                       int loss_type, int n_heads, float* __restrict__ row_loss, float* __restrict__ row_lse) {
+    __shared__ float red_m[4], red_s[4];
+    const int pr = blockIdx.x;
+    const int g = tile_group[pr / SEG_ALIGN];
+    if (g < 0) return;
+    const int V = vocab[g];
+    const int Vp = (V + 63) / 64 * 64;
+    bf16_t* row = logits + (size_t)pr * ldl;
+    const int src = perm[pr];
+    if (src < 0) {
+        if (threadIdx.x == 0) { row_loss[pr] = 0.f; row_lse[pr] = 0.f; }
+        for (int c = threadIdx.x; c < Vp / 8; c += 256) *(uint4*)(row + c * 8) = make_uint4(0u, 0u, 0u, 0u);
+        return;
+    }
+    uint4 keep[NCH];
+#pragma unroll
+    for (int k = 0; k < NCH; ++k) {
+        const int c = (k * 256 + threadIdx.x) * 8;
+        keep[k] = c < Vp ? *(const uint4*)(row + c) : make_uint4(0u, 0u, 0u, 0u);
+    }
+    const int tgt = (int)target_ids[src];
+    const float xt = bf2f(row[tgt]);
+    float m = -INFINITY, ssum = 0.f;
+#pragma unroll
+    for (int k = 0; k < NCH; ++k) {
+        const int c = (k * 256 + threadIdx.x) * 8;
+        if (c < V) {
+            float v[8];
+            unpack_chunk(keep[k], c, V, v);
+            online_chunk(v, m, ssum);
+        }
+    }
+    const float lse = block_lse(m, ssum, red_m, red_s);
+    if (threadIdx.x == 0) { row_lse[pr] = lse; row_loss[pr] = lse - xt; }
+    const float w = head_coef(g, V, seg_count, vocab, loss_type, n_heads);
+#pragma unroll
+    for (int k = 0; k < NCH; ++k) {
+        const int c = (k * 256 + threadIdx.x) * 8;
+        if (c < Vp) {
+            float v[8], o[8];
+            unpack_chunk(keep[k], c, Vp, v);
+#pragma unroll
+            for (int e = 0; e < 8; ++e) o[e] = (c + e < V) ? (__expf(v[e] - lse) - ((c + e) == tgt ? 1.f : 0.f)) * w : 0.f;
+            *(uint4*)(row + c) = make_uint4(pack2bf(o[0], o[1]), pack2bf(o[2], o[3]), pack2bf(o[4], o[5]), pack2bf(o[6], o[7]));
+        }
+    }
+}
+
+__global__ __launch_bounds__(256) void ce_scale_kernel(bf16_t* __restrict__ logits, int ldl, const int32_t* __restrict__ tile_group,
+                                                       const int32_t* __restrict__ vocab, const float* __restrict__ gscale, int Rp) {
+    const float s = gscale[0];
+    if (s == 1.0f) return;
+    for (int pr = blockIdx.x; pr < Rp; pr += gridDim.x) {
+        const int g = tile_group[pr / SEG_ALIGN];
+        if (g < 0) continue;
+        const int Vp = (vocab[g] + 63) / 64 * 64;
+        bf16_t* row = logits + (size_t)pr * ldl;
+        for (int c = threadIdx.x * 8; c < Vp; c += 256 * 8) {
+            float v[8];
+            unpack_chunk(*(const uint4*)(row + c), c, Vp, v);
+            *(uint4*)(row + c) = make_uint4(pack2bf(v[0] * s, v[1] * s), pack2bf(v[2] * s, v[3] * s), pack2bf(v[4] * s, v[5] * s), pack2bf(v[6] * s, v[7] * s));
+        }
+    }
+}
+
 __global__ __launch_bounds__(256) void loss_finalize_kernel(const float* __restrict__ row_loss, const int32_t* __restrict__ seg_start,
                                                             const int32_t* __restrict__ seg_count, const int32_t* __restrict__ vocab,
                                                             int n_heads, int loss_type, float* __restrict__ head_loss, float* __restrict__ total) {
@@ -275,11 +364,29 @@
     FM_CHECK_ARG(loss_type == FM_LOSS_MOD || loss_type == FM_LOSS_TOKEN, "fm_cross_entropy: invalid loss type %d", loss_type);
     FM_CHECK_ARG(ldl % 8 == 0 && ldl >= (max_vocab + 63) / 64 * 64, "fm_cross_entropy: ldl=%d too small for vocab %d", ldl, max_vocab);
     FM_CHECK_ARG((((uintptr_t)logits) & 15) == 0, "fm_cross_entropy: logits must be 16-byte aligned");
-    if (!write_grad) {
+    FM_CHECK_ARG(write_grad >= 0 && write_grad <= FM_CE_SCALE, "fm_cross_entropy: invalid mode %d", write_grad);
+    FM_CHECK_ARG(Rp > 0, "fm_cross_entropy: Rp=%d", Rp);
+    if (write_grad == FM_CE_SCALE) {
+        FM_CHECK_ARG(grad_scale, "fm_cross_entropy: the rescale needs grad_scale");
+        hipLaunchKernelGGL(ce_scale_kernel, dim3(std::min(Rp, 1024)), dim3(256), 0, (hipStream_t)stream, (bf16_t*)logits, ldl, tile_group, vocab,
+                           (const float*)grad_scale, Rp);
+    } else if (write_grad == FM_CE_FUSED && max_vocab <= FM_CE_FUSED_MAX_VOCAB) {
+#define CE_FUSED(NCH)                                                                                                                      \
+    hipLaunchKernelGGL(ce_fused_kernel<NCH>, dim3(Rp), dim3(256), 0, (hipStream_t)stream, (bf16_t*)logits, ldl, perm, tile_group,          \
+                       (const long long*)target_ids, vocab, seg_count, loss_type, n_heads, (float*)row_loss, (float*)row_lse)
+        const int nch = ((max_vocab + 63) / 64 * 64 + 2047) / 2048;
+        if (nch <= 4) CE_FUSED(4); else if (nch <= 8) CE_FUSED(8); else CE_FUSED(16);
+#undef CE_FUSED
+        hipLaunchKernelGGL(loss_finalize_kernel, dim3(1), dim3(256), 0, (hipStream_t)stream, (const float*)row_loss, seg_start, seg_count,
+                           vocab, n_heads, loss_type, (float*)head_loss, (float*)total_loss);
+    } else if (write_grad == 0 || write_grad == FM_CE_FUSED) {
         hipLaunchKernelGGL(ce_fwd_kernel, dim3(Rp), dim3(256), 0, (hipStream_t)stream, (const bf16_t*)logits, ldl, perm, tile_group,
                            (const long long*)target_ids, vocab, (float*)row_loss, (float*)row_lse);
         hipLaunchKernelGGL(loss_finalize_kernel, dim3(1), dim3(256), 0, (hipStream_t)stream, (const float*)row_loss, seg_start, seg_count,
                            vocab, n_heads, loss_type, (float*)head_loss, (float*)total_loss);
+        if (write_grad == FM_CE_FUSED)
+            hipLaunchKernelGGL(ce_bwd_kernel, dim3(Rp), dim3(256), 0, (hipStream_t)stream, (bf16_t*)logits, ldl, perm, tile_group,
+                               (const long long*)target_ids, vocab, seg_count, (const float*)nullptr, loss_type, n_heads, (const float*)row_lse);
     } else {
         hipLaunchKernelGGL(ce_bwd_kernel, dim3(Rp), dim3(256), 0, (hipStream_t)stream, (bf16_t*)logits, ldl, perm, tile_group,
                            (const long long*)target_ids, vocab, seg_count, (const float*)grad_scale, loss_type, n_heads, (const float*)row_lse);
diff --git a/ml-4m_amd/fourm/hip/_lib.py b/ml-4m_amd/fourm/hip/_lib.py
--- a/ml-4m_amd/fourm/hip/_lib.py
+++ b/ml-4m_amd/fourm/hip/_lib.py
@@ -30,6 +30,7 @@
 MASK_NONE, MASK_KEYPAD, MASK_DECODER, MASK_DENSE = 0, 1, 2, 3
 KIND_TOK, KIND_PATCH, KIND_SEQ, KIND_SEQ_EMB = 0, 1, 2, 3
 LOSS_MOD, LOSS_TOKEN = 0, 1
+CE_FUSED, CE_SCALE, CE_FUSED_MAX_VOCAB = 2, 3, 32768
 
 
 class GemmGroup(C.Structure):
@@ -92,6 +93,13 @@
 
 class FoldGradJob(C.Structure):
     _fields_ = [("dWp", vp), ("W", vp), ("gamma", vp), ("gW", vp), ("ggamma", vp), ("rows", i32), ("cols", i32), ("ld_dwp", i32), ("reserved", i32)]
+
+
+LN_REDUCE_MAX_JOBS = 64
+
+
+class LnReduceJob(C.Structure):
+    _fields_ = [("partials", vp), ("dst", vp), ("n_blocks", i32), ("D", i32), ("first", i32), ("reserved", i32)]
 
 
 class GemmF32Args(C.Structure):
@@ -152,6 +160,9 @@
 layernorm_fwd_res = _sig("fm_layernorm_fwd_res", vp, i32, vp, i32, vp, i32, vp, vp, vp, i32, i32, vp, vp, vp, i32, i32, f32, vp)
 layernorm_bwd = _sig("fm_layernorm_bwd", vp, i32, vp, vp, i32, vp, vp, vp, vp, vp, i32, vp, i32, vp, vp, i32, i32, vp)
 layernorm_bwd_h = _sig("fm_layernorm_bwd_h", vp, i32, vp, i32, vp, i32, vp, vp, vp, vp, vp, i32, vp, i32, vp, i32, i32, vp)
+ln_bwd_blocks = _sig("fm_ln_bwd_blocks", i32)
+layernorm_bwd_partials = _sig("fm_layernorm_bwd_partials", vp, i32, vp, vp, i32, vp, i32, vp, vp, vp, vp, vp, i32, vp, i32, vp, vp, i32, i32, vp)
+ln_dw_reduce = _sig("fm_ln_dw_reduce", P(LnReduceJob), C.c_int, vp)
 attn_fwd = _sig("fm_attn_fwd", P(AttnArgs), vp)
 attn_bwd = _sig("fm_attn_bwd", P(AttnArgs), vp)
 attn_decode = _sig("fm_attn_decode", P(AttnDecodeArgs), vp)
@@ -256,7 +267,7 @@
 vit_colsum = _sig("fm_vit_colsum", vp, i32, vp, i32, i32, vp, i64, vp)
 EXPORTS = ["fm_attn_decode", "fm_vit_patch_rows", "fm_vit_emb_rows", "fm_vit_colsum", "fm_lora_apply", "fm_lora_grad", "fm_vq_assign_wide", "fm_memcodes_assign", "fm_convnext_block", "fm_split3_bf16", "fm_unet_im2col", "fm_groupnorm_nhwc", "fm_add_bf16", "fm_silu_f32_to_bf16", "fm_timestep_embedding", "fm_unet_attention", "fm_diffusion_x0", "fm_quantile_abs",
            "fm_diffusion_step", "fm_unpack_image_u8", "fm_unpack_ids_u16", "fm_unpack_mask_bits", "fm_decoder_attention_from_target", "fm_guidance_combine", "fm_image_mask", "fm_token_budgets", "fm_span_mask", "fm_vq_code_stats", "fm_vq_ema_update", "fm_vq_code_bias", "fm_vq_assign_bias", "fm_vq_code_stats_raw", "fm_vq_ema_update_euclid", "fm_vq_unpatchify", "fm_vq_latent_grad", "fm_tanh_bwd_f32", "fm_embed_rows_f32", "fm_vq_patchify_ex", "fm_vq_cls_emb_bwd", "fm_vq_latent_grad_normalized", "fm_abi_version", "fm_last_error", "fm_gemm_nt", "fm_set_gemm_nt_config", "fm_get_gemm_nt_config", "fm_set_reserved_cus", "fm_get_reserved_cus", "fm_bf16_to_f32_scaled", "fm_add_bf16_f32", "fm_scale_rows_bf16", "fm_gemm_tn", "fm_gemm_tn_multi", "fm_set_gemm_tn_config", "fm_get_gemm_tn_config", "fm_set_tn_transpose_read",
-           "fm_get_tn_transpose_read", "fm_layernorm_fwd", "fm_layernorm_fwd_res", "fm_layernorm_bwd", "fm_layernorm_bwd_h", "fm_headnorm_fwd", "fm_headnorm_bwd", "fm_attn_fwd", "fm_attn_bwd",
+           "fm_get_tn_transpose_read", "fm_layernorm_fwd", "fm_layernorm_fwd_res", "fm_layernorm_bwd", "fm_layernorm_bwd_h", "fm_ln_bwd_blocks", "fm_layernorm_bwd_partials", "fm_ln_dw_reduce", "fm_headnorm_fwd", "fm_headnorm_bwd", "fm_attn_fwd", "fm_attn_bwd",
            "fm_set_attn_transpose_read", "fm_get_attn_transpose_read", "fm_select_embed", "fm_embed_bwd",
            "fm_dense_decoder_mask", "fm_segment_rows", "fm_gather_rows", "fm_cross_entropy", "fm_swiglu_bwd",
            "fm_gelu_bwd", "fm_cast_pad", "fm_transpose_cast_pad", "fm_shadow_refresh", "fm_fold_colscale_grad", "fm_colsum", "fm_f32_to_bf16", "fm_adamw", "fm_adamw_shadow",
diff --git a/ml-4m_amd/fourm/hip/engine.py b/ml-4m_amd/fourm/hip/engine.py
--- a/ml-4m_amd/fourm/hip/engine.py
+++ b/ml-4m_amd/fourm/hip/engine.py
@@ -17,6 +17,8 @@
 DEFER_RESIDUAL = os.environ.get("FOURM_DEFER_RESIDUAL", "1") == "1"
 HOIST_CTX = os.environ.get("FOURM_HOIST_CTX", "1") == "1"
 LN_BWD_FROM_H = os.environ.get("FOURM_LN_BWD_FROM_H", "1") == "1"
+LN_BWD_PARTIALS = os.environ.get("FOURM_LN_BWD_PARTIALS", "1") == "1"
+LN_PARTIAL_SLOTS = int(os.environ.get("FOURM_LN_PARTIAL_SLOTS", "16"))
 DP_RESERVE_ALWAYS = os.environ.get("FOURM_DP_RESERVE_ALWAYS", "0") == "1"
 
 
@@ -130,6 +132,7 @@
 
 class FourMEngine:
     _pending = None
+    _ln_ring = None
     _drop_now = None
     drop_uniforms = None
 
@@ -249,6 +252,8 @@
 
     def _stage(self, name):
         if self.reducer is not None:
+            if self._ln_ring is not None:
+                self._ln_ring.flush()
             self.reducer.stage_done(name)
 
     def grad_view(self, p):
@@ -771,11 +776,13 @@
         hs["total"] = ws.get("heads.total", (1,), torch.float32)
         return hs
 
-    def loss_forward(self, dec, hs, loss_type):
+    def loss_forward(self, dec, hs, loss_type, save=False):
         lt = L.LOSS_MOD if loss_type in ("mod", "modality") else L.LOSS_TOKEN
         hs["loss_type"] = lt
+        hs["ce_fused"] = bool(save) and not self.fp32
         ops.cross_entropy(hs["logits"], hs["perm"], hs["tile_group"], dec["target_ids"].view(-1), hs["vocab_t"], hs["seg_start"],
-                          hs["seg_count"], hs["n"], hs["maxV"], hs["row_loss"], hs["row_lse"], hs["head_loss"], hs["total"], loss_type=lt)
+                          hs["seg_count"], hs["n"], hs["maxV"], hs["row_loss"], hs["row_lse"], hs["head_loss"], hs["total"], loss_type=lt,
+                          write_grad="fused" if hs["ce_fused"] else False)
         return hs["total"], hs["head_loss"]
 
     def dec_order(self, mod_dict):
@@ -793,7 +800,7 @@
         dec = self.select(mod_dict, n_dec, True, self.dec_order(mod_dict), "dec.")
         y, st = self.trunk_forward(enc, dec, save)
         hs = self.heads_setup(dec, y, save)
-        total, head_loss = self.loss_forward(dec, hs, loss_type)
+        total, head_loss = self.loss_forward(dec, hs, loss_type, save)
         if save:
             self._ctx = dict(enc=enc, dec=dec, st=st, hs=hs)
         return total, head_loss, hs["heads"], hs["seg_count"]
@@ -819,7 +826,8 @@
     def _ln_bwd(self, norm, dy, x, sv, key, g, g_bf, R, dres, dy_row_map=None):
         dw = self._g(norm.weight)
         db = self._g(norm.bias) if isinstance(norm.bias, nn.Parameter) else None
-        ops.layernorm_bwd(dy, x, norm.weight, sv[key + ".mu"], sv[key + ".rs"], g, dres=dres, dx_bf16=g_bf, dw=dw, db=db,
+        fn = ops.layernorm_bwd if self._ln_ring is None else self._ln_ring.ln_bwd
+        fn(dy, x, norm.weight, sv[key + ".mu"], sv[key + ".rs"], g, dres=dres, dx_bf16=g_bf, dw=dw, db=db,
                           dy_row_map=dy_row_map, R=R, h=sv.get(key + ".h"))
 
     def _mlp_bwd(self, mlp, sv, g_bf, R, Rp):
@@ -987,7 +995,7 @@
         c = self._ctx
         if c is None:
             raise RuntimeError("train_backward without a preceding training forward")
-        self._ctx, self._dw_jobs = None, None
+        self._ctx, self._dw_jobs, self._ln_ring = None, None, None
         if self.reducer is not None:
             self.reducer.begin()
             if getattr(self.reducer, "reserved_cus", 0):
@@ -998,9 +1006,12 @@
         bf, f32 = self.adt, torch.float32
         Rq, Rc = B * Mt, B * N
         Rqp, Rcp = st["y_final"].shape[0], st["x_final"].shape[0]
+        if LN_BWD_PARTIALS and not self.fp32:
+            slot = max(L.ln_bwd_blocks(Rq), L.ln_bwd_blocks(Rc)) * D
+            self._ln_ring = ops.LnPartials(ws.get("bwd.ln_partials", (LN_PARTIAL_SLOTS, slot), f32))
         ops.cross_entropy(hs["logits"], hs["perm"], hs["tile_group"], dec["target_ids"].view(-1), hs["vocab_t"], hs["seg_start"],
                           hs["seg_count"], hs["n"], hs["maxV"], hs["row_loss"], hs["row_lse"], hs["head_loss"], hs["total"],
-                          loss_type=hs["loss_type"], grad_scale=grad_scale, write_grad=True)
+                          loss_type=hs["loss_type"], grad_scale=grad_scale, write_grad="scale" if hs["ce_fused"] else True)
         dyp = ws.get("bwd.dyp", (hs["Rp"], D), bf)
         ops.gemm_nt_grouped(hs["logits"], hs["g_bwd"], hs["tile_group"], dyp, D, max_K=ru(hs["maxV"], 64))
         heads = [m.decoder_embeddings[h] for h in hs["heads"]]
@@ -1072,6 +1083,9 @@
             elif e.kind == L.KIND_SEQ_EMB and e.emb_proj.weight.requires_grad:
                 ops.gemm_tn(ge_bf, enc["seqemb_rows"], self.grad_view(e.emb_proj.weight), N=D, K=e.emb_proj.weight.shape[1], R=Rc)
         self._embed_bwd(enc, ge, dctx, False)
+        if self._ln_ring is not None:
+            self._ln_ring.flush()
+            self._ln_ring = None
         if self.reducer is not None:
             self.reducer.finish()
             if getattr(self.reducer, "reserved_cus", 0) and not DP_RESERVE_ALWAYS:
diff --git a/ml-4m_amd/fourm/hip/ops.py b/ml-4m_amd/fourm/hip/ops.py
--- a/ml-4m_amd/fourm/hip/ops.py
+++ b/ml-4m_amd/fourm/hip/ops.py
@@ -298,6 +298,44 @@
     return dx
 
 
+class LnPartials:
+
+    def __init__(self, buf):
+        assert buf.dtype == torch.float32 and buf.dim() == 2 and buf.is_contiguous() and 2 <= buf.shape[0] <= L.LN_REDUCE_MAX_JOBS
+        self.buf, self.jobs = buf, []
+
+    def ln_bwd(self, dy, x, w, mean, rstd, dx, *, dres=None, dx_bf16=None, dw=None, db=None, dy_row_map=None, R=None, h=None):
+        R = x.shape[0] if R is None else R
+        if (dw is None and db is None) or dy.dtype == torch.float32:
+            return layernorm_bwd(dy, x, w, mean, rstd, dx, dres=dres, dx_bf16=dx_bf16, dw=dw, db=db, dy_row_map=dy_row_map, R=R, h=h)
+        D, nb = w.numel(), L.ln_bwd_blocks(R)
+        if nb * D > self.buf.shape[1]:
+            raise ValueError(f"LnPartials: a slot holds {self.buf.shape[1]} floats, the norm needs {nb} x {D}")
+        if len(self.jobs) + (dw is not None) + (db is not None) > self.buf.shape[0]:
+            self.flush()
+        slot = {}
+        for name, dst in (("w", dw), ("b", db)):
+            if dst is not None:
+                slot[name] = self.buf[len(self.jobs)]
+                self.jobs.append((slot[name], nb, D, dst))
+        from_h = h is not None and db is None and dy_row_map is None
+        with _prof("layernorm_bwd", 0.0, R * D * (2 + (2 if from_h else 4) + 4 + 4 + (2 if dx_bf16 is not None else 0))):
+            L.check(L.layernorm_bwd_partials(_p(dy), _ld(dy), _p(dy_row_map), _p(h) if from_h else None, _ld(h) if from_h else 0, _p(x), _ld(x),
+                                             _p(w), _p(mean), _p(rstd), _p(dres), _p(dx), _ld(dx), _p(dx_bf16),
+                                             _ld(dx_bf16) if dx_bf16 is not None else 0, _p(slot.get("w")), _p(slot.get("b")), R, D, _stream()))
+        return dx
+
+    def flush(self):
+        if not self.jobs:
+            return
+        tab = (L.LnReduceJob * len(self.jobs))()
+        for t, (part, nb, D, dst) in zip(tab, self.jobs):
+            t.partials, t.dst, t.n_blocks, t.D = part.data_ptr(), dst.data_ptr(), nb, D
+        with _prof("layernorm_bwd", 0.0, sum(4 * nb * D for _, nb, D, _ in self.jobs)):
+            L.check(L.ln_dw_reduce(tab, len(self.jobs), _stream()))
+        self.jobs = []
+
+
 @_timed("headnorm")
 def headnorm_fwd(x, w, b, y, stats, R, H, eps):
     if x.dtype == torch.float32:
@@ -389,9 +427,12 @@
 def cross_entropy(logits, perm, tile_group, target_ids, vocab, seg_start, seg_count, n_heads, max_vocab, row_loss, row_lse, head_loss,
                   total_loss, *, loss_type=L.LOSS_MOD, grad_scale=None, write_grad=False):
     fn = L.cross_entropy_f32 if logits.dtype == torch.float32 else L.cross_entropy
+    mode = {False: 0, True: 1, "fused": L.CE_FUSED, "scale": L.CE_SCALE}[write_grad]
+    if mode > 1 and logits.dtype == torch.float32:
+        raise ValueError("cross_entropy: the fused training forward exists for bf16 logits only")
     L.check(fn(_p(logits), _ld(logits), _p(perm), _p(tile_group), _p(target_ids), _p(vocab), _p(seg_start),
                             _p(seg_count), _p(grad_scale), loss_type, n_heads, perm.numel(), max_vocab, _p(row_loss), _p(row_lse),
-                            _p(head_loss), _p(total_loss), 1 if write_grad else 0, _stream()))
+                            _p(head_loss), _p(total_loss), mode, _stream()))
 
 
 @_timed("swiglu_bwd")
```
